# AsteriosPar/mmWave_MSc

Hardware: NVIDIA B200
Metric: radar frames/sec (cluster+track+pose) (higher is better)
Workload: dtype f64

## Files before the change

### mmwave_msc_b200/csrc/mmw_api.cu

```cuda
#include <algorithm>
#include <climits>
#include <dlfcn.h>
#include <cmath>
#include <cstdio>
#include <cstdlib>
#include <cstring>
#include <new>
#include <string>
#include <utility>
#include <vector>

#include "dbscan.cuh"
#include "linalg.cuh"
#include "mmw_internal.cuh"
#include "pose.cuh"
#include "pose_tc.cuh"

using namespace mmw;

static thread_local std::string g_err;

static int fail(int code, const std::string& msg) {
    g_err = msg;
    return code;
}

#define CK(call)                                                                                   \
    do {                                                                                           \
        cudaError_t e__ = (call);                                                                  \
        if (e__ != cudaSuccess)                                                                    \
            return fail(MMW_ERR_CUDA, std::string(#call) + ": " + cudaGetErrorString(e__));        \
    } while (0)

constexpr int kGroup = 4;
constexpr size_t kStageSlack = 64;

struct StageSlot {
    float* pts = nullptr;
    size_t pts_cap = 0;
    int32_t* offsets = nullptr;
    double* dt = nullptr;
    uint8_t* pk = nullptr;
    size_t pk_cap = 0;
    cudaEvent_t uploaded = nullptr, free = nullptr;
};

struct mmw_ctx {
    mmw_config cfg;
    DevConfig dc;
    int device = 0, S = 0, ncap = 0, tcap = 0;
    cudaStream_t stream = nullptr;
    std::vector<mmw_scene_sensor> sensors;
    SensorRec* d_sensors = nullptr;
    double* d_doppler_wrap = nullptr;
    TrackRec* d_tracks = nullptr;
    SceneRec* d_scenes = nullptr;
    float* d_track_ring = nullptr;
    float* d_uring = nullptr;
    float* d_keypoints = nullptr;
    float* d_default_posture = nullptr;
    int32_t* d_assoc = nullptr;
    int32_t* d_labels = nullptr;
    unsigned long long* d_counters = nullptr;
    unsigned long long* d_phase = nullptr;
    bool phase_clocks = false;
    uint8_t* d_ring_hist = nullptr;
    int32_t* h_defer_hint = nullptr;
    int32_t* d_defer_hint = nullptr;
    int32_t* h_rows_hint = nullptr;
    int32_t* d_rows_hint = nullptr;
    int32_t* d_scene_stats = nullptr;
    int32_t* d_defer = nullptr;
    bool fold_pose_index = true;
    StageSlot stage[2];
    unsigned stage_idx = 0;
    unsigned stage_pending = 0;
    cudaStream_t h2d_stream = nullptr, d2h_stream = nullptr;
    cudaStream_t pose_stream = nullptr;
    cudaEvent_t feat_done[2] = {nullptr, nullptr}, packt_done[2] = {nullptr, nullptr}, pose_done[2] = {nullptr, nullptr};
    int32_t *d_row_scene2 = nullptr, *d_row_track2 = nullptr, *d_row_slot2 = nullptr;
    int* d_pose_total2 = nullptr;
    int32_t* d_pose_extra = nullptr;
    int rows_buf = 0;
    unsigned pipe_idx = 0;
    int pipe_r = -1;
    bool pose_pending = false;
    cudaEvent_t packed[2] = {nullptr, nullptr}, results_done[2] = {nullptr, nullptr};
    float* d_results[2] = {nullptr, nullptr};
    double* d_export = nullptr;
    int32_t* d_export_valid = nullptr;
    unsigned char* d_move = nullptr;
    size_t move_cap = 0;
    unsigned result_idx = 0;
    int variant = -1;
    bool has_weights = false;
    int D = 0, Kf = 0, H = 0;
    float* d_blob = nullptr;
    const float *w1 = nullptr, *b1 = nullptr, *w2 = nullptr, *b2 = nullptr, *wd1 = nullptr, *bd1 = nullptr,
                *wd2 = nullptr, *bd2 = nullptr;
    float *d_bn1s = nullptr, *d_bn1t = nullptr, *d_bn2s = nullptr, *d_bn2t = nullptr;
    float* d_feats = nullptr;
    int32_t *d_row_scene = nullptr, *d_row_track = nullptr, *d_row_slot = nullptr;
    int* d_pose_total = nullptr;
    float *d_act2 = nullptr, *d_act3 = nullptr, *d_pose_out = nullptr;
    int pose_cap = 0;
    PoseTc tc;
    bool use_tc = true;
    int last_pose_run = 0;
    uint64_t launches = 0;
    bool profiling = false;
    std::vector<std::pair<cudaEvent_t, int>> marks;
    double kernel_ms[MMW_N_KERNELS] = {0, 0, 0, 0, 0, 0, 0, 0};
    uint64_t kernel_calls[MMW_N_KERNELS] = {0, 0, 0, 0, 0, 0, 0, 0};
};

static cudaError_t sync_main(mmw_ctx* x) {
    if (x->pose_pending) {
        cudaError_t e = cudaStreamSynchronize(x->pose_stream);
        if (e != cudaSuccess) return e;
        x->pose_pending = false;
    }
    return cudaStreamSynchronize(x->stream);
}
static cudaError_t join_pose(mmw_ctx* x) {
    if (!x->pose_pending) return cudaSuccess;
    x->pose_pending = false;
    return cudaStreamWaitEvent(x->stream, x->pose_done[(x->pipe_idx + 1) & 1], 0);
}

static void prof_mark(mmw_ctx* x, int next_kernel) {
    if (!x->profiling) return;
    cudaEvent_t e;
    if (cudaEventCreate(&e) != cudaSuccess) return;
    cudaEventRecord(e, x->stream);
    x->marks.emplace_back(e, next_kernel);
}

static SensorRec sensor_rec(const mmw_scene_sensor& p) {
    SensorRec r{};
    const double ang = p.s_tilt_deg * (M_PI / 180.0);
    r.cos_t = std::cos(ang);
    r.sin_t = std::sin(ang);
    r.s_height = p.s_height;
    r.z_max = p.z_max;
    r.doppler_res = p.doppler_res;
    r.xyz_scale = (float)std::ldexp(1.0, -(p.xyz_q_format));
    return r;
}

static double doppler_wrap(const mmw_scene_sensor& p) { return (double)p.num_doppler_bins / 2 - 1; }

static mmw_scene_sensor config_sensor(const mmw_config& c) {
    mmw_scene_sensor p{};
    p.s_height = c.s_height;
    p.s_tilt_deg = c.s_tilt_deg;
    p.z_max = c.z_max;
    p.doppler_res = c.doppler_res != 0.0 ? c.doppler_res : 1.0;
    p.xyz_q_format = c.xyz_q_format;
    return p;
}

static void fill_devconfig(const mmw_config& c, int ncap, int tcap, DevConfig* d) {
    d->sensor = sensor_rec(config_sensor(c));
    d->db_z_weight = c.db_z_weight;
    d->db_range_weight = c.db_range_weight;
    d->db_eps = c.db_eps;
    d->life_dyn = c.tr_lifetime_dynamic;
    d->life_sta = c.tr_lifetime_static;
    d->vel_thres = c.tr_vel_thres;
    d->gate = c.tr_gate;
    d->q_var = c.kf_q_var;
    d->p_init = c.kf_p_init;
    d->g_init = c.kf_group_disp_init;
    d->a_n = c.kf_a_n;
    d->a_spr = c.kf_a_spr;
    for (int i = 0; i < 6; ++i) d->spread_lim[i] = c.kf_spread_lim[i];
    d->int_mu = c.intensity_mu;
    d->int_std = c.intensity_std;
    d->nudge_thres = c.x_nudge_thres;
    d->nudge_gain = c.x_nudge_gain;
    d->db_min_samples = c.db_min_samples;
    d->ring_size = c.frames_batch + 1;
    d->tr_max_tracks = c.tr_max_tracks;
    d->enable_est = c.kf_enable_est;
    d->est_pointnum = c.kf_est_pointnum;
    d->ncap = ncap;
    d->tcap = tcap;
    grid_screen_config(c.db_eps, c.db_range_weight, c.db_z_weight, c.db_min_samples, &d->grid_inv_h, &d->grid_ybound,
                       &d->grid_ok);
    screen_config(c.db_eps, c.db_range_weight, c.db_z_weight, &d->screen_lo, &d->screen_hi, &d->screen_rmax);
}

static const float kDefaultPosture[57] = {
    0.0000f, -0.0007f, -0.0006f, -0.0038f, -0.1820f, -0.2540f, -0.2579f, 0.1830f, 0.2957f, 0.2940f,
    -0.0805f, -0.1141f, -0.1232f, -0.1358f, 0.0796f, 0.1436f, 0.1558f, 0.1720f, -0.0007f, 0.7699f,
    1.0906f, 1.4020f, 1.5513f, 1.2893f, 1.0360f, 0.7994f, 1.2865f, 1.0483f, 0.8117f, 0.7670f,
    0.3428f, 0.0000f, -0.0746f, 0.7713f, 0.3706f, -0.0128f, -0.0796f, 1.3255f, 0.0752f, 0.0533f,
    0.0203f, 0.0000f, 0.0496f, 0.1350f, 0.1303f, 0.0345f, 0.1277f, 0.1050f, 0.0392f, 0.0533f,
    0.0786f, -0.0056f, 0.0346f, -0.0007f, 0.0683f, -0.0082f, 0.0312f};

extern "C" {

int mmw_abi_version(void) { return MMW_ABI_VERSION; }
const char* mmw_last_error(void) { return g_err.c_str(); }

int mmw_default_config(mmw_config* c) {
    if (!c) return fail(MMW_ERR_INVALID, "cfg is NULL");
    std::memset(c, 0, sizeof(*c));
    c->s_height = 1.8; c->s_tilt_deg = -5; c->z_max = 2.5;
    c->frames_batch = 2; c->db_min_samples = 35;
    c->db_z_weight = 0.4; c->db_range_weight = 0.03; c->db_eps = 0.3;
    c->tr_max_tracks = 4; c->kf_enable_est = 0;
    c->tr_lifetime_dynamic = 3; c->tr_lifetime_static = 7; c->tr_vel_thres = 0.12; c->tr_gate = 4.5;
    c->kf_q_var = 1; c->kf_p_init = 0.1; c->kf_group_disp_init = 0.1; c->kf_a_n = 0.9; c->kf_a_spr = 0.9;
    const double lim[6] = {0.2, 0.2, 2, 1.2, 1.2, 0.2};
    for (int i = 0; i < 6; ++i) c->kf_spread_lim[i] = lim[i];
    c->kf_est_pointnum = 10;
    c->intensity_mu = 27.0187; c->intensity_std = 70.351;
    c->x_nudge_thres = 0.6; c->x_nudge_gain = 0.4;
    std::memcpy(c->default_posture, kDefaultPosture, sizeof(kDefaultPosture));
    c->m_x = 0.32; c->m_y = -0.6; c->m_z = 1.3;
    c->fade_size_max = 0.3; c->fade_size_min = 0.2; c->fade_weight = 0.08;
    c->doppler_res = 1.0;
    c->xyz_q_format = 9;
    return MMW_OK;
}

int mmw_destroy(mmw_ctx* x) {
    if (!x) return MMW_OK;
    cudaSetDevice(x->device);
    if (x->stream) cudaStreamSynchronize(x->stream);
    void* ptrs[] = {x->d_sensors, x->d_doppler_wrap, x->d_export, x->d_export_valid, x->d_move, x->d_tracks, x->d_scenes, x->d_track_ring, x->d_uring, x->d_keypoints, x->d_default_posture,
                    x->d_assoc, x->d_labels, x->d_counters, x->d_phase, x->d_defer, x->d_scene_stats, x->d_ring_hist,
                    x->d_results[0], x->d_results[1], x->d_blob, x->d_bn1s,
                    x->d_bn1t, x->d_bn2s, x->d_bn2t, x->d_feats, x->d_row_scene, x->d_row_track, x->d_row_slot,
                    x->d_pose_total, x->d_act2, x->d_act3, x->d_pose_out, x->d_row_scene2, x->d_row_track2, x->d_row_slot2,
                    x->d_pose_total2, x->d_pose_extra};
    for (void* p : ptrs)
        if (p) cudaFree(p);
    pose_tc_free(&x->tc);
    if (x->h_defer_hint) cudaFreeHost(x->h_defer_hint);
    if (x->h_rows_hint) cudaFreeHost(x->h_rows_hint);
    for (int i = 0; i < 2; ++i) {
        const StageSlot& s = x->stage[i];
        for (void* p : {(void*)s.pts, (void*)s.offsets, (void*)s.dt, (void*)s.pk})
            if (p) cudaFree(p);
        for (cudaEvent_t e : {s.uploaded, s.free, x->packed[i], x->results_done[i], x->feat_done[i], x->packt_done[i],
                              x->pose_done[i]})
            if (e) cudaEventDestroy(e);
    }
    if (x->h2d_stream) cudaStreamDestroy(x->h2d_stream);
    if (x->d2h_stream) cudaStreamDestroy(x->d2h_stream);
    if (x->pose_stream) { cudaStreamSynchronize(x->pose_stream); cudaStreamDestroy(x->pose_stream); }
    if (x->stream) cudaStreamDestroy(x->stream);
    delete x;
    return MMW_OK;
}

int mmw_reset(mmw_ctx* x) {
    if (!x) return fail(MMW_ERR_INVALID, "ctx is NULL");
    CK(cudaSetDevice(x->device));
    if (x->pose_stream) CK(join_pose(x));
    x->pipe_r = -1;
    x->last_pose_run = 0;
    CK(cudaMemsetAsync(x->d_scenes, 0, sizeof(SceneRec) * x->S, x->stream));
    CK(cudaMemsetAsync(x->d_tracks, 0, sizeof(TrackRec) * (size_t)x->S * x->tcap, x->stream));
    CK(cudaMemsetAsync(x->d_counters, 0, sizeof(unsigned long long) * 8, x->stream));
    CK(cudaMemsetAsync(x->d_assoc, 0xff, sizeof(int32_t) * (size_t)x->S * x->ncap, x->stream));
    CK(cudaMemsetAsync(x->d_pose_total, 0, sizeof(int), x->stream));
    CK(cudaMemsetAsync(x->d_pose_total2, 0, sizeof(int), x->stream));
    CK(cudaMemsetAsync(x->d_pose_extra, 0, 2 * sizeof(int32_t), x->stream));
    CK(cudaMemsetAsync(x->d_defer, 0, sizeof(int32_t) * (2 + 2 * (size_t)x->S), x->stream));
    CK(cudaMemsetAsync(x->d_scene_stats, 0, sizeof(int32_t) * 8 * (size_t)x->S, x->stream));
    CK(cudaMemsetAsync(x->d_ring_hist, 0, (size_t)kRing * kHistBytes * x->S, x->stream));
    return MMW_OK;
}

namespace {
struct StateHeader {
    uint32_t magic, abi;
    int32_t S, ncap, tcap, ring_size;
    uint64_t bytes;
};
constexpr uint32_t kStateMagic = 0x4d4d5753u;
struct StatePart { void* dev; size_t bytes; };
enum { kPartScene, kPartTracks, kPartTrackRing, kPartURing, kPartHist, kPartKeypoints, kPartPoseCnt, kNumStateParts };
std::vector<StatePart> state_parts(mmw_ctx* x) {
    const size_t S = x->S;
    return {{x->d_scenes, sizeof(SceneRec) * S},
            {x->d_tracks, sizeof(TrackRec) * S * x->tcap},
            {x->d_track_ring, sizeof(float) * S * x->tcap * kRing * kFeatPts * kRawCols},
            {x->d_uring, sizeof(float) * S * kRing * x->ncap * kRawCols},
            {x->d_ring_hist, (size_t)kRing * kHistBytes * S},
            {x->d_keypoints, sizeof(float) * S * x->tcap * kKp},
            {x->d_defer + 1 + S, sizeof(int32_t) * S}};
}
}

size_t mmw_state_size(mmw_ctx* x) {
    if (!x) return 0;
    size_t n = sizeof(StateHeader);
    for (const StatePart& p : state_parts(x)) n += p.bytes;
    return n;
}

int mmw_state_dump(mmw_ctx* x, void* host_blob, size_t bytes) {
    if (!x || !host_blob) return fail(MMW_ERR_INVALID, "ctx/host_blob is NULL");
    const size_t need = mmw_state_size(x);
    if (bytes < need) return fail(MMW_ERR_CAPACITY, "state blob buffer is smaller than mmw_state_size()");
    CK(cudaSetDevice(x->device));
    CK(sync_main(x));
    StateHeader h{kStateMagic, MMW_ABI_VERSION, x->S, x->ncap, x->tcap, x->dc.ring_size, (uint64_t)need};
    unsigned char* o = static_cast<unsigned char*>(host_blob);
    std::memcpy(o, &h, sizeof(h));
    o += sizeof(h);
    for (const StatePart& p : state_parts(x)) {
        CK(cudaMemcpy(o, p.dev, p.bytes, cudaMemcpyDeviceToHost));
        o += p.bytes;
    }
    return MMW_OK;
}

int mmw_state_restore(mmw_ctx* x, const void* host_blob, size_t bytes) {
    if (!x || !host_blob) return fail(MMW_ERR_INVALID, "ctx/host_blob is NULL");
    StateHeader h;
    if (bytes < sizeof(h)) return fail(MMW_ERR_INVALID, "state blob is truncated");
    std::memcpy(&h, host_blob, sizeof(h));
    if (h.magic != kStateMagic || h.abi != MMW_ABI_VERSION)
        return fail(MMW_ERR_INVALID, "not a state blob of this library version");
    if (h.S != x->S || h.ncap != x->ncap || h.tcap != x->tcap || h.ring_size != x->dc.ring_size)
        return fail(MMW_ERR_INVALID, "state blob was taken from a context of another shape "
                                     "(n_scenes / max_points_per_frame / max_tracks / frames_batch)");
    if (h.bytes != mmw_state_size(x) || bytes < h.bytes) return fail(MMW_ERR_INVALID, "state blob is truncated");
    CK(cudaSetDevice(x->device));
    CK(mmw_sync(x) == MMW_OK ? cudaSuccess : cudaErrorUnknown);
    const unsigned char* o = static_cast<const unsigned char*>(host_blob) + sizeof(h);
    for (const StatePart& p : state_parts(x)) {
        CK(cudaMemcpy(p.dev, o, p.bytes, cudaMemcpyHostToDevice));
        o += p.bytes;
    }
    return MMW_OK;
}

int mmw_create(const mmw_config* cfg, int device, int n_scenes, int max_points, int max_tracks, mmw_ctx** out) {
    if (!cfg || !out) return fail(MMW_ERR_INVALID, "cfg/out is NULL");
    if (n_scenes < 1 || max_points < 1 || max_tracks < 1 || max_tracks > kMaxTcap)
        return fail(MMW_ERR_INVALID, "n_scenes >= 1, max_points >= 1, 1 <= max_tracks <= 32 required");
    if (cfg->frames_batch < 0 || cfg->frames_batch > kRing - 1)
        return fail(MMW_ERR_INVALID, "frames_batch must be 0..2");
    if (cfg->xyz_q_format < 0 || cfg->xyz_q_format > 15) return fail(MMW_ERR_INVALID, "xyz_q_format must be 0..15");
    if (cfg->db_min_samples < 1 || cfg->tr_max_tracks < 0)
        return fail(MMW_ERR_INVALID, "db_min_samples >= 1 and tr_max_tracks >= 0 required");
    int ndev = 0;
    CK(cudaGetDeviceCount(&ndev));
    if (device < 0 || device >= ndev) return fail(MMW_ERR_CUDA, "no such CUDA device");
    CK(cudaSetDevice(device));
    cudaDeviceProp prop;
    CK(cudaGetDeviceProperties(&prop, device));
    const int smem = step_smem_bytes(max_points, max_tracks);
    if ((size_t)smem > prop.sharedMemPerBlockOptin || (size_t)dbscan_big_smem_bytes(max_points) > prop.sharedMemPerBlockOptin)
        return fail(MMW_ERR_CAPACITY, "max_points/max_tracks need more shared memory than one CTA can have");
    mmw_ctx* x = new (std::nothrow) mmw_ctx();
    if (!x) return fail(MMW_ERR_INVALID, "out of host memory");
    x->cfg = *cfg;
    x->device = device; x->S = n_scenes; x->ncap = max_points; x->tcap = max_tracks;
    fill_devconfig(*cfg, max_points, max_tracks, &x->dc);
    const size_t S = n_scenes;
#define ALLOC(p, bytes)                                                       \
    do {                                                                      \
        cudaError_t e__ = cudaMalloc((void**)&(p), (bytes));                  \
        if (e__ != cudaSuccess) {                                             \
            mmw_destroy(x);                                                   \
            return fail(MMW_ERR_CUDA, std::string("cudaMalloc: ") + cudaGetErrorString(e__)); \
        }                                                                     \
    } while (0)
    if (cudaStreamCreateWithFlags(&x->stream, cudaStreamNonBlocking) != cudaSuccess) {
        delete x;
        return fail(MMW_ERR_CUDA, "cudaStreamCreate failed");
    }
    ALLOC(x->d_tracks, sizeof(TrackRec) * S * max_tracks);
    ALLOC(x->d_scenes, sizeof(SceneRec) * S);
    ALLOC(x->d_track_ring, sizeof(float) * S * max_tracks * kRing * kFeatPts * kRawCols);
    ALLOC(x->d_uring, sizeof(float) * S * kRing * max_points * kRawCols);
    ALLOC(x->d_keypoints, sizeof(float) * S * max_tracks * kKp);
    ALLOC(x->d_default_posture, sizeof(float) * kKp);
    ALLOC(x->d_assoc, sizeof(int32_t) * S * max_points);
    ALLOC(x->d_labels, sizeof(int32_t) * S * 3 * max_points);
    ALLOC(x->d_counters, sizeof(unsigned long long) * 8);
    ALLOC(x->d_phase, sizeof(unsigned long long) * (16 + 3 * S + 16));
    ALLOC(x->d_defer, sizeof(int32_t) * (2 + 2 * S));
    ALLOC(x->d_scene_stats, sizeof(int32_t) * 8 * S);
    if (cudaHostAlloc((void**)&x->h_defer_hint, sizeof(int32_t), cudaHostAllocMapped) == cudaSuccess) {
        *x->h_defer_hint = 0;
        if (cudaHostGetDevicePointer((void**)&x->d_defer_hint, x->h_defer_hint, 0) != cudaSuccess) x->d_defer_hint = nullptr;
    } else {
        (void)cudaGetLastError();
        x->h_defer_hint = nullptr;
    }
    if (cudaHostAlloc((void**)&x->h_rows_hint, sizeof(int32_t), cudaHostAllocMapped) == cudaSuccess) {
        *x->h_rows_hint = 0;
        if (cudaHostGetDevicePointer((void**)&x->d_rows_hint, x->h_rows_hint, 0) != cudaSuccess) x->d_rows_hint = nullptr;
    } else {
        (void)cudaGetLastError();
        x->h_rows_hint = nullptr;
    }
    ALLOC(x->d_ring_hist, (size_t)kRing * kHistBytes * S);
    {
        const char* env = getenv("MMW_POSE_INDEX_FOLD");
        x->fold_pose_index = S <= 4096 && !(env && env[0] == '0');
    }
    for (int i = 0; i < 2; ++i) {
        StageSlot& st = x->stage[i];
        st.pts_cap = sizeof(float) * kRawCols * S * max_points + kStageSlack;
        ALLOC(st.pts, st.pts_cap);
        ALLOC(st.offsets, sizeof(int32_t) * kGroup * (S + 1));
        ALLOC(st.dt, sizeof(double) * kGroup * S);
        ALLOC(x->d_results[i], sizeof(float) * S * max_tracks * MMW_RESULT_FLOATS);
        if (cudaEventCreateWithFlags(&st.uploaded, cudaEventDisableTiming) != cudaSuccess ||
            cudaEventCreateWithFlags(&st.free, cudaEventDisableTiming) != cudaSuccess ||
            cudaEventCreateWithFlags(&x->packed[i], cudaEventDisableTiming) != cudaSuccess ||
            cudaEventCreateWithFlags(&x->results_done[i], cudaEventDisableTiming) != cudaSuccess ||
            cudaEventCreateWithFlags(&x->feat_done[i], cudaEventDisableTiming) != cudaSuccess ||
            cudaEventCreateWithFlags(&x->packt_done[i], cudaEventDisableTiming) != cudaSuccess ||
            cudaEventCreateWithFlags(&x->pose_done[i], cudaEventDisableTiming) != cudaSuccess) {
            mmw_destroy(x);
            return fail(MMW_ERR_CUDA, "cudaEventCreate failed");
        }
    }
    int prio_lo = 0, prio_hi = 0;
    cudaDeviceGetStreamPriorityRange(&prio_lo, &prio_hi);
    if (cudaStreamCreateWithFlags(&x->h2d_stream, cudaStreamNonBlocking) != cudaSuccess ||
        cudaStreamCreateWithPriority(&x->pose_stream, cudaStreamNonBlocking, prio_hi) != cudaSuccess ||
        cudaStreamCreateWithFlags(&x->d2h_stream, cudaStreamNonBlocking) != cudaSuccess) {
        mmw_destroy(x);
        return fail(MMW_ERR_CUDA, "cudaStreamCreate failed");
    }
    ALLOC(x->d_pose_total, sizeof(int));
    ALLOC(x->d_pose_extra, 2 * sizeof(int32_t));
    x->pose_cap = n_scenes * max_tracks;
    ALLOC(x->d_row_scene, sizeof(int32_t) * x->pose_cap);
    ALLOC(x->d_row_track, sizeof(int32_t) * x->pose_cap);
    ALLOC(x->d_row_slot, sizeof(int32_t) * x->pose_cap);
    ALLOC(x->d_row_scene2, sizeof(int32_t) * x->pose_cap);
    ALLOC(x->d_row_track2, sizeof(int32_t) * x->pose_cap);
    ALLOC(x->d_row_slot2, sizeof(int32_t) * x->pose_cap);
    ALLOC(x->d_pose_total2, sizeof(int));
    ALLOC(x->d_feats, sizeof(float) * (size_t)x->pose_cap * kRing * kFeatPts * kRawCols);
    ALLOC(x->d_pose_out, sizeof(float) * (size_t)x->pose_cap * kKp);
    ALLOC(x->d_sensors, sizeof(SensorRec) * S);
    ALLOC(x->d_doppler_wrap, sizeof(double) * S);
#undef ALLOC
    cudaMemcpy(x->d_default_posture, cfg->default_posture, sizeof(float) * kKp, cudaMemcpyHostToDevice);
    x->sensors.assign(S, config_sensor(*cfg));
    {
        const std::vector<SensorRec> recs(S, x->dc.sensor);
        const std::vector<double> wrap(S, doppler_wrap(x->sensors[0]));
        if (cudaMemcpy(x->d_sensors, recs.data(), sizeof(SensorRec) * S, cudaMemcpyHostToDevice) != cudaSuccess ||
            cudaMemcpy(x->d_doppler_wrap, wrap.data(), sizeof(double) * S, cudaMemcpyHostToDevice) != cudaSuccess) {
            mmw_destroy(x);
            return fail(MMW_ERR_CUDA, "upload of the sensor table failed");
        }
    }
    cudaMemset(x->d_keypoints, 0, sizeof(float) * S * max_tracks * kKp);
    int rc = mmw_reset(x);
    if (rc != MMW_OK) { mmw_destroy(x); return rc; }
    sync_main(x);
    *out = x;
    return MMW_OK;
}

static int upload_sensors(mmw_ctx* x, int first, int n) {
    std::vector<SensorRec> recs(n);
    std::vector<double> wrap(n);
    for (int i = 0; i < n; ++i) {
        recs[i] = sensor_rec(x->sensors[first + i]);
        wrap[i] = doppler_wrap(x->sensors[first + i]);
    }
    CK(cudaSetDevice(x->device));
    CK(cudaMemcpyAsync(x->d_sensors + first, recs.data(), sizeof(SensorRec) * n, cudaMemcpyHostToDevice, x->stream));
    CK(cudaMemcpyAsync(x->d_doppler_wrap + first, wrap.data(), sizeof(double) * n, cudaMemcpyHostToDevice, x->stream));
    return MMW_OK;
}

int mmw_set_doppler_resolution(mmw_ctx* x, double doppler_res) {
    if (!x) return fail(MMW_ERR_INVALID, "ctx is NULL");
    if (!(doppler_res > 0.0) || !std::isfinite(doppler_res)) return fail(MMW_ERR_INVALID, "doppler_res must be positive and finite");
    x->cfg.doppler_res = doppler_res;
    x->dc.sensor.doppler_res = doppler_res;
    for (mmw_scene_sensor& p : x->sensors) p.doppler_res = doppler_res;
    return upload_sensors(x, 0, x->S);
}

static const char* sensor_error(const mmw_scene_sensor& p) {
    if (!std::isfinite(p.s_height) || !std::isfinite(p.s_tilt_deg) || !std::isfinite(p.z_max) ||
        !std::isfinite(p.doppler_res))
        return "sensor parameters must be finite";
    if (!(p.doppler_res > 0.0)) return "doppler_res must be positive";
    if (p.xyz_q_format < 0 || p.xyz_q_format > 15) return "xyz_q_format must be 0..15";
    if (p.num_doppler_bins < 0) return "num_doppler_bins must not be negative";
    return nullptr;
}

int mmw_set_scene_sensors(mmw_ctx* x, int first, int n, const mmw_scene_sensor* params) {
    if (!x || !params) return fail(MMW_ERR_INVALID, "ctx/params is NULL");
    if (first < 0 || n < 0 || n > x->S - first) return fail(MMW_ERR_INVALID, "scene range out of bounds");
    for (int i = 0; i < n; ++i)
        if (const char* e = sensor_error(params[i])) return fail(MMW_ERR_INVALID, e);
    if (n == 0) return MMW_OK;
    for (int i = 0; i < n; ++i) x->sensors[first + i] = params[i];
    return upload_sensors(x, first, n);
}

int mmw_get_scene_sensors(mmw_ctx* x, int first, int n, mmw_scene_sensor* out) {
    if (!x || !out) return fail(MMW_ERR_INVALID, "ctx/out is NULL");
    if (first < 0 || n < 0 || n > x->S - first) return fail(MMW_ERR_INVALID, "scene range out of bounds");
    for (int i = 0; i < n; ++i) out[i] = x->sensors[first + i];
    return MMW_OK;
}

static int check_scene_list(const mmw_ctx* x, const int32_t* scenes, int n) {
    if (n < 0) return fail(MMW_ERR_INVALID, "n must not be negative");
    std::vector<char> seen(x->S, 0);
    for (int i = 0; i < n; ++i) {
        const int s = scenes[i];
        if (s < 0 || s >= x->S) return fail(MMW_ERR_INVALID, "scene index out of range");
        if (seen[s]) return fail(MMW_ERR_INVALID, "scene index listed twice");
        seen[s] = 1;
    }
    return MMW_OK;
}

int mmw_reset_scenes(mmw_ctx* x, const int32_t* scenes, int n) {
    if (!x || (!scenes && n > 0)) return fail(MMW_ERR_INVALID, "ctx/scenes is NULL");
    const int rc = check_scene_list(x, scenes, n);
    if (rc != MMW_OK) return rc;
    CK(cudaSetDevice(x->device));
    if (x->pose_stream) CK(join_pose(x));
    int32_t* pose_cnt = x->d_defer + 1 + x->S;
    for (int i = 0; i < n; ++i) {
        const size_t s = scenes[i];
        CK(cudaMemsetAsync(x->d_scenes + s, 0, sizeof(SceneRec), x->stream));
        CK(cudaMemsetAsync(x->d_tracks + s * x->tcap, 0, sizeof(TrackRec) * x->tcap, x->stream));
        CK(cudaMemsetAsync(x->d_ring_hist + s * kRing * kHistBytes, 0, (size_t)kRing * kHistBytes, x->stream));
        CK(cudaMemsetAsync(x->d_scene_stats + s * 8, 0, sizeof(int32_t) * 8, x->stream));
        CK(cudaMemsetAsync(pose_cnt + s, 0, sizeof(int32_t), x->stream));
    }
    return MMW_OK;
}

int mmw_sync(mmw_ctx* x) {
    if (!x) return fail(MMW_ERR_INVALID, "ctx is NULL");
    CK(cudaSetDevice(x->device));
    CK(cudaStreamSynchronize(x->h2d_stream));
    CK(sync_main(x));
    CK(cudaStreamSynchronize(x->d2h_stream));
    return MMW_OK;
}

void* mmw_stream(mmw_ctx* x) { return x ? (void*)x->stream : nullptr; }
uint64_t mmw_launch_count(mmw_ctx* x) { return x ? x->launches : 0; }

int mmw_load_pose_weights(mmw_ctx* x, int variant, const float* blob, size_t n) {
    if (!x || !blob) return fail(MMW_ERR_INVALID, "ctx/blob is NULL");
    if (variant != MMW_POSE_2D && variant != MMW_POSE_3D) return fail(MMW_ERR_INVALID, "unknown pose variant");
    const int D = variant == MMW_POSE_3D ? 3 : 1;
    if (D != x->dc.ring_size)
        return fail(MMW_ERR_INVALID, "pose variant does not match frames_batch (2-D net needs frames_batch=0, "
                                     "3-D net needs frames_batch=2; Utils.py:517-520)");
    const int taps = D == 3 ? 27 : 9;
    const int Kf = D * 64 * 32, H = D * 512;
    const size_t sz[16] = {(size_t)taps * 5 * 16, 16, (size_t)taps * 16 * 32, 32, 32, 32, 32, 32,
                           (size_t)Kf * H, (size_t)H, (size_t)H, (size_t)H, (size_t)H, (size_t)H,
                           (size_t)H * kKp, (size_t)kKp};
    size_t off[17];
    off[0] = 0;
    for (int i = 0; i < 16; ++i) off[i + 1] = off[i] + sz[i];
    if (n != off[16]) return fail(MMW_ERR_INVALID, "weight blob has the wrong number of floats for this variant");
    CK(cudaSetDevice(x->device));
    CK(sync_main(x));
    x->has_weights = false;
    x->last_pose_run = 0;
    if (x->d_blob) { cudaFree(x->d_blob); x->d_blob = nullptr; }
    for (float** p : {&x->d_bn1s, &x->d_bn1t, &x->d_bn2s, &x->d_bn2t, &x->d_act2, &x->d_act3})
        if (*p) { cudaFree(*p); *p = nullptr; }
    CK(cudaMalloc((void**)&x->d_blob, sizeof(float) * n));
    CK(cudaMemcpy(x->d_blob, blob, sizeof(float) * n, cudaMemcpyHostToDevice));
    x->w1 = x->d_blob + off[0]; x->b1 = x->d_blob + off[1];
    x->w2 = x->d_blob + off[2]; x->b2 = x->d_blob + off[3];
    x->wd1 = x->d_blob + off[8]; x->bd1 = x->d_blob + off[9];
    x->wd2 = x->d_blob + off[14]; x->bd2 = x->d_blob + off[15];
    auto bn = [&](size_t g, int cnt, float** ds, float** dt) -> int {
        std::vector<float> sc(cnt), sh(cnt);
        for (int i = 0; i < cnt; ++i) {
            const float gamma = blob[off[g] + i], beta = blob[off[g + 1] + i], mean = blob[off[g + 2] + i],
                        var = blob[off[g + 3] + i];
            const float s = gamma / std::sqrt(var + 1e-3f);
            sc[i] = s;
            sh[i] = beta - mean * s;
        }
        if (cudaMalloc((void**)ds, sizeof(float) * cnt) != cudaSuccess) return -1;
        if (cudaMalloc((void**)dt, sizeof(float) * cnt) != cudaSuccess) return -1;
        cudaMemcpy(*ds, sc.data(), sizeof(float) * cnt, cudaMemcpyHostToDevice);
        cudaMemcpy(*dt, sh.data(), sizeof(float) * cnt, cudaMemcpyHostToDevice);
        return 0;
    };
    if (bn(4, 32, &x->d_bn1s, &x->d_bn1t) || bn(10, H, &x->d_bn2s, &x->d_bn2t))
        return fail(MMW_ERR_CUDA, "cudaMalloc failed for BatchNorm constants");
    CK(cudaMalloc((void**)&x->d_act2, sizeof(float) * (size_t)x->pose_cap * Kf));
    CK(cudaMalloc((void**)&x->d_act3, sizeof(float) * (size_t)x->pose_cap * H));
    x->variant = variant; x->D = D; x->Kf = Kf; x->H = H;
    int rc = pose_tc_init(&x->tc, blob, off, D, x->pose_cap);
    if (rc != 0) return fail(MMW_ERR_CUDA, std::string("tensor-core dense path init failed: ") + pose_tc_error());
    x->has_weights = true;
    return MMW_OK;
}

static int run_pose_tc(mmw_ctx* x, const PoseTcRun& r, int max_rows, int b, cudaStream_t st,
                       cudaEvent_t before_fc2 = nullptr) {
    const bool marks = st == x->stream;
    int nl = 0;
    if (marks) prof_mark(x, MMW_K_CONV);
    if (pose_tc_conv(&x->tc, r, st, &nl, b) != 0) return fail(MMW_ERR_CUDA, std::string("tensor-core conv: ") + pose_tc_error());
    x->launches += nl;
    if (marks) prof_mark(x, MMW_K_FC1);
    if (pose_tc_fc1(&x->tc, r, max_rows, st, &nl, x->h_rows_hint ? *(volatile int32_t*)x->h_rows_hint : 0) != 0)
        return fail(MMW_ERR_CUDA, std::string("tensor-core dense 1: ") + pose_tc_error());
    x->launches += nl;
    if (before_fc2) CK(cudaStreamWaitEvent(st, before_fc2, 0));
    if (marks) prof_mark(x, MMW_K_FC2);
    if (pose_tc_fc2(&x->tc, r, max_rows, st, &nl) != 0) return fail(MMW_ERR_CUDA, std::string("tensor-core dense 2: ") + pose_tc_error());
    x->launches += nl;
    if (marks) prof_mark(x, -1);
    return MMW_OK;
}

static int run_pose_net(mmw_ctx* x, float* keypoints_by_slot, int max_rows) {
    x->last_pose_run = x->use_tc && x->tc.ready ? 1 : 2;
    if (x->use_tc && x->tc.ready) {
        PoseTcRun r{x->d_pose_total, x->b1, x->b2, x->d_bn1s, x->d_bn1t, x->bd1, x->d_bn2s, x->d_bn2t, x->bd2,
                    x->d_pose_out, keypoints_by_slot, x->d_row_scene, x->d_row_slot, x->tcap};
        return run_pose_tc(x, r, max_rows, 0, x->stream);
    }
    ConvArgs ca{x->d_feats, x->w1, x->b1, x->w2, x->b2, x->d_bn1s, x->d_bn1t, x->d_act2, x->d_pose_total};
    int grid = max_rows < 296 ? max_rows : 296;
    prof_mark(x, MMW_K_CONV);
    CK(launch_conv(ca, x->D, grid, x->stream));
    x->launches++;
    FcArgs fa{x->d_act2, x->wd1, x->bd1, x->d_bn2s, x->d_bn2t, x->d_act3, x->d_pose_total, x->Kf, x->H};
    prof_mark(x, MMW_K_FC1);
    CK(launch_fc1_simt(fa, max_rows, x->stream));
    x->launches++;
    Fc2Args f2{x->d_act3, x->wd2, x->bd2, x->d_pose_out, keypoints_by_slot, x->d_row_scene, x->d_row_slot,
               x->d_pose_total, x->H, x->tcap};
    grid = (max_rows + 7) / 8 < 148 * 4 ? (max_rows + 7) / 8 : 148 * 4;
    prof_mark(x, MMW_K_FC2);
    CK(launch_fc2(f2, grid, x->stream));
    x->launches++;
    prof_mark(x, -1);
    return MMW_OK;
}

static int pipeline_pose(mmw_ctx* x);
static int estimate_posture_impl(mmw_ctx* x, bool late);
static int launch_pack_tracks(mmw_ctx* x, float* results);

static int launch_feature_stage(mmw_ctx* x, int b, bool late, cudaStream_t st) {
    int* pose_total = b ? x->d_pose_total2 : x->d_pose_total;
    if (!x->fold_pose_index) {
        prof_mark(x, MMW_K_POSE_INDEX);
        CK(launch_pose_index(x->d_scenes, x->S, pose_total, x->d_counters, st));
        x->launches++;
    }
    PoseFeatArgs fa{x->dc, x->d_sensors, x->d_scenes, x->d_tracks, x->d_track_ring, x->d_feats,
                    (x->use_tc && x->tc.ready) ? pose_tc_input(&x->tc, b) : nullptr, b ? x->d_row_scene2 : x->d_row_scene,
                    b ? x->d_row_track2 : x->d_row_track, b ? x->d_row_slot2 : x->d_row_slot,
                    x->fold_pose_index ? x->d_defer + 1 + x->S : nullptr, pose_total, x->d_counters, x->S};
    fa.rows_hint = x->d_rows_hint;
    fa.late_extra = late ? x->d_pose_extra + b : nullptr;
    x->rows_buf = b;
    prof_mark(x, MMW_K_POSE_FEATURES);
    CK(launch_pose_features(fa, x->S, st));
    x->launches++;
    return MMW_OK;
}

static int check_step_flags(const mmw_ctx* x, uint32_t flags) {
    if ((flags & MMW_STEP_POSE) && !x->has_weights)
        return fail(MMW_ERR_STATE, "MMW_STEP_POSE needs mmw_load_pose_weights first");
    if ((flags & MMW_STEP_PIPELINE) && (!(flags & MMW_STEP_POSE) || !(x->use_tc && x->tc.ready)))
        return fail(MMW_ERR_STATE, "MMW_STEP_PIPELINE needs MMW_STEP_POSE and the tensor-core pose path");
    if ((flags & MMW_STEP_PIPELINE) && (flags & MMW_STEP_RECORD_LABELS))
        return fail(MMW_ERR_INVALID, "MMW_STEP_PIPELINE cannot record labels");
    return MMW_OK;
}

static long long offsets_total(const int32_t* offsets, int S) {
    if (offsets[0] != 0) return -1;
    for (int i = 0; i < S; ++i)
        if (offsets[i] > offsets[i + 1]) return -1;
    return offsets[S];
}


static cudaError_t grow(void** buf, size_t* cap, size_t bytes) {
    if (bytes <= *cap) return cudaSuccess;
    cudaError_t e = cudaFree(*buf);
    *buf = nullptr;
    *cap = 0;
    if (e == cudaSuccess && (e = cudaMalloc(buf, bytes)) == cudaSuccess) *cap = bytes;
    return e;
}

static int stage_acquire(mmw_ctx* x, size_t pts_bytes, size_t pk_bytes, int* k) {
    for (int i = 0; i < 2; ++i)
        if (x->stage_pending & (1u << i)) CK(cudaEventRecord(x->stage[i].free, x->stream));
    x->stage_pending = 0;
    *k = (int)(x->stage_idx++ & 1u);
    StageSlot& s = x->stage[*k];
    if (pts_bytes + kStageSlack > s.pts_cap || pk_bytes > s.pk_cap) {
        CK(cudaEventSynchronize(s.free));
        CK(grow((void**)&s.pts, &s.pts_cap, pts_bytes + kStageSlack));
        CK(grow((void**)&s.pk, &s.pk_cap, pk_bytes));
    }
    CK(cudaStreamWaitEvent(x->h2d_stream, s.free, 0));
    return MMW_OK;
}

static int stage_submit(mmw_ctx* x, int k) {
    CK(cudaEventRecord(x->stage[k].uploaded, x->h2d_stream));
    CK(cudaStreamWaitEvent(x->stream, x->stage[k].uploaded, 0));
    return MMW_OK;
}

static void stage_release(mmw_ctx* x, int k) { x->stage_pending |= 1u << k; }

static int step_queue(mmw_ctx* x, StepArgs& a, uint32_t flags);

int mmw_step(mmw_ctx* x, const float* pts, const int32_t* offsets, const double* dt, uint32_t flags) {
    if (!x || !offsets || !dt) return fail(MMW_ERR_INVALID, "ctx/offsets/dt is NULL");
    if ((flags & MMW_STEP_DEVICE_INPUT) && !pts) return fail(MMW_ERR_INVALID, "pts is NULL");
    int rc = check_step_flags(x, flags);
    if (rc != MMW_OK) return rc;
    CK(cudaSetDevice(x->device));
    StepArgs a;
    if (flags & MMW_STEP_DEVICE_INPUT) {
        a.pts = pts; a.offsets = offsets; a.dt = dt;
        return step_queue(x, a, flags);
    }
    const long long total = offsets_total(offsets, x->S);
    if (total < 0) return fail(MMW_ERR_INVALID, "offsets must start at 0 and must not decrease");
    if (total > (long long)x->S * x->ncap)
        return fail(MMW_ERR_CAPACITY, "more points than n_scenes * max_points_per_frame");
    if (total > 0 && !pts) return fail(MMW_ERR_INVALID, "pts is NULL");
    const size_t bytes = ((flags & MMW_STEP_INPUT_I16) ? sizeof(int16_t) : sizeof(float)) * kRawCols * total;
    int k;
    if ((rc = stage_acquire(x, bytes, 0, &k)) != MMW_OK) return rc;
    const StageSlot& s = x->stage[k];
    if (total) CK(cudaMemcpyAsync(s.pts, pts, bytes, cudaMemcpyHostToDevice, x->h2d_stream));
    CK(cudaMemcpyAsync(s.offsets, offsets, sizeof(int32_t) * (x->S + 1), cudaMemcpyHostToDevice, x->h2d_stream));
    CK(cudaMemcpyAsync(s.dt, dt, sizeof(double) * x->S, cudaMemcpyHostToDevice, x->h2d_stream));
    if ((rc = stage_submit(x, k)) != MMW_OK) return rc;
    a.pts = s.pts; a.offsets = s.offsets; a.dt = s.dt;
    rc = step_queue(x, a, flags);
    stage_release(x, k);
    return rc;
}

static int step_queue(mmw_ctx* x, StepArgs& a, uint32_t flags) {
    a.cfg = x->dc;
    a.sensors = x->d_sensors;
    a.tracks = x->d_tracks; a.scenes = x->d_scenes; a.track_ring = x->d_track_ring; a.uring = x->d_uring;
    a.keypoints = x->d_keypoints; a.default_posture = x->d_default_posture; a.assoc_out = x->d_assoc;
    a.labels_out = (flags & MMW_STEP_RECORD_LABELS) ? x->d_labels : nullptr;
    a.counters = x->d_counters; a.n_scenes = x->S; a.flags = flags;
    a.phase_cycles = x->phase_clocks ? x->d_phase : nullptr;
    a.defer_count = x->d_defer;
    a.defer_done = x->d_defer + 1 + 2 * x->S;
    a.defer_list = x->d_defer + 1;
    a.pose_cnt = x->d_defer + 1 + x->S;
    a.scene_stats = x->d_scene_stats;
    a.defer_hint = x->d_defer_hint;
    a.ring_hist = x->d_ring_hist;
    const bool pipelined = (flags & MMW_STEP_PIPELINE) != 0;
    const bool late = !pipelined && (flags & MMW_STEP_POSE) && x->fold_pose_index && x->use_tc && x->tc.ready;
    if (late) {
        a.nr_feats = x->d_feats;
        a.nr_packed = pose_tc_input(&x->tc);
        a.nr_row_scene = x->d_row_scene;
        a.nr_row_track = x->d_row_track;
        a.nr_row_slot = x->d_row_slot;
        a.nr_extra = x->d_pose_extra;
    }
    if (pipelined) {
        if (x->pipe_idx >= 2) CK(cudaStreamWaitEvent(x->stream, x->pose_done[x->pipe_idx & 1u], 0));
    } else {
        CK(join_pose(x));
        x->pipe_r = -1;
    }
    prof_mark(x, MMW_K_STEP);
    CK(launch_step(a, x->stream));
    prof_mark(x, MMW_K_DBSCAN_BIG);
    CK(launch_dbscan_big(a, x->stream, x->h_defer_hint ? *(volatile int32_t*)x->h_defer_hint : 16));
    x->launches += 2;
    prof_mark(x, -1);
    if (pipelined) return pipeline_pose(x);
    if (flags & MMW_STEP_POSE) return estimate_posture_impl(x, late);
    return MMW_OK;
}

int mmw_estimate_posture(mmw_ctx* x) { return estimate_posture_impl(x, false); }

static int estimate_posture_impl(mmw_ctx* x, bool late) {
    if (!x) return fail(MMW_ERR_INVALID, "ctx is NULL");
    if (!x->has_weights) return fail(MMW_ERR_STATE, "estimate_posture needs mmw_load_pose_weights first");
    CK(cudaSetDevice(x->device));
    CK(join_pose(x));
    const int rc = launch_feature_stage(x, 0, late, x->stream);
    if (rc != MMW_OK) return rc;
    return run_pose_net(x, x->d_keypoints, x->pose_cap);
}

int mmw_pose_features_only(mmw_ctx* x) {
    if (!x) return fail(MMW_ERR_INVALID, "ctx is NULL");
    CK(cudaSetDevice(x->device));
    CK(join_pose(x));
    x->last_pose_run = 0;
    return launch_feature_stage(x, 0, false, x->stream);
}

int mmw_set_keypoints(mmw_ctx* x, int scene, int track_index, const float* kp57) {
    if (!x || !kp57) return fail(MMW_ERR_INVALID, "NULL argument");
    if (scene < 0 || scene >= x->S || track_index < 0 || track_index >= x->tcap)
        return fail(MMW_ERR_INVALID, "scene/track out of range");
    CK(cudaSetDevice(x->device));
    CK(sync_main(x));
    TrackRec t;
    CK(cudaMemcpy(&t, x->d_tracks + (size_t)scene * x->tcap + track_index, sizeof(t), cudaMemcpyDeviceToHost));
    CK(cudaMemcpy(x->d_keypoints + ((size_t)scene * x->tcap + t.slot) * kKp, kp57, sizeof(float) * kKp,
                  cudaMemcpyHostToDevice));
    return MMW_OK;
}

int mmw_get_tracks(mmw_ctx* x, mmw_track_out* tracks, int32_t* n_tracks) {
    if (!x) return fail(MMW_ERR_INVALID, "ctx is NULL");
    CK(cudaSetDevice(x->device));
    CK(sync_main(x));
    std::vector<SceneRec> sc(x->S);
    CK(cudaMemcpy(sc.data(), x->d_scenes, sizeof(SceneRec) * x->S, cudaMemcpyDeviceToHost));
    if (n_tracks)
        for (int s = 0; s < x->S; ++s) n_tracks[s] = sc[s].n_tracks;
    if (!tracks) return MMW_OK;
    std::vector<TrackRec> tr((size_t)x->S * x->tcap);
    std::vector<float> kp((size_t)x->S * x->tcap * kKp);
    CK(cudaMemcpy(tr.data(), x->d_tracks, sizeof(TrackRec) * tr.size(), cudaMemcpyDeviceToHost));
    CK(cudaMemcpy(kp.data(), x->d_keypoints, sizeof(float) * kp.size(), cudaMemcpyDeviceToHost));
    for (int s = 0; s < x->S; ++s) {
        for (int k = 0; k < x->tcap; ++k) {
            mmw_track_out& o = tracks[(size_t)s * x->tcap + k];
            std::memset(&o, 0, sizeof(o));
            if (k >= sc[s].n_tracks) { o.id = -1; continue; }
            const TrackRec& t = tr[(size_t)s * x->tcap + k];
            o.id = t.id; o.point_num = t.point_num; o.is_static = t.is_static; o.ring_frames = t.ring_n;
            for (int f = 0; f < kRing; ++f)
                o.ring_counts[f] = f < t.ring_n ? t.ring_cnt[(t.ring_head + f) % x->dc.ring_size] : -1;
            o.lifetime = t.lifetime; o.n_est = t.n_est;
            std::memcpy(o.x, t.x, sizeof(t.x)); std::memcpy(o.P, t.P, sizeof(t.P));
            std::memcpy(o.spread_est, t.spread, sizeof(t.spread));
            std::memcpy(o.group_disp_est, t.G, sizeof(t.G));
            std::memcpy(o.centroid, t.centroid, sizeof(t.centroid));
            std::memcpy(o.min_vals, t.minv, sizeof(t.minv)); std::memcpy(o.max_vals, t.maxv, sizeof(t.maxv));
            std::memcpy(o.keypoints, &kp[((size_t)s * x->tcap + t.slot) * kKp], sizeof(float) * kKp);
        }
    }
    return MMW_OK;
}

int mmw_get_scene_summary(mmw_ctx* x, int32_t* n_tracks, int32_t* next_id, int32_t* last_M) {
    if (!x) return fail(MMW_ERR_INVALID, "ctx is NULL");
    CK(cudaSetDevice(x->device));
    std::vector<SceneRec> sc(x->S);
    CK(cudaMemcpyAsync(sc.data(), x->d_scenes, sizeof(SceneRec) * x->S, cudaMemcpyDeviceToHost, x->stream));
    CK(sync_main(x));
    for (int s = 0; s < x->S; ++s) {
        if (n_tracks) n_tracks[s] = sc[s].n_tracks;
        if (next_id) next_id[s] = sc[s].next_id;
        if (last_M) last_M[s] = sc[s].last_M;
    }
    return MMW_OK;
}

int mmw_get_point_assoc(mmw_ctx* x, int32_t* assoc, size_t n) {
    if (!x || !assoc) return fail(MMW_ERR_INVALID, "ctx/assoc is NULL");
    if (n > (size_t)x->S * x->ncap) return fail(MMW_ERR_CAPACITY, "n exceeds n_scenes * max_points_per_frame");
    CK(cudaSetDevice(x->device));
    CK(cudaMemcpyAsync(assoc, x->d_assoc, sizeof(int32_t) * n, cudaMemcpyDeviceToHost, x->stream));
    CK(sync_main(x));
    return MMW_OK;
}

int mmw_get_labels(mmw_ctx* x, int32_t* labels, int32_t* n_fused) {
    if (!x) return fail(MMW_ERR_INVALID, "ctx is NULL");
    CK(cudaSetDevice(x->device));
    CK(sync_main(x));
    if (labels)
        CK(cudaMemcpy(labels, x->d_labels, sizeof(int32_t) * (size_t)x->S * 3 * x->ncap, cudaMemcpyDeviceToHost));
    if (n_fused) {
        std::vector<SceneRec> sc(x->S);
        CK(cudaMemcpy(sc.data(), x->d_scenes, sizeof(SceneRec) * x->S, cudaMemcpyDeviceToHost));
        for (int s = 0; s < x->S; ++s) n_fused[s] = sc[s].last_ran ? sc[s].dbscan_n : -1;
    }
    return MMW_OK;
}

int mmw_get_status(mmw_ctx* x, uint32_t* flags) {
    if (!x || !flags) return fail(MMW_ERR_INVALID, "ctx/flags is NULL");
    CK(cudaSetDevice(x->device));
    CK(sync_main(x));
    std::vector<SceneRec> sc(x->S);
    CK(cudaMemcpy(sc.data(), x->d_scenes, sizeof(SceneRec) * x->S, cudaMemcpyDeviceToHost));
    for (int s = 0; s < x->S; ++s) flags[s] = sc[s].flags;
    return MMW_OK;
}

int mmw_get_ring_counts(mmw_ctx* x, int32_t* counts) {
    if (!x || !counts) return fail(MMW_ERR_INVALID, "ctx/counts is NULL");
    CK(cudaSetDevice(x->device));
    CK(sync_main(x));
    std::vector<SceneRec> sc(x->S);
    CK(cudaMemcpy(sc.data(), x->d_scenes, sizeof(SceneRec) * x->S, cudaMemcpyDeviceToHost));
    for (int s = 0; s < x->S; ++s)
        for (int f = 0; f < kRing; ++f)
            counts[s * kRing + f] =
                f < sc[s].ring_n ? sc[s].ring_cnt[(sc[s].ring_head + f) % x->dc.ring_size] : -1;
    return MMW_OK;
}

static int ring_edit(mmw_ctx* x, int scene, bool clear) {
    if (!x) return fail(MMW_ERR_INVALID, "ctx is NULL");
    if (scene < 0 || scene >= x->S) return fail(MMW_ERR_INVALID, "scene out of range");
    CK(cudaSetDevice(x->device));
    CK(sync_main(x));
    SceneRec sc;
    CK(cudaMemcpy(&sc, x->d_scenes + scene, sizeof(sc), cudaMemcpyDeviceToHost));
    if (clear) {
        sc.ring_n = 0; sc.ring_head = 0; sc.ring_cnt[0] = sc.ring_cnt[1] = sc.ring_cnt[2] = 0;
        sc.ring_ph_gone = 1;
    } else if (!sc.ring_ph_gone) {
        sc.ring_ph_gone = 1;
    } else if (sc.ring_n > 0) {
        sc.ring_cnt[sc.ring_head] = 0;
        sc.ring_head = (sc.ring_head + 1) % x->dc.ring_size;
        sc.ring_n -= 1;
    }
    CK(cudaMemcpy(x->d_scenes + scene, &sc, sizeof(sc), cudaMemcpyHostToDevice));
    return MMW_OK;
}
int mmw_ring_pop(mmw_ctx* x, int scene) { return ring_edit(x, scene, false); }
int mmw_ring_clear(mmw_ctx* x, int scene) { return ring_edit(x, scene, true); }

int mmw_get_pose_rows(mmw_ctx* x, int32_t* n_rows, int32_t* scene_idx, int32_t* track_idx, float* feats,
                      size_t cap_floats) {
    if (!x || !n_rows) return fail(MMW_ERR_INVALID, "ctx/n_rows is NULL");
    CK(cudaSetDevice(x->device));
    CK(sync_main(x));
    const int b = x->rows_buf;
    int n = 0;
    CK(cudaMemcpy(&n, b ? x->d_pose_total2 : x->d_pose_total, sizeof(int), cudaMemcpyDeviceToHost));
    *n_rows = n;
    if (n == 0 || (!scene_idx && !track_idx && !feats)) return MMW_OK;
    std::vector<int32_t> hs(n), ht(n);
    CK(cudaMemcpy(hs.data(), b ? x->d_row_scene2 : x->d_row_scene, sizeof(int32_t) * n, cudaMemcpyDeviceToHost));
    CK(cudaMemcpy(ht.data(), b ? x->d_row_track2 : x->d_row_track, sizeof(int32_t) * n, cudaMemcpyDeviceToHost));
    std::vector<int> order(n);
    for (int i = 0; i < n; ++i) order[i] = i;
    std::stable_sort(order.begin(), order.end(), [&](int p, int q) { return hs[p] != hs[q] ? hs[p] < hs[q] : ht[p] < ht[q]; });
    for (int i = 0; i < n; ++i) {
        if (scene_idx) scene_idx[i] = hs[order[i]];
        if (track_idx) track_idx[i] = ht[order[i]];
    }
    if (feats) {
        const size_t per = (size_t)x->dc.ring_size * kFeatPts * kRawCols;
        if (cap_floats < per * n) return fail(MMW_ERR_CAPACITY, "feats buffer too small");
        std::vector<float> hf(per * n);
        CK(cudaMemcpy(hf.data(), x->d_feats, sizeof(float) * per * n, cudaMemcpyDeviceToHost));
        for (int i = 0; i < n; ++i) std::memcpy(feats + per * i, hf.data() + per * order[i], sizeof(float) * per);
    }
    return MMW_OK;
}

int mmw_get_counters(mmw_ctx* x, uint64_t out[8], int reset) {
    if (!x || !out) return fail(MMW_ERR_INVALID, "ctx/out is NULL");
    CK(cudaSetDevice(x->device));
    CK(sync_main(x));
    unsigned long long h[8];
    CK(cudaMemcpy(h, x->d_counters, sizeof(h), cudaMemcpyDeviceToHost));
    for (int i = 0; i < 8; ++i) out[i] = h[i];
    if (reset) CK(cudaMemset(x->d_counters, 0, sizeof(h)));
    return MMW_OK;
}

}

namespace mmw {

__global__ void preprocess_kernel(DevConfig c, const float* pts, size_t n, double* world, uint8_t* keep) {
    const size_t i = (size_t)blockIdx.x * blockDim.x + threadIdx.x;
    if (i >= n) return;
    const float* p = pts + i * kRawCols;
    double w[6];
    world_from_raw(c.sensor, p[0], p[1], p[2], p[3], w);
    double* o = world + i * 8;
#pragma unroll
    for (int k = 0; k < 6; ++k) o[k] = w[k];
    o[6] = __dmul_rn((double)p[3], c.sensor.doppler_res);
    o[7] = (double)p[4];
    keep[i] = ((w[2] <= c.sensor.z_max) && (w[2] > 0.0) && (w[1] > 0.0)) ? 1 : 0;
}

__global__ void __launch_bounds__(kStepThreads) dbscan_stage_kernel(DevConfig c, const double* xyz,
                                                                    const int32_t* offsets, double eps, int min_samples,
                                                                    int32_t* labels, int maxB) {
    extern __shared__ __align__(16) unsigned char smem[];
    double* X = reinterpret_cast<double*>(smem);
    double* Y = X + maxB;
    double* Z = Y + maxB;
    int* par = reinterpret_cast<int*>(Z + maxB);
    int* cl = par + maxB;
    int* scan = cl + maxB;
    const int off = offsets[blockIdx.x];
    const int B = offsets[blockIdx.x + 1] - off;
    if (B <= 0) return;
    for (int b = threadIdx.x; b < B; b += blockDim.x) {
        X[b] = xyz[(size_t)(off + b) * 3 + 0];
        Y[b] = xyz[(size_t)(off + b) * 3 + 1];
        Z[b] = xyz[(size_t)(off + b) * 3 + 2];
    }
    __syncthreads();
    dbscan_block(NbExact{c, X, Y, Z, eps}, B, min_samples, par, cl, scan);
    for (int b = threadIdx.x; b < B; b += blockDim.x) labels[off + b] = cl[b];
}

__global__ void __launch_bounds__(128) kalman_predict_kernel(double* x, double* P, const double* dt, int n, double q_var) {
    __shared__ double sx[9], sP[81];
    const int i = blockIdx.x, tid = threadIdx.x;
    const Elem el(tid);
    if (tid < 81) sP[tid] = P[(size_t)i * 81 + tid];
    if (tid < 9) sx[tid] = x[(size_t)i * 9 + tid];
    __syncthreads();
    const double pv = tid < 81 ? kf_predict_elem(sP, dt[i], q_var, el) : 0.0;
    const double xn = tid < 9 ? kf_predict_x(sx, dt[i], tid) : 0.0;
    if (tid < 81) P[(size_t)i * 81 + tid] = pv;
    if (tid < 9) x[(size_t)i * 9 + tid] = xn;
}

__global__ void __launch_bounds__(128) kalman_update_kernel(double* x, double* P, const double* z, const double* R,
                                                            const uint8_t* life0, int n, double thres, double gain) {
    __shared__ double sx[9], sP[81], sz[6], sR[36], sS[36], sM1[81], sK[54], sKR[54];
    const int i = blockIdx.x, tid = threadIdx.x, lane = tid & 31, warp = tid >> 5;
    const Elem el(tid);
    if (tid < 81) sP[tid] = P[(size_t)i * 81 + tid];
    if (tid < 36) sR[tid] = R[(size_t)i * 36 + tid];
    if (tid < 9) sx[tid] = x[(size_t)i * 9 + tid];
    if (tid < 6) sz[tid] = z[(size_t)i * 6 + tid];
    __syncthreads();
    if (tid < 36) sS[tid] = sP[el.i6 * 9 + el.a6] + sR[tid];
    __syncthreads();
    if (warp == 0) {
        double r[6];
        (void)inv6_spd_half(lane < 16 ? sS : nullptr, lane, r);
        __syncwarp();
        if (lane >= 6 && lane < 12) {
#pragma unroll
            for (int k = 0; k < 6; ++k) sS[k * 6 + (lane - 6)] = r[k];
        }
    }
    __syncthreads();
    if (tid < 54) sK[tid] = kf_update_K_elem(sP, sS, el);
    __syncthreads();
    if (tid < 81) sM1[tid] = kf_update_M1_elem(sP, sK, el);
    if (tid < 54) sKR[tid] = kf_update_KR_elem(sK, sR, el);
    if (warp == 3) {
        const double xv = lane < 9 ? kf_update_x(sx, sz, sK, lane) : 0.0;
        __syncwarp();
        if (lane < 9) sx[lane] = xv;
    }
    __syncthreads();
    if (tid < 81) sP[tid] = kf_update_P_elem(sM1, sK, sKR, el);
    if (tid == 96) kf_update_nudge(sx, sz, life0[i] != 0, thres, gain);
    __syncthreads();
    if (tid < 81) P[(size_t)i * 81 + tid] = sP[tid];
    if (tid < 9) x[(size_t)i * 9 + tid] = sx[tid];
}

__global__ void __launch_bounds__(128) gate_stage_kernel(const double* pts, int M, const double* hx, const double* C,
                                                         int T, double gate, double* d2, int32_t* assoc) {
    extern __shared__ __align__(16) unsigned char smem[];
    double* gp = reinterpret_cast<double*>(smem);
    double* sC = gp + (size_t)T * kGateWords;
    const int warp = threadIdx.x >> 5, lane = threadIdx.x & 31;
    for (int e = threadIdx.x; e < T * 36; e += blockDim.x) sC[e] = C[e];
    for (int e = threadIdx.x; e < T * 6; e += blockDim.x) gp[(e / 6) * kGateWords + 21 + e % 6] = hx[e];
    __syncthreads();
    for (int j0 = 0; j0 < T; j0 += 8) {
        const int j = j0 + 2 * warp + (lane >> 4);
        const bool live = j < T;
        if (__ballot_sync(kFull, live) == 0u) continue;
        double r[6];
        const double det = inv6_spd_half(live ? sC + j * 36 : nullptr, lane, r);
        if (live) gate_pack_half(gp + j * kGateWords, r, det, lane);
    }
    __syncthreads();
    for (int i = threadIdx.x; i < M; i += blockDim.x) {
        double w[6];
#pragma unroll
        for (int k = 0; k < 6; ++k) w[k] = pts[(size_t)i * 6 + k];
        double best = INFINITY;
        int bj = -1;
        for (int j = 0; j < T; ++j) {
            const double v = gate_score(gp + j * kGateWords, w);
            d2[(size_t)i * T + j] = v;
            if (v < gate && v < best) { best = v; bj = j; }
        }
// ... 1076 lines not shown
```

### mmwave_msc_b200/csrc/mmw_internal.cuh

```cuda
#pragma once
#include <utility>
#include <cuda_runtime.h>
#include <stdint.h>
#include "../../include/mmw.h"

namespace mmw {

constexpr int kRing = 3;
constexpr int kFeatPts = 64;
constexpr int kRawCols = 5;
constexpr int kKp = 57;
constexpr int kHistBytes = 272;
constexpr int kStepThreads = 128;
constexpr int kStepWarps = kStepThreads / 32;
constexpr int kMaxTcap = 32;

struct SensorRec {
    double cos_t, sin_t, s_height, z_max;
    double doppler_res;
    float xyz_scale;
    int32_t pad;
};
static_assert(sizeof(SensorRec) == 48, "SensorRec is three 16-byte chunks (moved with one bulk copy)");

__device__ __forceinline__ SensorRec sensor_at_use(const SensorRec& r) {
    const volatile SensorRec& v = r;
    SensorRec o;
    o.cos_t = v.cos_t; o.sin_t = v.sin_t; o.s_height = v.s_height; o.z_max = v.z_max;
    o.doppler_res = v.doppler_res; o.xyz_scale = v.xyz_scale; o.pad = 0;
    return o;
}

struct DevConfig {
    SensorRec sensor;
    double db_z_weight, db_range_weight, db_eps;
    double life_dyn, life_sta, vel_thres, gate;
    double q_var, p_init, g_init, a_n, a_spr;
    double spread_lim[6];
    double int_mu, int_std, nudge_thres, nudge_gain;
    int db_min_samples, ring_size, tr_max_tracks, enable_est, est_pointnum;
    int ncap, tcap;
    float grid_inv_h, grid_ybound;
    int grid_ok;
    float screen_lo, screen_hi, screen_rmax;
};

struct TrackRec {
    double x[9];
    double P[81];
    double spread[6];
    double G[36];
    double centroid[6];
    double minv[6];
    double maxv[6];
    double n_est;
    double lifetime;
    int32_t id;
    int32_t point_num;
    int32_t is_static;
    int32_t slot;
    int32_t ring_n;
    int32_t ring_head;
    int32_t ring_cnt[kRing];
    int32_t pad[3];
};
static_assert(sizeof(TrackRec) % 16 == 0, "TrackRec must be a whole number of 16-byte chunks");
constexpr int kTrackWords = sizeof(TrackRec) / 8;

struct SceneRec {
    int32_t n_tracks;
    int32_t next_id;
    int32_t ring_n;
    int32_t ring_head;
    int32_t ring_cnt[kRing];
    uint32_t slot_mask;
    uint32_t flags;
    int32_t last_M;
    int32_t last_ran;
    int32_t dbscan_n;
    int32_t pose_base;
    int32_t ring_ph_gone;
    int32_t pad[2];
};
static_assert(sizeof(SceneRec) == 64, "SceneRec is one 64-byte record");

struct StepArgs {
    DevConfig cfg;
    const SensorRec* sensors;
    const float* pts;
    const int32_t* offsets;
    const double* dt;
    TrackRec* tracks;
    SceneRec* scenes;
    float* track_ring;
    float* uring;
    float* keypoints;
    const float* default_posture;
    int32_t* assoc_out;
    int32_t* labels_out;
    unsigned long long* counters;
    unsigned long long* phase_cycles;
    int32_t* defer_list;
    int32_t* defer_count;
    int32_t* defer_done;
    int32_t* defer_hint;
    int32_t* pose_cnt;
    uint8_t* ring_hist;
    int32_t* scene_stats;
    int n_scenes;
    uint32_t flags;
    float* nr_feats = nullptr;
    void* nr_packed = nullptr;
    int32_t *nr_row_scene = nullptr, *nr_row_track = nullptr, *nr_row_slot = nullptr;
    int32_t* nr_extra = nullptr;
    long long pts_row0 = 0;
};

__device__ __forceinline__ void pdl_wait() { asm volatile("griddepcontrol.wait;" ::: "memory"); }
__device__ __forceinline__ void pdl_launch_dependents() { asm volatile("griddepcontrol.launch_dependents;" ::: "memory"); }

template <class... KArgs, class... Args>
inline cudaError_t launch_pdl(void (*kernel)(KArgs...), dim3 grid, dim3 block, size_t smem, cudaStream_t st,
                              dim3 cluster, Args&&... args) {
    cudaLaunchConfig_t cfg{};
    cfg.gridDim = grid; cfg.blockDim = block; cfg.dynamicSmemBytes = smem; cfg.stream = st;
    cudaLaunchAttribute at[2];
    int n = 0;
    if (cluster.x * cluster.y * cluster.z > 1) {
        at[n].id = cudaLaunchAttributeClusterDimension;
        at[n].val.clusterDim.x = cluster.x; at[n].val.clusterDim.y = cluster.y; at[n].val.clusterDim.z = cluster.z;
        ++n;
    }
    at[n].id = cudaLaunchAttributeProgrammaticStreamSerialization;
    at[n].val.programmaticStreamSerializationAllowed = 1;
    ++n;
    cfg.attrs = at; cfg.numAttrs = n;
    return cudaLaunchKernelEx(&cfg, kernel, std::forward<Args>(args)...);
}

constexpr int kMaxDevices = 64;
inline cudaError_t ensure_smem_attr(const void* fn, int* configured , int smem) {
    int dev = 0;
    cudaError_t e = cudaGetDevice(&dev);
    if (e != cudaSuccess) return e;
    if (dev < 0 || dev >= kMaxDevices) return cudaErrorInvalidDevice;
    const int want = smem < 0 ? 1 : smem;
    if (want > configured[dev]) {
        if (smem >= 0) {
            e = cudaFuncSetAttribute(fn, cudaFuncAttributeMaxDynamicSharedMemorySize, smem);
            if (e != cudaSuccess) return e;
        }
        e = cudaFuncSetAttribute(fn, cudaFuncAttributePreferredSharedMemoryCarveout, cudaSharedmemCarveoutMaxShared);
        if (e != cudaSuccess) return e;
        configured[dev] = want;
    }
    return cudaSuccess;
}

__device__ __forceinline__ void world_yz(const SensorRec& c, double y, double z, double& yw, double& zw) {
    yw = __dadd_rn(__dmul_rn(c.cos_t, y), __dmul_rn(-c.sin_t, z));
    zw = __dadd_rn(__dadd_rn(__dmul_rn(c.sin_t, y), __dmul_rn(c.cos_t, z)), c.s_height);
}

__device__ __forceinline__ int ring_wrap(int v, int ring_size) {
    v = v >= ring_size ? v - ring_size : v;
    return v >= ring_size ? v - ring_size : v;
}

__device__ __forceinline__ double div_zero_fast(double num, double den) {
    const bool z = num == 0.0 && den != 0.0 && fabs(den) <= 1.7976931348623157e308;
    double nsafe = z ? 1.0 : num;
    asm("" : "+d"(nsafe));
    const double q = __ddiv_rn(nsafe, den);
    return z ? (den < 0.0 ? -num : num) : q;
}

__device__ __forceinline__ void world_from_raw(const SensorRec& c, float fx, float fy, float fz, float fd,
                                               double w[6]) {
    const double x = fx, y = fy, z = fz, d = __dmul_rn((double)fd, c.doppler_res);
    const double r = sqrt(__dadd_rn(__dadd_rn(__dmul_rn(x, x), __dmul_rn(y, y)), __dmul_rn(z, z)));
    double vx, vy, vz;
    if (r == 0.0) {
        vx = 0.0; vy = d; vz = 0.0;
    } else {
        vx = div_zero_fast(__dmul_rn(d, x), r);
        vy = div_zero_fast(__dmul_rn(d, y), r);
        vz = div_zero_fast(__dmul_rn(d, z), r);
    }
    w[0] = x;
    world_yz(c, y, z, w[1], w[2]);
    w[3] = vx;
    w[4] = __dadd_rn(__dmul_rn(c.cos_t, vy), __dmul_rn(-c.sin_t, vz));
    w[5] = __dadd_rn(__dmul_rn(c.sin_t, vy), __dmul_rn(c.cos_t, vz));
}

struct FadeCfg { double m_x, m_y, m_z, smax, smin, weight; };

__device__ __forceinline__ void projection_point(const FadeCfg& f, double xo, double yo, double zo, double& xp,
                                                 double& zp) {
    const double xd = xo - f.m_x, yd = yo - f.m_y, zd = zo - f.m_z;
    xp = (xd == 0.0) ? xo : (-f.m_y / (yd / xd)) + f.m_x;
    zp = (zd == 0.0) ? zo : (-f.m_y / (yd / zd)) + f.m_z;
}

__device__ __forceinline__ void write_fade_square(const FadeCfg& fade, double x0, double x1, const float* kp, float* rec) {
    double cx, cz;
    projection_point(fade, x0 + (double)kp[3], x1 + (double)kp[41], (double)kp[22], cx, cz);
    const double size = fmax(fade.smin, fmin(fade.smax, fade.smax - (x1 + (double)kp[12]) * fade.weight));
    rec[68] = (float)cx; rec[69] = (float)cz; rec[70] = (float)size; rec[71] = 0.f;
}

__device__ __forceinline__ bool eps_neighbour(const DevConfig& c, double x1, double y1, double z1, double x2,
                                              double y2, double z2, double eps) {
    const double w = __dsub_rn(1.0, __dmul_rn(__dmul_rn(__dadd_rn(y1, y2), 0.5), c.db_range_weight));
    const double dx = __dsub_rn(x1, x2), dy = __dsub_rn(y1, y2), dz = __dsub_rn(z1, z2);
    const double q = __dadd_rn(__dadd_rn(__dmul_rn(dx, dx), __dmul_rn(dy, dy)),
                               __dmul_rn(c.db_z_weight, __dmul_rn(dz, dz)));
    return __dmul_rn(w, q) <= eps;
}

}
```

### mmwave_msc_b200/csrc/pose.cuh

```cuda
#pragma once
#include <cuda_bf16.h>

#include "mmw_internal.cuh"

namespace mmw {

struct PoseFeatArgs {
    DevConfig cfg;
    const SensorRec* sensors;
    const SceneRec* scenes;
    const TrackRec* tracks;
    const float* track_ring;
    float* feats;
    __nv_bfloat16* packed;
    int32_t* row_scene;
    int32_t* row_track;
    int32_t* row_slot;
    const int32_t* pose_cnt;
    int* pose_total;
    unsigned long long* counters;
    int n_scenes;
    int dbg = 0;
    const int32_t* late_extra = nullptr;
    int* rows_hint = nullptr;
};

struct ConvArgs {
    const float* feats;
    const float *w1, *b1, *w2, *b2, *bn1_scale, *bn1_shift;
    float* act2;
    const int* n_rows;
};

struct FcArgs {
    const float* A;
    const float* W;
    const float *bias, *bn_scale, *bn_shift;
    float* out;
    const int* n_rows;
    int K, H;
};

struct Fc2Args {
    const float* act3;
    const float* W;
    const float* bias;
    float* out;
    float* keypoints;
    const int32_t* row_scene;
    const int32_t* row_slot;
    const int* n_rows;
    int H, tcap;
};

cudaError_t launch_pose_index(SceneRec* scenes, int S, int* pose_total, unsigned long long* counters,
                              cudaStream_t st);
cudaError_t launch_pose_features(const PoseFeatArgs& a, int S, cudaStream_t st);
cudaError_t launch_conv(const ConvArgs& a, int D, int grid, cudaStream_t st);
cudaError_t launch_fc1_simt(const FcArgs& a, int max_rows, cudaStream_t st);
cudaError_t launch_fc2(const Fc2Args& a, int grid, cudaStream_t st);

int step_smem_bytes(int ncap, int tcap);
int dbscan_big_smem_bytes(int ncap);
cudaError_t launch_step(const StepArgs& a, cudaStream_t stream);
cudaError_t launch_dbscan_big(const StepArgs& a, cudaStream_t stream, int grid = 16);

}
```

### mmwave_msc_b200/csrc/pose_kernels.cu

```cuda
#include "mmw_internal.cuh"
#include <cstdlib>

#include "pose.cuh"
#include "pose_feat.cuh"

namespace mmw {

__global__ void __launch_bounds__(1024) pose_index_kernel(SceneRec* scenes, int S, int* pose_total,
                                                          unsigned long long* counters) {
    __shared__ int wsum[32];
    __shared__ int running;
    const int tid = threadIdx.x, lane = tid & 31, warp = tid >> 5;
    if (tid == 0) running = 0;
    __syncthreads();
    for (int base = 0; base < S; base += 1024) {
        const int s = base + tid;
        int v = 0;
        if (s < S && scenes[s].last_ran) v = scenes[s].n_tracks;
        int incl = v;
#pragma unroll
        for (int o = 1; o < 32; o <<= 1) {
            const int t = __shfl_up_sync(0xffffffffu, incl, o);
            if (lane >= o) incl += t;
        }
        if (lane == 31) wsum[warp] = incl;
        __syncthreads();
        int before = 0, tot = 0;
        for (int w = 0; w < 32; ++w) {
            const int cw = wsum[w];
            if (w < warp) before += cw;
            tot += cw;
        }
        const int r0 = running;
        if (s < S) scenes[s].pose_base = r0 + before + incl - v;
        __syncthreads();
        if (tid == 0) running = r0 + tot;
        __syncthreads();
    }
    if (tid == 0) {
        *pose_total = running;
        atomicAdd(&counters[7], (unsigned long long)running);
    }
}

constexpr int kFeatWarps = 6;
__global__ void __launch_bounds__(kFeatWarps * 32, 7) pose_feature_kernel(PoseFeatArgs a) {
    __shared__ __align__(16) long long keys[kFeatWarps][kFeatPts];
    __shared__ __align__(16) float srow[kFeatWarps][kFeatPts * kRawCols];
    __shared__ __align__(16) uint4 spk[kFeatWarps][kFeatPts * 2];
    const int s = blockIdx.x;
    const int lane = threadIdx.x & 31, warp = threadIdx.x >> 5;
    const bool late = a.late_extra != nullptr && a.pose_cnt != nullptr;
    if (!late) pdl_wait();
    pdl_launch_dependents();
    SceneRec sc;
    if (!late) sc = a.scenes[s];
    int pose_base = late ? 0 : sc.pose_base;
    int n_tr = 0;
    if (a.dbg & 1) { pose_base = 2 * s; n_tr = late ? __ldg(a.pose_cnt + s) : (sc.last_ran ? sc.n_tracks : 0); }
    else if (a.pose_cnt != nullptr) {
        __shared__ int wpart[kFeatWarps];
        int part = 0;
        for (int i = threadIdx.x; i < s; i += kFeatWarps * 32) part += __ldg(a.pose_cnt + i);
#pragma unroll
        for (int o = 16; o > 0; o >>= 1) part += __shfl_xor_sync(0xffffffffu, part, o);
        if (lane == 0) wpart[warp] = part;
        __syncthreads();
        pose_base = 0;
#pragma unroll
        for (int w = 0; w < kFeatWarps; ++w) pose_base += wpart[w];
        n_tr = late ? __ldg(a.pose_cnt + s) : (sc.last_ran ? sc.n_tracks : 0);
    } else {
        n_tr = sc.last_ran ? sc.n_tracks : 0;
    }
    const DevConfig& c = a.cfg;
    __shared__ SensorRec sr;
    if (threadIdx.x < sizeof(SensorRec) / 8)
        reinterpret_cast<double*>(&sr)[threadIdx.x] = reinterpret_cast<const double*>(a.sensors + s)[threadIdx.x];
    __syncthreads();
    const int nfr = c.ring_size;
    const int items = n_tr * nfr;
    for (int item = warp; item < items; item += kFeatWarps) {
        const int k = item / nfr, f = item - k * nfr;
        const TrackRec* t = a.tracks + (size_t)s * c.tcap + k;
        const int row = pose_base + k;
        const int slot = t->slot, rn = t->ring_n, rh = t->ring_head;
        if (f == 0 && lane == 0) {
            a.row_scene[row] = s;
            a.row_track[row] = k;
            a.row_slot[row] = slot;
        }
        float* out = a.feats + ((size_t)row * nfr + f) * (kFeatPts * kRawCols);
        uint4* pk = a.packed ? reinterpret_cast<uint4*>(a.packed + (size_t)row * nfr * kFeatPts * 16) : nullptr;
        const float* src = nullptr;
        int cnt = 0;
        if (f < rn) {
            const int phys = ring_wrap(rh + f, c.ring_size);
            cnt = t->ring_cnt[phys];
            src = a.track_ring + (((size_t)s * c.tcap + slot) * kRing + phys) * (kFeatPts * kRawCols);
        }
        pose_feature_item<true>(c, sr, src, cnt, t->centroid[0], t->centroid[1], f, out, pk, keys[warp], srow[warp],
                                spk[warp], lane, a.dbg);
    }
    if (a.pose_cnt != nullptr && !(a.dbg & 1) && s == a.n_scenes - 1 && threadIdx.x == 0) {
        int total = pose_base + n_tr;
        if (late) {
            pdl_wait();
            total += __ldcg(a.late_extra);
        }
        *a.pose_total = total;
        if (a.rows_hint != nullptr) *a.rows_hint = total;
        atomicAdd(&a.counters[7], (unsigned long long)total);
    }
}

template <int D>
__global__ void __launch_bounds__(256) conv_kernel(ConvArgs a) {
    constexpr int P = D * 64;
    constexpr int TAPS = (D == 3 ? 27 : 9);
    constexpr int A1S = 17;
    extern __shared__ __align__(16) float sm[];
    float* w2 = sm;
    float* w1 = w2 + TAPS * 16 * 32;
    float* in = w1 + TAPS * 5 * 16;
    float* a1 = in + P * 5;
    __shared__ int total;
    if (threadIdx.x == 0) total = *a.n_rows;
    for (int i = threadIdx.x; i < TAPS * 16 * 32; i += 256) w2[i] = a.w2[i];
    for (int i = threadIdx.x; i < TAPS * 5 * 16; i += 256) w1[i] = a.w1[i];
    __syncthreads();
    for (int row = blockIdx.x; row < total; row += gridDim.x) {
        const float* feat = a.feats + (size_t)row * P * 5;
        for (int i = threadIdx.x; i < P * 5; i += 256) in[i] = feat[i];
        __syncthreads();
        for (int it = threadIdx.x; it < P * 2; it += 256) {
            const int pos = it >> 1, c0 = (it & 1) * 8;
            const int d = pos / 64, h = (pos / 8) % 8, w = pos % 8;
            float acc[8];
#pragma unroll
            for (int q = 0; q < 8; ++q) acc[q] = a.b1[c0 + q];
            for (int tap = 0; tap < TAPS; ++tap) {
                const int kd = (D == 3) ? tap / 9 - 1 : 0, kh = (tap / 3) % 3 - 1, kw = tap % 3 - 1;
                const int dd = d + kd, hh = h + kh, ww = w + kw;
                if (dd < 0 || dd >= D || hh < 0 || hh >= 8 || ww < 0 || ww >= 8) continue;
                const float* ip = in + ((dd * 8 + hh) * 8 + ww) * 5;
                const float* wp_ = w1 + tap * 5 * 16 + c0;
#pragma unroll
                for (int ci = 0; ci < 5; ++ci) {
                    const float v = ip[ci];
#pragma unroll
                    for (int q = 0; q < 8; ++q) acc[q] = fmaf(v, wp_[ci * 16 + q], acc[q]);
                }
            }
#pragma unroll
            for (int q = 0; q < 8; ++q) a1[pos * A1S + c0 + q] = fmaxf(acc[q], 0.f);
        }
        __syncthreads();
        float* out = a.act2 + (size_t)row * P * 32;
        for (int it = threadIdx.x; it < P * 4; it += 256) {
            const int pos = it % P, c0 = (it / P) * 8;
            const int d = pos / 64, h = (pos / 8) % 8, w = pos % 8;
            float acc[8];
#pragma unroll
            for (int q = 0; q < 8; ++q) acc[q] = a.b2[c0 + q];
            for (int tap = 0; tap < TAPS; ++tap) {
                const int kd = (D == 3) ? tap / 9 - 1 : 0, kh = (tap / 3) % 3 - 1, kw = tap % 3 - 1;
                const int dd = d + kd, hh = h + kh, ww = w + kw;
                if (dd < 0 || dd >= D || hh < 0 || hh >= 8 || ww < 0 || ww >= 8) continue;
                const float* ip = a1 + ((dd * 8 + hh) * 8 + ww) * A1S;
                const float* wp_ = w2 + tap * 16 * 32 + c0;
#pragma unroll
                for (int ci = 0; ci < 16; ++ci) {
                    const float v = ip[ci];
#pragma unroll
                    for (int q = 0; q < 8; ++q) acc[q] = fmaf(v, wp_[ci * 32 + q], acc[q]);
                }
            }
#pragma unroll
            for (int q = 0; q < 8; ++q)
                out[pos * 32 + c0 + q] = fmaf(fmaxf(acc[q], 0.f), a.bn1_scale[c0 + q], a.bn1_shift[c0 + q]);
        }
        __syncthreads();
    }
}

size_t conv_smem_bytes(int D) {
    const int P = D * 64, TAPS = (D == 3 ? 27 : 9);
    return sizeof(float) * (size_t)(TAPS * 16 * 32 + TAPS * 5 * 16 + P * 5 + P * 17);
}

cudaError_t launch_conv(const ConvArgs& a, int D, int grid, cudaStream_t st) {
    const size_t smem = conv_smem_bytes(D);
    cudaError_t e;
    if (D == 3) {
        e = cudaFuncSetAttribute(conv_kernel<3>, cudaFuncAttributeMaxDynamicSharedMemorySize, (int)smem);
        if (e != cudaSuccess) return e;
        conv_kernel<3><<<grid, 256, smem, st>>>(a);
    } else {
        e = cudaFuncSetAttribute(conv_kernel<1>, cudaFuncAttributeMaxDynamicSharedMemorySize, (int)smem);
        if (e != cudaSuccess) return e;
        conv_kernel<1><<<grid, 256, smem, st>>>(a);
    }
    return cudaGetLastError();
}

__global__ void __launch_bounds__(256) fc1_simt_kernel(FcArgs a) {
    __shared__ float As[16][64 + 4];
    __shared__ float Bs[16][64 + 4];
    const int n = *a.n_rows;
    const int m0 = blockIdx.y * 64, h0 = blockIdx.x * 64;
    if (m0 >= n) return;
    const int tx = threadIdx.x % 16, ty = threadIdx.x / 16;
    float acc[4][4] = {};
    for (int k0 = 0; k0 < a.K; k0 += 16) {
        for (int i = threadIdx.x; i < 64 * 16; i += 256) {
            const int r = i / 16, kk = i % 16;
            As[kk][r] = (m0 + r < n) ? a.A[(size_t)(m0 + r) * a.K + k0 + kk] : 0.f;
        }
        for (int i = threadIdx.x; i < 16 * 64; i += 256) {
            const int kk = i / 64, cc = i % 64;
            Bs[kk][cc] = a.W[(size_t)(k0 + kk) * a.H + h0 + cc];
        }
        __syncthreads();
#pragma unroll
        for (int kk = 0; kk < 16; ++kk) {
            float av[4], bv[4];
#pragma unroll
            for (int i = 0; i < 4; ++i) av[i] = As[kk][ty * 4 + i];
#pragma unroll
            for (int j = 0; j < 4; ++j) bv[j] = Bs[kk][tx * 4 + j];
#pragma unroll
            for (int i = 0; i < 4; ++i)
#pragma unroll
                for (int j = 0; j < 4; ++j) acc[i][j] = fmaf(av[i], bv[j], acc[i][j]);
        }
        __syncthreads();
    }
#pragma unroll
    for (int i = 0; i < 4; ++i) {
        const int m = m0 + ty * 4 + i;
        if (m >= n) continue;
#pragma unroll
        for (int j = 0; j < 4; ++j) {
            const int h = h0 + tx * 4 + j;
            const float v = fmaxf(acc[i][j] + a.bias[h], 0.f);
            a.out[(size_t)m * a.H + h] = fmaf(v, a.bn_scale[h], a.bn_shift[h]);
        }
    }
}

cudaError_t launch_fc1_simt(const FcArgs& a, int max_rows, cudaStream_t st) {
    dim3 grid(a.H / 64, (max_rows + 63) / 64);
    fc1_simt_kernel<<<grid, 256, 0, st>>>(a);
    return cudaGetLastError();
}

constexpr int kFc2Rows = 8;
__global__ void __launch_bounds__(128) fc2_kernel(Fc2Args a) {
    extern __shared__ float xs[];
    __shared__ float part[kFc2Rows][64];
    const int n = *a.n_rows;
    const int o = threadIdx.x & 63, half = threadIdx.x >> 6;
    const int hlen = a.H / 2;
    for (int r0 = blockIdx.x * kFc2Rows; r0 < n; r0 += gridDim.x * kFc2Rows) {
        const int nr = min(kFc2Rows, n - r0);
        for (int i = threadIdx.x; i < kFc2Rows * a.H; i += 128) {
            const int r = i / a.H;
            xs[i] = r < nr ? a.act3[(size_t)(r0 + r) * a.H + (i - r * a.H)] : 0.f;
        }
        __syncthreads();
        float acc[kFc2Rows];
#pragma unroll
        for (int r = 0; r < kFc2Rows; ++r) acc[r] = 0.f;
        if (o < kKp) {
            const float* wp_ = a.W + (size_t)(half * hlen) * kKp + o;
            const float* xp = xs + half * hlen;
#pragma unroll 4
            for (int h = 0; h < hlen; ++h) {
                const float w = __ldg(wp_ + (size_t)h * kKp);
#pragma unroll
                for (int r = 0; r < kFc2Rows; ++r) acc[r] = fmaf(xp[r * a.H + h], w, acc[r]);
            }
        }
        if (half == 1) {
#pragma unroll
            for (int r = 0; r < kFc2Rows; ++r) part[r][o] = acc[r];
        }
        __syncthreads();
        if (half == 0 && o < kKp) {
#pragma unroll
            for (int r = 0; r < kFc2Rows; ++r) {
                if (r >= nr) break;
                const float v = (acc[r] + part[r][o]) + a.bias[o];
                const int row = r0 + r;
                a.out[(size_t)row * kKp + o] = v;
                if (a.keypoints != nullptr) {
                    const int s = a.row_scene[row], slot = a.row_slot[row];
                    a.keypoints[((size_t)s * a.tcap + slot) * kKp + o] = v;
                }
            }
        }
        __syncthreads();
    }
}

cudaError_t launch_fc2(const Fc2Args& a, int grid, cudaStream_t st) {
    const size_t smem = (size_t)kFc2Rows * a.H * sizeof(float);
    static int configured[kMaxDevices] = {0};
    cudaError_t e = ensure_smem_attr(reinterpret_cast<const void*>(fc2_kernel), configured, 64 * 1024);
    if (e != cudaSuccess) return e;
    fc2_kernel<<<grid, 128, smem, st>>>(a);
    return cudaGetLastError();
}

cudaError_t launch_pose_index(SceneRec* scenes, int S, int* pose_total, unsigned long long* counters,
                              cudaStream_t st) {
    pose_index_kernel<<<1, 1024, 0, st>>>(scenes, S, pose_total, counters);
    return cudaGetLastError();
}

cudaError_t launch_pose_features(const PoseFeatArgs& a, int S, cudaStream_t st) {
    static int configured[kMaxDevices] = {0};
    cudaError_t e = ensure_smem_attr(reinterpret_cast<const void*>(pose_feature_kernel), configured, -1);
    if (e != cudaSuccess) return e;
    const char* env = getenv("MMW_FEAT_DBG");
    const int dbg = env ? atoi(env) : 0;
    PoseFeatArgs b = a;
    b.dbg = dbg;
    return launch_pdl(pose_feature_kernel, dim3(S), dim3(kFeatWarps * 32), 0, st, dim3(1, 1, 1), b);
}

}
```

### mmwave_msc_b200/csrc/pose_tc.cu

```cuda
#include <cuda.h>
#include <cuda_bf16.h>
#include <cstdio>
#include <cstdlib>
#include <cstring>
#include <string>
#include <vector>

#include "pose_tc.cuh"

namespace mmw {

__device__ __forceinline__ uint32_t smem_u32(const void* p) { return (uint32_t)__cvta_generic_to_shared(p); }

__device__ __forceinline__ void mbar_init(uint64_t* bar, uint32_t count) {
    asm volatile("mbarrier.init.shared::cta.b64 [%0], %1;" ::"r"(smem_u32(bar)), "r"(count));
}
__device__ __forceinline__ void mbar_expect_tx(uint64_t* bar, uint32_t bytes) {
    asm volatile("mbarrier.arrive.expect_tx.shared::cta.b64 _, [%0], %1;" ::"r"(smem_u32(bar)), "r"(bytes) : "memory");
}
__device__ __forceinline__ void mbar_arrive(uint64_t* bar) {
    asm volatile("mbarrier.arrive.shared::cta.b64 _, [%0];" ::"r"(smem_u32(bar)) : "memory");
}
__device__ __forceinline__ void mbar_wait(uint64_t* bar, uint32_t parity) {
    asm volatile(
        "{\n\t"
        ".reg .pred p;\n\t"
        "WAIT_LOOP:\n\t"
        "mbarrier.try_wait.parity.shared::cta.b64 p, [%0], %1;\n\t"
        "@p bra DONE;\n\t"
        "bra WAIT_LOOP;\n\t"
        "DONE:\n\t"
        "}" ::"r"(smem_u32(bar)), "r"(parity) : "memory");
}
__device__ __forceinline__ void tma_load_2d(void* dst, const CUtensorMap* map, uint64_t* bar, int c0, int c1) {
    asm volatile(
        "cp.async.bulk.tensor.2d.shared::cluster.global.mbarrier::complete_tx::bytes [%0], [%1, {%3, %4}], [%2];" ::
            "r"(smem_u32(dst)), "l"(map), "r"(smem_u32(bar)), "r"(c0), "r"(c1)
        : "memory");
}
__device__ __forceinline__ void umma_bf16(uint32_t tmem_d, uint64_t adesc, uint64_t bdesc, uint32_t idesc,
                                          uint32_t accumulate) {
    asm volatile(
        "{\n\t"
        ".reg .pred p;\n\t"
        "setp.ne.b32 p, %4, 0;\n\t"
        "tcgen05.mma.cta_group::1.kind::f16 [%0], %1, %2, %3, p;\n\t"
        "}" ::"r"(tmem_d), "l"(adesc), "l"(bdesc), "r"(idesc), "r"(accumulate)
        : "memory");
}
__device__ __forceinline__ void umma_commit(uint64_t* bar) {
    asm volatile("tcgen05.commit.cta_group::1.mbarrier::arrive::one.shared::cluster.b64 [%0];" ::"r"(smem_u32(bar))
                 : "memory");
}
__device__ __forceinline__ void tmem_ld32(uint32_t taddr, uint32_t (&v)[32]) {
    asm volatile(
        "tcgen05.ld.sync.aligned.32x32b.x32.b32 "
        "{%0, %1, %2, %3, %4, %5, %6, %7, %8, %9, %10, %11, %12, %13, %14, %15, "
        "%16, %17, %18, %19, %20, %21, %22, %23, %24, %25, %26, %27, %28, %29, %30, %31}, [%32];"
        : "=r"(v[0]), "=r"(v[1]), "=r"(v[2]), "=r"(v[3]), "=r"(v[4]), "=r"(v[5]), "=r"(v[6]), "=r"(v[7]), "=r"(v[8]),
          "=r"(v[9]), "=r"(v[10]), "=r"(v[11]), "=r"(v[12]), "=r"(v[13]), "=r"(v[14]), "=r"(v[15]), "=r"(v[16]),
          "=r"(v[17]), "=r"(v[18]), "=r"(v[19]), "=r"(v[20]), "=r"(v[21]), "=r"(v[22]), "=r"(v[23]), "=r"(v[24]),
          "=r"(v[25]), "=r"(v[26]), "=r"(v[27]), "=r"(v[28]), "=r"(v[29]), "=r"(v[30]), "=r"(v[31])
        : "r"(taddr));
    asm volatile("tcgen05.wait::ld.sync.aligned;" ::: "memory");
}
__device__ __forceinline__ void tc_fence_before() { asm volatile("tcgen05.fence::before_thread_sync;" ::: "memory"); }
__device__ __forceinline__ void tc_fence_after() { asm volatile("tcgen05.fence::after_thread_sync;" ::: "memory"); }

template <uint32_t COLS>
__device__ __forceinline__ void tmem_alloc(uint32_t* slot) {
    asm volatile("tcgen05.alloc.cta_group::1.sync.aligned.shared::cta.b32 [%0], %1;" ::"r"(smem_u32(slot)), "r"(COLS)
                 : "memory");
    asm volatile("tcgen05.relinquish_alloc_permit.cta_group::1.sync.aligned;" ::: "memory");
}
template <uint32_t COLS>
__device__ __forceinline__ void tmem_dealloc(uint32_t addr) {
    asm volatile("tcgen05.dealloc.cta_group::1.sync.aligned.b32 %0, %1;" ::"r"(addr), "r"(COLS) : "memory");
}

template <int SW>
__device__ __forceinline__ uint64_t make_desc(uint32_t saddr) {
    constexpr uint64_t layout = SW == 128 ? 2 : (SW == 64 ? 4 : 6);
    uint64_t d = 0;
    d |= (uint64_t)((saddr >> 4) & 0x3fff);
    d |= (uint64_t)(((8 * SW) >> 4) & 0x3fff) << 32;
    d |= (uint64_t)1 << 46;
    d |= layout << 61;
    return d;
}
__device__ __forceinline__ constexpr uint32_t make_idesc(int n) {
    return (1u << 4) | (1u << 7) | (1u << 10) | ((uint32_t)(n >> 3) << 17) | ((uint32_t)(128 >> 4) << 24);
}

__device__ __forceinline__ void split2(float x, __nv_bfloat16& hi, __nv_bfloat16& lo) {
    hi = __float2bfloat16_rn(x);
    lo = __float2bfloat16_rn(x - __bfloat162float(hi));
}

struct ConvTcArgs {
    const int* n_rows;
    const float *bias, *bn_scale, *bn_shift;
    const __nv_bfloat16* in;
    __nv_bfloat16* out0;
    __nv_bfloat16* out1;
    int dbg;
};

constexpr int kSlabThreads = 320;
constexpr int kSlabAtoms = 1 + 5 * 10 + 3;

template <int CK>
__host__ __device__ constexpr int slab_ring() { return CK == 16 ? 8 : 4; }

template <int CK, int NOUT>
__host__ __device__ constexpr int conv_b_tap_bytes() { return CK == 32 ? (NOUT + NOUT / 2) * 32 : NOUT * CK * 2; }
template <int CK, int NOUT>
constexpr int conv_smem_bytes_tc(int taps) {
    return taps * conv_b_tap_bytes<CK, NOUT>() + slab_ring<CK>() * kSlabAtoms * (CK / 8) * 128 + 1024 + 1024;
}

__device__ __forceinline__ uint64_t make_desc_interleaved(uint32_t saddr, uint32_t lbo, uint32_t sbo) {
    uint64_t d = 0;
    d |= (uint64_t)((saddr >> 4) & 0x3fff);
    d |= (uint64_t)((lbo >> 4) & 0x3fff) << 16;
    d |= (uint64_t)((sbo >> 4) & 0x3fff) << 32;
    d |= (uint64_t)1 << 46;
    return d;
}

template <int CK, int NOUT, int MODE, int KD>
__global__ void __launch_bounds__(kSlabThreads, 1)
conv_slab_kernel(const __grid_constant__ CUtensorMap map_b, const ConvTcArgs a) {
    constexpr int D = 3;
    constexpr bool TRIPLE = KD == 1;
    constexpr int NCH = CK / 8;
    constexpr int ATOM = NCH * 128;
    constexpr int SLAB_BYTES = kSlabAtoms * ATOM;
    constexpr int NSLAB = slab_ring<CK>();
    constexpr int B_TAP = conv_b_tap_bytes<CK, NOUT>();
    constexpr int B_ROWS = CK == 32 ? NOUT + NOUT / 2 : NOUT;
    constexpr int COUT = NOUT / 2;
    constexpr uint32_t TCOLS = 4 * NOUT;
    constexpr int taps = KD == 3 ? 27 : 9;
    constexpr int MT = 2;

    extern __shared__ unsigned char smem_raw[];
    unsigned char* smem = reinterpret_cast<unsigned char*>(((uintptr_t)smem_raw + 1023) & ~(uintptr_t)1023);
    unsigned char* sB = smem;
    unsigned char* slab = smem + taps * B_TAP;
    uint64_t* sfull = reinterpret_cast<uint64_t*>(slab + NSLAB * SLAB_BYTES);
    uint64_t* sempty = sfull + NSLAB;
    uint64_t* tfull = sempty + NSLAB;
    uint64_t* tempty = tfull + 2;
    uint64_t* bfull = tempty + 2;
    uint32_t* tmem_slot = reinterpret_cast<uint32_t*>(bfull + 1);
    float* sconst = reinterpret_cast<float*>(tmem_slot + 2);

    const int warp = threadIdx.x >> 5, lane = threadIdx.x & 31;

    for (int i = threadIdx.x; i < NSLAB * SLAB_BYTES / 16; i += kSlabThreads)
        reinterpret_cast<uint4*>(slab)[i] = make_uint4(0, 0, 0, 0);
    if (threadIdx.x < COUT) {
        sconst[threadIdx.x] = a.bias[threadIdx.x];
        sconst[COUT + threadIdx.x] = MODE == 1 ? a.bn_scale[threadIdx.x] : 1.f;
        sconst[2 * COUT + threadIdx.x] = MODE == 1 ? a.bn_shift[threadIdx.x] : 0.f;
    }
    asm volatile("fence.proxy.async.shared::cta;" ::: "memory");
    if (warp == 4 && lane == 0) {
        asm volatile("prefetch.tensormap [%0];" ::"l"(&map_b) : "memory");
        for (int c = 0; c < NSLAB; ++c) { mbar_init(&sfull[c], 128); mbar_init(&sempty[c], MT); }
        for (int b = 0; b < 2; ++b) { mbar_init(&tfull[b], MT); mbar_init(&tempty[b], 4); }
        mbar_init(bfull, 1);
        asm volatile("fence.mbarrier_init.release.cluster;" ::: "memory");
        mbar_expect_tx(bfull, taps * B_TAP);
        for (int t = 0; t < taps; ++t) tma_load_2d(sB + t * B_TAP, &map_b, bfull, 0, t * B_ROWS);
    }
    if (warp == 4) tmem_alloc<TCOLS>(tmem_slot);
    tc_fence_before();
    __syncthreads();
    tc_fence_after();
    const uint32_t tmem_base = *tmem_slot;
    pdl_wait();
    pdl_launch_dependents();
    const int n_samples = *a.n_rows;
    const int rows = TRIPLE ? (n_samples + 2) / 3 : n_samples;

    if (warp < 4) {
        constexpr int ITEMS = D * 64 * NCH / 128;
        const int tid = threadIdx.x;
        int dstoff[ITEMS];
        const int hsrc = tid & 7;
#pragma unroll
        for (int j = 0; j < ITEMS; ++j) {
            const int i = tid + 128 * j;
            const int chunk = (i >> 3) % NCH, w = (i / (8 * NCH)) & 7, d = i / (64 * NCH);
            dstoff[j] = (1 + (d + 1) * 10 + (w + 1)) * ATOM + chunk * 128;
        }
        uint4 cur[ITEMS], nxt[ITEMS];
        auto load_row = [&](int row, uint4 (&r)[ITEMS]) {
            const uint4* src = reinterpret_cast<const uint4*>(a.in) + (size_t)row * (D * 64 * NCH);
#pragma unroll
            for (int j = 0; j < ITEMS; ++j) {
                const bool there = !TRIPLE || row * 3 + (tid + 128 * j) / (64 * NCH) < n_samples;
                r[j] = there ? __ldg(src + tid + 128 * j) : make_uint4(0, 0, 0, 0);
            }
        };
        if ((int)blockIdx.x < rows && !(a.dbg & 8)) load_row(blockIdx.x, cur);
        int u = 0;
        for (int row = blockIdx.x; row < rows; row += gridDim.x) {
            const int next = row + gridDim.x;
            if (next < rows && !(a.dbg & 8)) load_row(next, nxt);
#pragma unroll
            for (int c = 0; c < 3; ++c, ++u) {
                const int slot = u % NSLAB;
                mbar_wait(&sempty[slot], (uint32_t)(((u / NSLAB) & 1) ^ 1));
                unsigned char* sl = slab + slot * SLAB_BYTES;
                const int hh = hsrc - (c - 1);
                if (hh >= 0 && hh <= 7 && !(a.dbg & 8)) {
#pragma unroll
                    for (int j = 0; j < ITEMS; ++j) *reinterpret_cast<uint4*>(sl + dstoff[j] + hh * 16) = cur[j];
                }
                const int hz = c == 0 ? 0 : (c == 2 ? 7 : -1);
                if (hz >= 0 && hsrc == hz) {
#pragma unroll
                    for (int j = 0; j < ITEMS; ++j)
                        *reinterpret_cast<uint4*>(sl + dstoff[j] + hz * 16) = make_uint4(0, 0, 0, 0);
                }
                asm volatile("fence.proxy.async.shared::cta;" ::: "memory");
                mbar_arrive(&sfull[slot]);
            }
#pragma unroll
            for (int j = 0; j < ITEMS; ++j) cur[j] = nxt[j];
        }
    } else if (warp == 4 || warp == 5) {
        const int mt = warp - 4;
        if (lane == 0) {
            constexpr uint32_t idesc = make_idesc(NOUT);
            constexpr uint32_t idesc_lo = make_idesc(NOUT / 2);
            const uint64_t db0 = make_desc<32>(smem_u32(sB));
            const uint64_t da00 = make_desc_interleaved(smem_u32(slab) + (uint32_t)((1 + mt * 16) * ATOM), 128, ATOM);
            mbar_wait(bfull, 0);
            int n = 0, u = 0;
            for (int row = blockIdx.x; row < rows; row += gridDim.x, ++n) {
                const int buf = n & 1;
                mbar_wait(&tempty[buf], (uint32_t)(((n >> 1) & 1) ^ 1));
                tc_fence_after();
                const uint32_t tmem_d = tmem_base + (uint32_t)((buf * 2 + mt) * NOUT);
#pragma unroll
                for (int c = 0; c < 3; ++c, ++u) {
                    const int slot = u % NSLAB;
                    mbar_wait(&sfull[slot], (uint32_t)((u / NSLAB) & 1));
                    tc_fence_after();
                    const uint64_t da0 = da00 + (uint64_t)((slot * SLAB_BYTES) >> 4);
#pragma unroll
                    for (int kdi = 0; kdi < (KD == 3 ? 3 : 1); ++kdi) {
#pragma unroll
                        for (int kwi = 0; kwi < 3; ++kwi) {
                            const int kd = KD == 3 ? kdi - 1 : 0, kw = kwi - 1;
                            const int tap = KD == 3 ? (kdi * 3 + c) * 3 + kwi : c * 3 + kwi;
                            const bool first = c == 0 && kdi == 0 && kwi == 0;
                            const int aoff = ((1 + kd) * 10 + kw) * ATOM;
#pragma unroll
                            for (int kk = 0; kk < CK / 16; ++kk)
                                if (!(a.dbg & 16)) umma_bf16(tmem_d, da0 + (uint64_t)((aoff + kk * 256) >> 4),
                                          db0 + (uint64_t)((tap * B_TAP + kk * NOUT * 32) >> 4), kk == 0 ? idesc : idesc_lo,
                                          (first && kk == 0) ? 0u : 1u);
                        }
                    }
                    umma_commit(&sempty[slot]);
                }
                umma_commit(&tfull[buf]);
            }
        }
    } else {
        const int q = warp & 3;
        int n = 0;
        for (int row = blockIdx.x; row < rows; row += gridDim.x, ++n) {
            const int buf = n & 1;
            mbar_wait(&tfull[buf], (uint32_t)((n >> 1) & 1));
            tc_fence_after();
            float y[2][COUT];
#pragma unroll
            for (int mt = 0; mt < MT; ++mt) {
                const uint32_t taddr = tmem_base + ((uint32_t)(q * 32) << 16) + (uint32_t)((buf * 2 + mt) * NOUT);
                uint32_t v[32];
                tmem_ld32(taddr, v);
                if (NOUT == 32) {
#pragma unroll
                    for (int c = 0; c < COUT; ++c) y[mt][c] = __uint_as_float(v[c]) + __uint_as_float(v[COUT + c]);
                } else {
#pragma unroll
                    for (int c = 0; c < 32; ++c) y[mt][c % COUT] = __uint_as_float(v[c]);
                    tmem_ld32(taddr + 32, v);
#pragma unroll
                    for (int c = 0; c < 32; ++c) y[mt][c % COUT] += __uint_as_float(v[c]);
                }
            }
            tc_fence_before();
            __syncwarp();
            if (lane == 0) mbar_arrive(&tempty[buf]);
#pragma unroll
            for (int mt = 0; mt < MT; ++mt) {
                const int m = q * 32 + lane;
                const int aidx = mt * 16 + (m >> 3), hh = m & 7;
                const int d = aidx / 10, w2 = aidx % 10;
                if (d >= D || w2 < 1 || w2 > 8 || (a.dbg & 32)) continue;
                if (TRIPLE && row * 3 + d >= n_samples) continue;
                __align__(16) __nv_bfloat16 hi[COUT], lo[COUT];
#pragma unroll
                for (int c = 0; c < COUT; ++c) {
                    float x = fmaxf(y[mt][c] + sconst[c], 0.f);
                    if (MODE == 1) x = fmaf(x, sconst[COUT + c], sconst[2 * COUT + c]);
                    split2(x, hi[c], lo[c]);
                }
                if (MODE == 0) {
                    uint4* o = reinterpret_cast<uint4*>(a.out0) +
                               ((((size_t)row * D + d) * 8 + (w2 - 1)) * (2 * COUT / 8)) * 8 + hh;
#pragma unroll
                    for (int i = 0; i < COUT / 8; ++i) o[i * 8] = reinterpret_cast<const uint4*>(hi)[i];
#pragma unroll
                    for (int i = 0; i < COUT / 8; ++i) o[(COUT / 8 + i) * 8] = reinterpret_cast<const uint4*>(lo)[i];
                } else {
                    const size_t p = ((size_t)row * D + d) * 64 + hh * 8 + (w2 - 1);
                    uint4* oh = reinterpret_cast<uint4*>(a.out0 + p * COUT);
                    uint4* ol = reinterpret_cast<uint4*>(a.out1 + p * COUT);
#pragma unroll
                    for (int i = 0; i < COUT / 8; ++i) {
                        oh[i] = reinterpret_cast<const uint4*>(hi)[i];
                        ol[i] = reinterpret_cast<const uint4*>(lo)[i];
                    }
                }
            }
        }
    }
    tc_fence_before();
    __syncthreads();
    if (warp == 4) {
        tc_fence_after();
        tmem_dealloc<TCOLS>(tmem_base);
    }
}

struct GemmTcArgs {
    const int* n_rows;
    const float *bias, *bn_scale, *bn_shift;
    __nv_bfloat16 *out_hi, *out_lo;
    float* out;
    float* keypoints;
    const int32_t *row_scene, *row_slot;
    int K, N, tcap;
    int dbg;
    float* results = nullptr;
    const int32_t* row_track = nullptr;
    FadeCfg fade = {0, 0, 0, 0, 0, 0};
};

constexpr int kGemmThreads = 192;
constexpr int kBK = 64;

__device__ __forceinline__ uint32_t cluster_ctarank() {
    uint32_t r;
    asm volatile("mov.u32 %0, %%cluster_ctarank;" : "=r"(r));
    return r;
}
__device__ __forceinline__ void cluster_sync_all() {
    asm volatile("barrier.cluster.arrive.release.aligned;" ::: "memory");
    asm volatile("barrier.cluster.wait.acquire.aligned;" ::: "memory");
}
__device__ __forceinline__ uint32_t mapa_shared(uint32_t addr, uint32_t rank) {
    uint32_t r;
    asm volatile("mapa.shared::cluster.u32 %0, %1, %2;" : "=r"(r) : "r"(addr), "r"(rank));
    return r;
}

__device__ __forceinline__ void gemm_load_row_maps(const GemmTcArgs& a, int* maps, int row0, int nrow, int et) {
    for (int i = et; i < nrow; i += 128) {
        maps[i] = a.keypoints || a.results ? __ldg(a.row_scene + row0 + i) : 0;
        maps[128 + i] = a.keypoints ? __ldg(a.row_slot + row0 + i) : 0;
        maps[256 + i] = a.results ? __ldg(a.row_track + row0 + i) : 0;
    }
}
__device__ __forceinline__ void gemm_store_keypoints(const GemmTcArgs& a, const float* stg, const int* maps, int row0,
                                                     int nrow, int q, int lane, int et) {
    float* o = a.out + (size_t)row0 * kKp;
    for (int i = et; i < nrow * kKp; i += 128) o[i] = stg[i];
    if (a.keypoints) {
        for (int r = q; r < nrow; r += 4) {
            float* kp = a.keypoints + ((size_t)maps[r] * a.tcap + maps[128 + r]) * kKp;
            for (int n = lane; n < kKp; n += 32) kp[n] = stg[r * kKp + n];
        }
    }
    if (a.results) {
        for (int r = q; r < nrow; r += 4) {
            float* rec = a.results + ((size_t)maps[r] * a.tcap + maps[256 + r]) * MMW_RESULT_FLOATS;
            for (int n = lane; n < kKp; n += 32) rec[11 + n] = stg[r * kKp + n];
            if (lane == 0) {
                const double x0 = reinterpret_cast<const double*>(rec + 68)[0], x1 = reinterpret_cast<const double*>(rec + 68)[1];
                write_fade_square(a.fade, x0, x1, stg + r * kKp, rec);
            }
        }
    }
}

template <int BN, int STAGES>
constexpr int gemm_smem_bytes() { return STAGES * (2 * 128 * kBK * 2 + 2 * BN * kBK * 2) + 1024 + 256 + 3 * 128 * 4; }

template <int BN, int STAGES, int KS = 1>
__global__ void __launch_bounds__(kGemmThreads, 1)
gemm_tc_kernel(const __grid_constant__ CUtensorMap map_ah, const __grid_constant__ CUtensorMap map_al,
               const __grid_constant__ CUtensorMap map_wh, const __grid_constant__ CUtensorMap map_wl,
               const GemmTcArgs a) {
    constexpr int BM = 128, UK = 16;
    constexpr int A_BYTES = BM * kBK * 2, B_BYTES = BN * kBK * 2;
    constexpr int STAGE_BYTES = 2 * A_BYTES + 2 * B_BYTES;
    constexpr uint32_t TCOLS = BN <= 32 ? 32 : (BN <= 64 ? 64 : (BN <= 128 ? 128 : 256));
    const int rows = __ldcg(a.n_rows);
    const int m0 = blockIdx.y * BM;
    if (m0 >= rows) return;

    extern __shared__ unsigned char smem_raw[];
    unsigned char* smem = reinterpret_cast<unsigned char*>(((uintptr_t)smem_raw + 1023) & ~(uintptr_t)1023);
    uint64_t* full = reinterpret_cast<uint64_t*>(smem + STAGES * STAGE_BYTES);
    uint64_t* empty = full + STAGES;
    uint64_t* tmem_full = empty + STAGES;
    uint32_t* tmem_slot = reinterpret_cast<uint32_t*>(tmem_full + 1);
    const int warp = threadIdx.x >> 5, lane = threadIdx.x & 31;
    const int ks = KS > 1 ? (int)blockIdx.x : 0;
    const int nkb = a.K / kBK / KS, kb0 = ks * nkb;

    if (warp == 0 && lane == 0) {
        asm volatile("prefetch.tensormap [%0];" ::"l"(&map_ah) : "memory");
        asm volatile("prefetch.tensormap [%0];" ::"l"(&map_al) : "memory");
        asm volatile("prefetch.tensormap [%0];" ::"l"(&map_wh) : "memory");
        asm volatile("prefetch.tensormap [%0];" ::"l"(&map_wl) : "memory");
        for (int s = 0; s < STAGES; ++s) { mbar_init(&full[s], 1); mbar_init(&empty[s], 1); }
        mbar_init(tmem_full, 1);
        asm volatile("fence.mbarrier_init.release.cluster;" ::: "memory");
    }
    if (warp == 1) tmem_alloc<TCOLS>(tmem_slot);
    tc_fence_before();
    __syncthreads();
    tc_fence_after();
    const uint32_t tmem_d = *tmem_slot;
    pdl_wait();
    pdl_launch_dependents();

    if (warp == 0) {
        if (lane == 0) {
            for (int kb = 0; kb < nkb; ++kb) {
                const int s = kb % STAGES;
                const uint32_t ph = (kb / STAGES) & 1;
                mbar_wait(&empty[s], ph ^ 1);
                unsigned char* st = smem + s * STAGE_BYTES;
                if (a.dbg & 1) { mbar_arrive(&full[s]); continue; }
                mbar_expect_tx(&full[s], STAGE_BYTES);
                const int k0 = (kb0 + kb) * kBK;
                tma_load_2d(st, &map_ah, &full[s], k0, m0);
                tma_load_2d(st + A_BYTES, &map_al, &full[s], k0, m0);
                tma_load_2d(st + 2 * A_BYTES, &map_wh, &full[s], k0, 0);
                tma_load_2d(st + 2 * A_BYTES + B_BYTES, &map_wl, &full[s], k0, 0);
            }
        }
    } else if (warp == 1) {
        if (lane == 0) {
            const uint32_t idesc = make_idesc(BN);
            for (int kb = 0; kb < nkb; ++kb) {
                const int s = kb % STAGES;
                const uint32_t ph = (kb / STAGES) & 1;
                mbar_wait(&full[s], ph);
                tc_fence_after();
                const uint32_t st = smem_u32(smem + s * STAGE_BYTES);
                const uint64_t dah = make_desc<128>(st), dal = make_desc<128>(st + A_BYTES);
                const uint64_t dwh = make_desc<128>(st + 2 * A_BYTES), dwl = make_desc<128>(st + 2 * A_BYTES + B_BYTES);
#pragma unroll
                for (int kk = 0; kk < kBK / UK; ++kk) {
                    if (a.dbg & 2) break;
                    const uint64_t adv = (uint64_t)((kk * UK * 2) >> 4);
                    umma_bf16(tmem_d, dah + adv, dwh + adv, idesc, (kb | kk) != 0);
                    umma_bf16(tmem_d, dah + adv, dwl + adv, idesc, 1);
                    umma_bf16(tmem_d, dal + adv, dwh + adv, idesc, 1);
                }
                umma_commit(&empty[s]);
            }
            umma_commit(tmem_full);
        }
    } else if (KS > 1) {
    } else {
        const int q = warp & 3;
        int* maps = reinterpret_cast<int*>(tmem_slot + 2);
        gemm_load_row_maps(a, maps, m0, min(BM, rows - m0), threadIdx.x - 64);
        mbar_wait(tmem_full, 0);
        tc_fence_after();
        const int row = m0 + q * 32 + lane;
        float* stg = reinterpret_cast<float*>(smem);
#pragma unroll 1
        for (int c0 = 0; c0 < BN; c0 += 32) {
            uint32_t v[32];
            tmem_ld32(tmem_d + ((uint32_t)(q * 32) << 16) + (uint32_t)c0, v);
            if (row >= rows) continue;
#pragma unroll
            for (int j = 0; j < 32; ++j) {
                const int n = c0 + j;
                if (n < kKp) stg[(q * 32 + lane) * kKp + n] = __uint_as_float(v[j]) + __ldg(a.bias + n);
            }
        }
        asm volatile("bar.sync 1, 128;" ::: "memory");
        gemm_store_keypoints(a, stg, maps, m0, min(BM, rows - m0), q, lane, threadIdx.x - 64);
    }
    if (KS > 1) {
        static_assert(KS == 1 || (KS == 4 && BN == 64), "split epilogue: 4 CTAs, 4 row quadrants, 64 columns");
        static_assert(KS == 1 || 32768 + 4 * 8192 <= STAGES * STAGE_BYTES, "partials fit in the pipeline stages");
        const int q = warp & 3;
        const int row0 = m0 + 32 * ks, nrow = max(0, min(32, rows - row0));
        int* maps = reinterpret_cast<int*>(tmem_slot + 2);
        uint32_t v0[32], v1[32];
        if (warp >= 2) {
            gemm_load_row_maps(a, maps, row0, nrow, threadIdx.x - 64);
            mbar_wait(tmem_full, 0);
            tc_fence_after();
            tmem_ld32(tmem_d + ((uint32_t)(q * 32) << 16), v0);
            tmem_ld32(tmem_d + ((uint32_t)(q * 32) << 16) + 32u, v1);
            tc_fence_before();
        }
        cluster_sync_all();
        float* part = reinterpret_cast<float*>(smem + 32768);
        if (warp >= 2 && q != ks) {
            const uint32_t base = mapa_shared(smem_u32(part + (size_t)ks * 2048 + lane * 4), (uint32_t)q);
#pragma unroll
            for (int g = 0; g < 16; ++g) {
                const uint32_t* v = g < 8 ? v0 : v1;
                const int j = (g & 7) * 4;
                asm volatile("st.shared::cluster.v4.b32 [%0], {%1, %2, %3, %4};" ::"r"(base + (uint32_t)(g * 512)),
                             "r"(v[j]), "r"(v[j + 1]), "r"(v[j + 2]), "r"(v[j + 3])
                             : "memory");
            }
        }
        cluster_sync_all();
        if (warp >= 2) {
            float* stg = reinterpret_cast<float*>(smem);
            if (q == ks) {
                const float4* p4 = reinterpret_cast<const float4*>(part);
#pragma unroll
                for (int g = 0; g < 16; ++g) {
                    const uint32_t* v = g < 8 ? v0 : v1;
                    const int j = (g & 7) * 4;
                    float acc[4] = {0.f, 0.f, 0.f, 0.f};
#pragma unroll
                    for (int o = 0; o < KS; ++o) {
                        if (o == ks) {
                            acc[0] += __uint_as_float(v[j]); acc[1] += __uint_as_float(v[j + 1]);
                            acc[2] += __uint_as_float(v[j + 2]); acc[3] += __uint_as_float(v[j + 3]);
                        } else {
                            const float4 t = p4[(size_t)o * 512 + g * 32 + lane];
                            acc[0] += t.x; acc[1] += t.y; acc[2] += t.z; acc[3] += t.w;
                        }
                    }
#pragma unroll
                    for (int e = 0; e < 4; ++e) {
                        const int n = g * 4 + e;
                        if (n < kKp) stg[lane * kKp + n] = acc[e] + __ldg(a.bias + n);
                    }
                }
            }
            asm volatile("bar.sync 1, 128;" ::: "memory");
            gemm_store_keypoints(a, stg, maps, row0, nrow, q, lane, threadIdx.x - 64);
        }
    }
    tc_fence_before();
    __syncthreads();
    if (warp == 1) {
        tc_fence_after();
        tmem_dealloc<TCOLS>(tmem_d);
    }
}

__device__ __forceinline__ void tma_load_2d_pair(void* dst, const CUtensorMap* map, uint32_t bar_cluster, int c0, int c1) {
    asm volatile(
        "cp.async.bulk.tensor.2d.cta_group::2.shared::cluster.global.mbarrier::complete_tx::bytes [%0], [%1, {%3, %4}], "
        "[%2];" ::"r"(smem_u32(dst)),
        "l"(map), "r"(bar_cluster), "r"(c0), "r"(c1)
        : "memory");
}
__device__ __forceinline__ void umma_bf16_pair(uint32_t tmem_d, uint64_t adesc, uint64_t bdesc, uint32_t idesc,
                                               uint32_t accumulate) {
    asm volatile(
        "{\n\t"
        ".reg .pred p;\n\t"
        "setp.ne.b32 p, %4, 0;\n\t"
        "tcgen05.mma.cta_group::2.kind::f16 [%0], %1, %2, %3, p;\n\t"
        "}" ::"r"(tmem_d), "l"(adesc), "l"(bdesc), "r"(idesc), "r"(accumulate)
        : "memory");
}
__device__ __forceinline__ void umma_commit_pair(uint64_t* bar, uint16_t mask) {
    asm volatile("tcgen05.commit.cta_group::2.mbarrier::arrive::one.shared::cluster.multicast::cluster.b64 [%0], %1;" ::
                     "r"(smem_u32(bar)), "h"(mask)
                 : "memory");
}
template <uint32_t COLS>
__device__ __forceinline__ void tmem_alloc_pair(uint32_t* slot) {
    asm volatile("tcgen05.alloc.cta_group::2.sync.aligned.shared::cta.b32 [%0], %1;" ::"r"(smem_u32(slot)), "r"(COLS)
                 : "memory");
    asm volatile("tcgen05.relinquish_alloc_permit.cta_group::2.sync.aligned;" ::: "memory");
}
template <uint32_t COLS>
__device__ __forceinline__ void tmem_dealloc_pair(uint32_t addr) {
    asm volatile("tcgen05.dealloc.cta_group::2.sync.aligned.b32 %0, %1;" ::"r"(addr), "r"(COLS) : "memory");
}
__device__ __forceinline__ constexpr uint32_t make_idesc_pair(int n) {
    return (1u << 4) | (1u << 7) | (1u << 10) | ((uint32_t)(n >> 3) << 17) | ((uint32_t)(256 >> 4) << 24);
}

template <int BN, int STAGES>
constexpr int gemm_pair_smem_bytes() {
    return STAGES * (2 * 128 * kBK * 2 + 2 * (BN / 2) * kBK * 2) + 1024 + 256 + 3 * BN * 4;
}

template <int BN, int STAGES>
__global__ void __launch_bounds__(kGemmThreads, 1)
gemm_tc_pair_kernel(const __grid_constant__ CUtensorMap map_ah, const __grid_constant__ CUtensorMap map_al,
                    const __grid_constant__ CUtensorMap map_wh_half, const __grid_constant__ CUtensorMap map_wl_half,
                    const GemmTcArgs a) {
    constexpr int BM = 128, UK = 16;
    constexpr int A_BYTES = BM * kBK * 2, BH_BYTES = (BN / 2) * kBK * 2;
    constexpr int STAGE_BYTES = 2 * A_BYTES + 2 * BH_BYTES;
    constexpr uint32_t TCOLS = BN <= 32 ? 32 : (BN <= 64 ? 64 : (BN <= 128 ? 128 : 256));
    __shared__ unsigned long long ts[8];
    auto mark = [&](int i) {
        if (a.dbg & 4) { unsigned long long t; asm volatile("mov.u64 %0, %%globaltimer;" : "=l"(t)); ts[i] = t; }
    };
    if (threadIdx.x == 0) mark(0);
    const int rows = __ldcg(a.n_rows);
    if ((int)(blockIdx.x & ~1u) * BM >= rows) return;
    const int m0 = blockIdx.x * BM, n0 = blockIdx.y * BN;
    const uint32_t rank = cluster_ctarank();

    extern __shared__ unsigned char smem_raw[];
    unsigned char* smem = reinterpret_cast<unsigned char*>(((uintptr_t)smem_raw + 1023) & ~(uintptr_t)1023);
    uint64_t* full = reinterpret_cast<uint64_t*>(smem + STAGES * STAGE_BYTES);
    uint64_t* empty = full + STAGES;
    uint64_t* tmem_full = empty + STAGES;
    uint32_t* tmem_slot = reinterpret_cast<uint32_t*>(tmem_full + 1);
    const int warp = threadIdx.x >> 5, lane = threadIdx.x & 31;
    const int nkb = a.K / kBK;

    if (warp == 0 && lane == 0) {
        asm volatile("prefetch.tensormap [%0];" ::"l"(&map_ah) : "memory");
        asm volatile("prefetch.tensormap [%0];" ::"l"(&map_al) : "memory");
        asm volatile("prefetch.tensormap [%0];" ::"l"(&map_wh_half) : "memory");
        asm volatile("prefetch.tensormap [%0];" ::"l"(&map_wl_half) : "memory");
        for (int s = 0; s < STAGES; ++s) { mbar_init(&full[s], 1); mbar_init(&empty[s], 1); }
        mbar_init(tmem_full, 1);
        asm volatile("fence.mbarrier_init.release.cluster;" ::: "memory");
    }
    if (warp == 1) tmem_alloc_pair<TCOLS>(tmem_slot);
    tc_fence_before();
    __syncthreads();
    cluster_sync_all();
    tc_fence_after();
    const uint32_t tmem_d = *tmem_slot;
    pdl_wait();
    pdl_launch_dependents();
    if (threadIdx.x == 0) mark(1);

    if (warp == 0) {
        if (lane == 0) {
            for (int kb = 0; kb < nkb; ++kb) {
                const int s = kb % STAGES;
                const uint32_t ph = (kb / STAGES) & 1;
                mbar_wait(&empty[s], ph ^ 1);
                unsigned char* st = smem + s * STAGE_BYTES;
                const uint32_t bar = mapa_shared(smem_u32(&full[s]), 0);
                if (a.dbg & 1) {
                    if (rank == 0) mbar_arrive(&full[s]);
                    continue;
                }
                if (rank == 0) mbar_expect_tx(&full[s], 2 * STAGE_BYTES);
                tma_load_2d_pair(st, &map_ah, bar, kb * kBK, m0);
                tma_load_2d_pair(st + A_BYTES, &map_al, bar, kb * kBK, m0);
                tma_load_2d_pair(st + 2 * A_BYTES, &map_wh_half, bar, kb * kBK, n0 + (int)rank * (BN / 2));
                tma_load_2d_pair(st + 2 * A_BYTES + BH_BYTES, &map_wl_half, bar, kb * kBK, n0 + (int)rank * (BN / 2));
            }
            mark(2);
        }
    } else if (warp == 1) {
        if (lane == 0 && rank == 0) {
            constexpr uint32_t idesc = make_idesc_pair(BN);
            for (int kb = 0; kb < nkb; ++kb) {
                const int s = kb % STAGES;
                const uint32_t ph = (kb / STAGES) & 1;
                mbar_wait(&full[s], ph);
                tc_fence_after();
                const uint32_t st = smem_u32(smem + s * STAGE_BYTES);
                const uint64_t dah = make_desc<128>(st), dal = make_desc<128>(st + A_BYTES);
                const uint64_t dwh = make_desc<128>(st + 2 * A_BYTES), dwl = make_desc<128>(st + 2 * A_BYTES + BH_BYTES);
#pragma unroll
                for (int kk = 0; kk < kBK / UK; ++kk) {
                    if (a.dbg & 2) break;
                    const uint64_t adv = (uint64_t)((kk * UK * 2) >> 4);
                    umma_bf16_pair(tmem_d, dah + adv, dwh + adv, idesc, (kb | kk) != 0);
                    umma_bf16_pair(tmem_d, dah + adv, dwl + adv, idesc, 1);
                    umma_bf16_pair(tmem_d, dal + adv, dwh + adv, idesc, 1);
                }
                umma_commit_pair(&empty[s], (uint16_t)3);
            }
            umma_commit_pair(tmem_full, (uint16_t)3);
            mark(3);
        }
    } else {
        const int q = warp & 3;
        float* sconst = reinterpret_cast<float*>(tmem_slot + 2);
        const int ncols = min(BN, a.N - n0);
        for (int i = threadIdx.x - 64; i < ncols; i += 128) {
            sconst[i] = __ldg(a.bias + n0 + i);
            sconst[BN + i] = __ldg(a.bn_scale + n0 + i);
            sconst[2 * BN + i] = __ldg(a.bn_shift + n0 + i);
        }
        asm volatile("bar.sync 1, 128;" ::: "memory");
        mbar_wait(tmem_full, 0);
        tc_fence_after();
        if (threadIdx.x == 64) mark(4);
        const int row = m0 + q * 32 + lane;
#pragma unroll 1
        for (int c0 = 0; c0 < ncols; c0 += 32) {
            uint32_t v[32];
            tmem_ld32(tmem_d + ((uint32_t)(q * 32) << 16) + (uint32_t)c0, v);
            if (row >= rows) continue;
            const int nv4 = min(32, ncols - c0) >> 3;
            __align__(16) __nv_bfloat16 hi[32], lo[32];
#pragma unroll
            for (int j = 0; j < 32; ++j) {
                float x = fmaxf(__uint_as_float(v[j]) + sconst[c0 + j], 0.f);
                x = fmaf(x, sconst[BN + c0 + j], sconst[2 * BN + c0 + j]);
                split2(x, hi[j], lo[j]);
            }
            uint4* oh = reinterpret_cast<uint4*>(a.out_hi + (size_t)row * a.N + n0 + c0);
            uint4* ol = reinterpret_cast<uint4*>(a.out_lo + (size_t)row * a.N + n0 + c0);
#pragma unroll
            for (int i = 0; i < 4; ++i) {
                if (i < nv4) {
                    oh[i] = reinterpret_cast<const uint4*>(hi)[i];
                    ol[i] = reinterpret_cast<const uint4*>(lo)[i];
                }
            }
        }
    }
    if (threadIdx.x == 64) mark(5);
    tc_fence_before();
    __syncthreads();
    if (threadIdx.x == 0) mark(6);
    cluster_sync_all();
    if (warp == 1) {
        tc_fence_after();
        tmem_dealloc_pair<TCOLS>(tmem_d);
    }
    if ((a.dbg & 4) && threadIdx.x == 0 && (blockIdx.x < 2 || blockIdx.x == 15) && (blockIdx.y == 0 || blockIdx.y == 7)) {
        unsigned long long t;
        asm volatile("mov.u64 %0, %%globaltimer;" : "=l"(t));
        printf("[pair %d,%d] t0 %llu | prologue %llu | tma issued %llu | mma issued %llu | acc ready %llu | epilogue %llu | "
               "sync %llu | end %llu (ns since t0)\n", (int)blockIdx.x, (int)blockIdx.y, ts[0], ts[1] - ts[0],
               ts[2] - ts[0], ts[3] - ts[0], ts[4] - ts[0], ts[5] - ts[0], ts[6] - ts[0], t - ts[0]);
    }
}

__global__ void pack_input_kernel(const float* __restrict__ feats, __nv_bfloat16* __restrict__ out, const int* n_rows,
                                  int P) {
    const size_t total = (size_t)(*n_rows) * P;
    for (size_t i = (size_t)blockIdx.x * blockDim.x + threadIdx.x; i < total; i += (size_t)gridDim.x * blockDim.x) {
        __align__(16) __nv_bfloat16 v[16];
#pragma unroll
        for (int k = 0; k < 16; ++k) v[k] = __float2bfloat16_rn(0.f);
#pragma unroll
        for (int k = 0; k < 5; ++k) split2(feats[i * 5 + k], v[k], v[8 + k]);
        const size_t slice = i / 64;
        const int pos = (int)(i % 64), h = pos >> 3, w = pos & 7;
        uint4* o = reinterpret_cast<uint4*>(out) + ((slice * 8 + w) * 2) * 8 + h;
        o[0] = reinterpret_cast<const uint4*>(v)[0];
        o[8] = reinterpret_cast<const uint4*>(v)[1];
    }
}

struct TcImpl {
    int D = 0, taps = 0, Kf = 0, H = 0, rows_cap = 0, rows_pad = 0;
    __nv_bfloat16 *in_p = nullptr, *in_p2 = nullptr, *act1_p = nullptr;
    __nv_bfloat16 *a_hi = nullptr, *a_lo = nullptr;
    __nv_bfloat16 *h_hi = nullptr, *h_lo = nullptr;
    __nv_bfloat16 *w1b = nullptr, *w2b = nullptr;
    __nv_bfloat16 *wd1_hi = nullptr, *wd1_lo = nullptr, *wd2_hi = nullptr, *wd2_lo = nullptr;
    CUtensorMap m_w1b, m_w2b, m_ah, m_al, m_hh, m_hl, m_w2h, m_w2l;
    CUtensorMap m_w1h_half256, m_w1l_half256, m_w1h_half192, m_w1l_half192, m_w1h_half176, m_w1l_half176;
    int force_bn = 0;
    int pair_slots = 74;
    int dbg = 0;
};

static std::string g_tc_err;
const char* pose_tc_error() { return g_tc_err.c_str(); }

typedef CUresult (*EncodeTiledFn)(CUtensorMap*, CUtensorMapDataType, cuuint32_t, void*, const cuuint64_t*,
                                  const cuuint64_t*, const cuuint32_t*, const cuuint32_t*, CUtensorMapInterleave,
                                  CUtensorMapSwizzle, CUtensorMapL2promotion, CUtensorMapFloatOOBfill);

static EncodeTiledFn get_encode() {
    static EncodeTiledFn fn = nullptr;
    if (fn) return fn;
    void* p = nullptr;
    cudaDriverEntryPointQueryResult qres;
    if (cudaGetDriverEntryPoint("cuTensorMapEncodeTiled", &p, cudaEnableDefault, &qres) != cudaSuccess ||
        qres != cudaDriverEntryPointSuccess)
        return nullptr;
    fn = reinterpret_cast<EncodeTiledFn>(p);
    return fn;
}

static CUtensorMapSwizzle swz(int bytes) {
    return bytes == 128 ? CU_TENSOR_MAP_SWIZZLE_128B : (bytes == 64 ? CU_TENSOR_MAP_SWIZZLE_64B : CU_TENSOR_MAP_SWIZZLE_32B);
}

static int make_map_2d(CUtensorMap* m, void* base, uint64_t rows, uint64_t K, uint32_t box_rows, uint32_t box_k) {
    EncodeTiledFn enc = get_encode();
    if (!enc) { g_tc_err = "cuTensorMapEncodeTiled not available"; return -1; }
    cuuint64_t dims[2] = {K, rows};
    cuuint64_t strides[1] = {K * 2};
    cuuint32_t box[2] = {box_k, box_rows};
    cuuint32_t estr[2] = {1, 1};
    CUresult r = enc(m, CU_TENSOR_MAP_DATA_TYPE_BFLOAT16, 2, base, dims, strides, box, estr, CU_TENSOR_MAP_INTERLEAVE_NONE,
                     swz((int)box_k * 2), CU_TENSOR_MAP_L2_PROMOTION_L2_256B, CU_TENSOR_MAP_FLOAT_OOB_FILL_NONE);
    if (r != CUDA_SUCCESS) { g_tc_err = "cuTensorMapEncodeTiled(2d) failed (" + std::to_string((int)r) + ")"; return -1; }
    return 0;
}

static inline uint16_t f2bf(float f) {
    uint32_t u;
    std::memcpy(&u, &f, 4);
    if ((u & 0x7fffffffu) > 0x7f800000u) return (uint16_t)((u >> 16) | 0x40);
    u += 0x7fffu + ((u >> 16) & 1u);
    return (uint16_t)(u >> 16);
}
static inline float bf2f(uint16_t h) {
    uint32_t u = (uint32_t)h << 16;
    float f;
    std::memcpy(&f, &u, 4);
    return f;
}

template <class T>
static bool dev_alloc(T** p, size_t bytes, bool zero = false) {
    if (cudaMalloc((void**)p, bytes) != cudaSuccess) return false;
    if (zero) cudaMemset(*p, 0, bytes);
    return true;
}
static bool upload(__nv_bfloat16** d, const std::vector<uint16_t>& h) {
    if (!dev_alloc(d, h.size() * 2)) return false;
    return cudaMemcpy(*d, h.data(), h.size() * 2, cudaMemcpyHostToDevice) == cudaSuccess;
}

static std::vector<uint16_t> conv_b(const float* w, int taps, int cin, int cinp, int cout) {
    const int CK = 2 * cinp, NO = 2 * cout;
    std::vector<uint16_t> b((size_t)taps * NO * CK, 0);
    for (int t = 0; t < taps; ++t)
        for (int n = 0; n < NO; ++n)
            for (int k = 0; k < CK; ++k) {
                const int ci = k % cinp, co = n % cout;
                if (ci >= cin) continue;
                const float wv = w[((size_t)t * cin + ci) * cout + co];
                const uint16_t hi = f2bf(wv), lo = f2bf(wv - bf2f(hi));
                uint16_t v = 0;
                if (n < cout) v = hi;
                else if (k < cinp) v = lo;
                b[((size_t)t * NO + n) * CK + k] = v;
            }
    return b;
}

static std::vector<uint16_t> conv_b2(const float* w, int taps, int cin, int cout) {
    std::vector<uint16_t> b((size_t)taps * 3 * cout * cin, 0);
    for (int t = 0; t < taps; ++t)
        for (int r = 0; r < 3 * cout; ++r)
            for (int ci = 0; ci < cin; ++ci) {
                const int co = r % cout;
                const float wv = w[((size_t)t * cin + ci) * cout + co];
                const uint16_t hi = f2bf(wv), lo = f2bf(wv - bf2f(hi));
                b[((size_t)t * 3 * cout + r) * cin + ci] = (r >= cout && r < 2 * cout) ? lo : hi;
            }
    return b;
}

static void dense_b(const float* w, int K, int N, int Npad, std::vector<uint16_t>& hi, std::vector<uint16_t>& lo) {
    hi.assign((size_t)Npad * K, 0);
    lo.assign((size_t)Npad * K, 0);
    for (int k = 0; k < K; ++k)
        for (int n = 0; n < N; ++n) {
            const float wv = w[(size_t)k * N + n];
            const uint16_t h = f2bf(wv);
            hi[(size_t)n * K + k] = h;
            lo[(size_t)n * K + k] = f2bf(wv - bf2f(h));
        }
}

int pose_tc_init(PoseTc* t, const float* blob, const size_t* off, int D, int rows_cap) {
    pose_tc_free(t);
    TcImpl* im = new TcImpl();
    t->impl = im;
    im->D = D; im->taps = D == 3 ? 27 : 9; im->Kf = D * 64 * 32; im->H = D * 512; im->rows_cap = rows_cap;
    im->rows_pad = (rows_cap + 127) / 128 * 128;
    t->D = D; t->K = im->Kf; t->H = im->H; t->rows_cap = rows_cap;
    const size_t R = im->rows_pad, P = (size_t)D * 64;
    bool ok = dev_alloc(&im->in_p, R * P * 16 * 2, true) && dev_alloc(&im->in_p2, R * P * 16 * 2, true) &&
              dev_alloc(&im->act1_p, R * P * 32 * 2, true) &&
              dev_alloc(&im->a_hi, R * im->Kf * 2, true) && dev_alloc(&im->a_lo, R * im->Kf * 2, true) &&
              dev_alloc(&im->h_hi, R * im->H * 2, true) && dev_alloc(&im->h_lo, R * im->H * 2, true);
    { const char* env = getenv("MMW_GEMM_DBG"); im->dbg = env ? atoi(env) : 0; }
    if (!ok) { g_tc_err = "cudaMalloc failed (activations)"; return -1; }
    std::vector<uint16_t> hi, lo;
    ok = upload(&im->w1b, conv_b(blob + off[0], im->taps, 5, 8, 16)) &&
         upload(&im->w2b, conv_b2(blob + off[2], im->taps, 16, 32));
    dense_b(blob + off[8], im->Kf, im->H, im->H, hi, lo);
    ok = ok && upload(&im->wd1_hi, hi) && upload(&im->wd1_lo, lo);
    dense_b(blob + off[14], im->H, kKp, 64, hi, lo);
    ok = ok && upload(&im->wd2_hi, hi) && upload(&im->wd2_lo, lo);
    if (!ok) { g_tc_err = "cudaMalloc/cudaMemcpy failed (weights)"; return -1; }
    if (make_map_2d(&im->m_w1b, im->w1b, (uint64_t)im->taps * 32, 16, 32, 16) ||
        make_map_2d(&im->m_w2b, im->w2b, (uint64_t)im->taps * 96, 16, 96, 16) ||
        make_map_2d(&im->m_ah, im->a_hi, R, im->Kf, 128, 64) || make_map_2d(&im->m_al, im->a_lo, R, im->Kf, 128, 64) ||
        make_map_2d(&im->m_w1h_half256, im->wd1_hi, im->H, im->Kf, 128, 64) ||
        make_map_2d(&im->m_w1l_half256, im->wd1_lo, im->H, im->Kf, 128, 64) ||
        make_map_2d(&im->m_hh, im->h_hi, R, im->H, 128, 64) || make_map_2d(&im->m_hl, im->h_lo, R, im->H, 128, 64) ||
        make_map_2d(&im->m_w2h, im->wd2_hi, 64, im->H, 64, 64) || make_map_2d(&im->m_w2l, im->wd2_lo, 64, im->H, 64, 64))
        return -1;
    cudaError_t e = cudaSuccess;
    auto set_smem = [&](const void* fn, int bytes) {
        if (e == cudaSuccess) e = cudaFuncSetAttribute(fn, cudaFuncAttributeMaxDynamicSharedMemorySize, bytes);
        if (e == cudaSuccess)
            e = cudaFuncSetAttribute(fn, cudaFuncAttributePreferredSharedMemoryCarveout, cudaSharedmemCarveoutMaxShared);
    };
    set_smem((const void*)conv_slab_kernel<16, 32, 0, 3>, conv_smem_bytes_tc<16, 32>(27));
    set_smem((const void*)conv_slab_kernel<32, 64, 1, 3>, conv_smem_bytes_tc<32, 64>(27));
    set_smem((const void*)conv_slab_kernel<16, 32, 0, 1>, conv_smem_bytes_tc<16, 32>(9));
    set_smem((const void*)conv_slab_kernel<32, 64, 1, 1>, conv_smem_bytes_tc<32, 64>(9));
    set_smem((const void*)gemm_tc_kernel<64, 4>, gemm_smem_bytes<64, 4>());
    set_smem((const void*)gemm_tc_kernel<64, 4, 4>, gemm_smem_bytes<64, 4>());
    if (e != cudaSuccess) { g_tc_err = std::string("cudaFuncSetAttribute: ") + cudaGetErrorString(e); return -1; }
    auto pair_fits = [&](const void* fn, int bytes, int bn) -> bool {
        set_smem(fn, bytes);
        int n = 0;
        if (e == cudaSuccess) {
            cudaLaunchConfig_t cfg{};
            cfg.gridDim = dim3(2, 8);
            cfg.blockDim = dim3(kGemmThreads);
            cfg.dynamicSmemBytes = bytes;
            cudaLaunchAttribute at[1];
            at[0].id = cudaLaunchAttributeClusterDimension;
            at[0].val.clusterDim.x = 2; at[0].val.clusterDim.y = 1; at[0].val.clusterDim.z = 1;
            cfg.attrs = at; cfg.numAttrs = 1;
            e = cudaOccupancyMaxActiveClusters(&n, fn, &cfg);
        }
        const std::string name = "gemm_tc_pair_kernel<" + std::to_string(bn) + ",3>";
        if (e != cudaSuccess) {
            (void)cudaGetLastError();
            g_tc_err = name + ": " + cudaGetErrorString(e);
            return false;
        }
        if (n < 1) {
            g_tc_err = name + ": a cluster of two CTAs with " + std::to_string(bytes) +
                       " bytes of shared memory each cannot be scheduled on this device";
            return false;
        }
        return true;
    };
    if (!pair_fits((const void*)gemm_tc_pair_kernel<256, 3>, gemm_pair_smem_bytes<256, 3>(), 256)) return -1;
    if (im->H % 192 == 0) {
        if (!pair_fits((const void*)gemm_tc_pair_kernel<192, 3>, gemm_pair_smem_bytes<192, 3>(), 192) ||
            !pair_fits((const void*)gemm_tc_pair_kernel<176, 3>, gemm_pair_smem_bytes<176, 3>(), 176))
            return -1;
        if (make_map_2d(&im->m_w1h_half192, im->wd1_hi, im->H, im->Kf, 96, 64) ||
            make_map_2d(&im->m_w1l_half192, im->wd1_lo, im->H, im->Kf, 96, 64) ||
            make_map_2d(&im->m_w1h_half176, im->wd1_hi, im->H, im->Kf, 88, 64) ||
            make_map_2d(&im->m_w1l_half176, im->wd1_lo, im->H, im->Kf, 88, 64))
            return -1;
    }
    {
        int dev = 0, sms = 148;
        cudaGetDevice(&dev);
        cudaDeviceGetAttribute(&sms, cudaDevAttrMultiProcessorCount, dev);
        im->pair_slots = sms / 2;
    }
    { const char* benv = getenv("MMW_FC1_BN"); im->force_bn = benv ? atoi(benv) : 0; }
    t->ready = true;
    return 0;
}

__nv_bfloat16* pose_tc_input(PoseTc* t, int buf) {
    TcImpl* im = reinterpret_cast<TcImpl*>(t->impl);
    return im ? (buf ? im->in_p2 : im->in_p) : nullptr;
}

static int check_launch(const char* what) {
    cudaError_t e = cudaGetLastError();
    if (e != cudaSuccess) { g_tc_err = std::string(what) + ": " + cudaGetErrorString(e); return -1; }
    return 0;
}

int pose_tc_pack_input(PoseTc* t, const float* feats, const int* n_rows, cudaStream_t st) {
    TcImpl* im = reinterpret_cast<TcImpl*>(t->impl);
    if (!im || !t->ready) { g_tc_err = "tensor-core path not initialised"; return -1; }
    pack_input_kernel<<<148 * 4, 256, 0, st>>>(feats, im->in_p, n_rows, im->D * 64);
    return check_launch("pack_input_kernel");
}

int pose_tc_conv(PoseTc* t, const PoseTcRun& r, cudaStream_t st, int* n_launches, int buf) {
    TcImpl* im = reinterpret_cast<TcImpl*>(t->impl);
    if (!im || !t->ready) { g_tc_err = "tensor-core path not initialised"; return -1; }
    ConvTcArgs c1{r.n_rows, r.b1, nullptr, nullptr, buf ? im->in_p2 : im->in_p, im->act1_p, nullptr, im->dbg};
    const dim3 one(1, 1, 1);
    cudaError_t le;
    if (im->D == 3)
        le = launch_pdl(conv_slab_kernel<16, 32, 0, 3>, dim3(148), dim3(kSlabThreads), conv_smem_bytes_tc<16, 32>(27), st, one,
                        im->m_w1b, c1);
    else
        le = launch_pdl(conv_slab_kernel<16, 32, 0, 1>, dim3(148), dim3(kSlabThreads), conv_smem_bytes_tc<16, 32>(9), st, one,
                        im->m_w1b, c1);
    if (le != cudaSuccess) { g_tc_err = std::string("conv_slab_kernel<conv1>: ") + cudaGetErrorString(le); return -1; }
    ConvTcArgs c2{r.n_rows, r.b2, r.bn1_scale, r.bn1_shift, im->act1_p, im->a_hi, im->a_lo, im->dbg};
    if (im->D == 3)
        le = launch_pdl(conv_slab_kernel<32, 64, 1, 3>, dim3(148), dim3(kSlabThreads), conv_smem_bytes_tc<32, 64>(27), st, one,
                        im->m_w2b, c2);
    else
        le = launch_pdl(conv_slab_kernel<32, 64, 1, 1>, dim3(148), dim3(kSlabThreads), conv_smem_bytes_tc<32, 64>(9), st, one,
                        im->m_w2b, c2);
    if (le != cudaSuccess) { g_tc_err = std::string("conv_slab_kernel<conv2>: ") + cudaGetErrorString(le); return -1; }
    if (n_launches) *n_launches = 2;
    return 0;
}

int pose_tc_fc1(PoseTc* t, const PoseTcRun& r, int max_rows, cudaStream_t st, int* n_launches, int rows_hint) {
    TcImpl* im = reinterpret_cast<TcImpl*>(t->impl);
    if (!im || !t->ready) { g_tc_err = "tensor-core path not initialised"; return -1; }
    GemmTcArgs g{r.n_rows, r.bd1, r.bn2_scale, r.bn2_shift, im->h_hi, im->h_lo, nullptr, nullptr, nullptr, nullptr,
                 im->Kf, im->H, r.tcap, im->dbg};
    int bn = 256;
    if (im->H % 192 == 0) {
        bn = 192;
        if (rows_hint > 0) {
            const int mt = (rows_hint + 48 + 255) / 256, P = im->pair_slots;
            auto cost = [&](int w) { return ((mt * ((im->H + w - 1) / w) + P - 1) / P) * w; };
            int best = cost(192);
            if (cost(256) < best) { best = cost(256); bn = 256; }
            if (cost(176) < best) bn = 176;
        }
        if (im->force_bn == 176 || im->force_bn == 192 || im->force_bn == 256) bn = im->force_bn;
    }
    const dim3 grid((((max_rows + 127) / 128) + 1) & ~1, (im->H + bn - 1) / bn), blk(kGemmThreads), cl(2, 1, 1);
    cudaError_t le;
    if (bn == 176)
        le = launch_pdl(gemm_tc_pair_kernel<176, 3>, grid, blk, gemm_pair_smem_bytes<176, 3>(), st, cl, im->m_ah, im->m_al,
                        im->m_w1h_half176, im->m_w1l_half176, g);
    else if (bn == 192)
        le = launch_pdl(gemm_tc_pair_kernel<192, 3>, grid, blk, gemm_pair_smem_bytes<192, 3>(), st, cl, im->m_ah, im->m_al,
                        im->m_w1h_half192, im->m_w1l_half192, g);
    else
        le = launch_pdl(gemm_tc_pair_kernel<256, 3>, grid, blk, gemm_pair_smem_bytes<256, 3>(), st, cl, im->m_ah, im->m_al,
                        im->m_w1h_half256, im->m_w1l_half256, g);
    if (le != cudaSuccess) { g_tc_err = std::string("dense 1 launch: ") + cudaGetErrorString(le); return -1; }
    if (n_launches) *n_launches = 1;
    return 0;
}

int pose_tc_fc2(PoseTc* t, const PoseTcRun& r, int max_rows, cudaStream_t st, int* n_launches) {
    TcImpl* im = reinterpret_cast<TcImpl*>(t->impl);
    if (!im || !t->ready) { g_tc_err = "tensor-core path not initialised"; return -1; }
    GemmTcArgs g{r.n_rows, r.bd2, nullptr, nullptr, nullptr, nullptr, r.out, r.keypoints, r.row_scene, r.row_slot,
                 im->H, 64, r.tcap, im->dbg, r.results, r.row_track, r.fade};
    cudaError_t le;
    if ((im->H / kBK) % 4 == 0 && (max_rows + 127) / 128 <= 128)
        le = launch_pdl(gemm_tc_kernel<64, 4, 4>, dim3(4, (max_rows + 127) / 128), dim3(kGemmThreads),
                        gemm_smem_bytes<64, 4>(), st, dim3(4, 1, 1), im->m_hh, im->m_hl, im->m_w2h, im->m_w2l, g);
    else
        le = launch_pdl(gemm_tc_kernel<64, 4>, dim3(1, (max_rows + 127) / 128), dim3(kGemmThreads),
                        gemm_smem_bytes<64, 4>(), st, dim3(1, 1, 1), im->m_hh, im->m_hl, im->m_w2h, im->m_w2l, g);
    if (le != cudaSuccess) { g_tc_err = std::string("dense 2 launch: ") + cudaGetErrorString(le); return -1; }
    if (n_launches) *n_launches = 1;
    return 0;
}

int pose_tc_intermediate(PoseTc* t, int layer, int n, uint16_t* out) {
    TcImpl* im = reinterpret_cast<TcImpl*>(t->impl);
    if (!im || !t->ready) { g_tc_err = "tensor-core path not initialised"; return -1; }
    const size_t P = (size_t)im->D * 64, rows = (size_t)n;
    const size_t per = layer == 0 ? P * 5 : layer == 1 ? P * 16 : layer == 2 ? (size_t)im->Kf : (size_t)im->H;
    uint16_t* lo_out = out + rows * per;
    if (layer >= 2) {
        const __nv_bfloat16* src[2] = {layer == 2 ? im->a_hi : im->h_hi, layer == 2 ? im->a_lo : im->h_lo};
        for (int p = 0; p < 2; ++p)
            if (cudaMemcpy(p ? lo_out : out, src[p], rows * per * 2, cudaMemcpyDeviceToHost) != cudaSuccess) {
                g_tc_err = "cudaMemcpy (intermediate)";
                return -1;
            }
        return 0;
    }
    const int nch = layer == 0 ? 2 : 4, cout = layer == 0 ? 5 : 16;
    std::vector<uint16_t> h(rows * P * nch * 8);
    if (cudaMemcpy(h.data(), layer == 0 ? im->in_p : im->act1_p, h.size() * 2, cudaMemcpyDeviceToHost) != cudaSuccess) {
        g_tc_err = "cudaMemcpy (intermediate)";
        return -1;
    }
    for (size_t r = 0; r < rows; ++r)
        for (size_t pos = 0; pos < P; ++pos) {
            const size_t d = pos / 64, hh = (pos / 8) % 8, w = pos % 8;
            const size_t base = ((r * im->D + d) * 8 + w) * nch;
            for (int c = 0; c < cout; ++c) {
                const int chunk_hi = c / 8, chunk_lo = nch / 2 + c / 8;
                const size_t o = (r * P + pos) * cout + c;
                out[o] = h[((base + chunk_hi) * 8 + hh) * 8 + c % 8];
                lo_out[o] = h[((base + chunk_lo) * 8 + hh) * 8 + c % 8];
            }
        }
    return 0;
}

void pose_tc_free(PoseTc* t) {
    TcImpl* im = reinterpret_cast<TcImpl*>(t->impl);
    if (im) {
        for (void* p : {(void*)im->in_p, (void*)im->in_p2, (void*)im->act1_p, (void*)im->a_hi, (void*)im->a_lo, (void*)im->h_hi,
                        (void*)im->h_lo, (void*)im->w1b, (void*)im->w2b, (void*)im->wd1_hi, (void*)im->wd1_lo,
                        (void*)im->wd2_hi, (void*)im->wd2_lo})
            if (p) cudaFree(p);
        delete im;
    }
    t->impl = nullptr;
    t->ready = false;
}

}
```

### mmwave_msc_b200/csrc/pose_tc.cuh

```cuda
#pragma once
#include <cuda_bf16.h>

#include "pose.cuh"

namespace mmw {

struct PoseTc {
    bool ready = false;
    int D = 0, K = 0, H = 0, rows_cap = 0;
    void* impl = nullptr;
};

struct PoseTcRun {
    const int* n_rows;
    const float *b1, *b2, *bn1_scale, *bn1_shift, *bd1, *bn2_scale, *bn2_shift, *bd2;
    float* out;
    float* keypoints;
    const int32_t *row_scene, *row_slot;
    int tcap;
    float* results = nullptr;
    const int32_t* row_track = nullptr;
    FadeCfg fade = {0, 0, 0, 0, 0, 0};
};

int pose_tc_init(PoseTc* tc, const float* host_blob, const size_t* off, int D, int rows_cap);
__nv_bfloat16* pose_tc_input(PoseTc* tc, int buf = 0);
int pose_tc_pack_input(PoseTc* tc, const float* feats, const int* n_rows, cudaStream_t st);
int pose_tc_conv(PoseTc* tc, const PoseTcRun& r, cudaStream_t st, int* n_launches, int buf = 0);
int pose_tc_fc1(PoseTc* tc, const PoseTcRun& r, int max_rows, cudaStream_t st, int* n_launches, int rows_hint = 0);
int pose_tc_fc2(PoseTc* tc, const PoseTcRun& r, int max_rows, cudaStream_t st, int* n_launches);
int pose_tc_intermediate(PoseTc* tc, int layer, int n, uint16_t* out);
void pose_tc_free(PoseTc* tc);
const char* pose_tc_error();

}
```

### mmwave_msc_b200/csrc/step_kernel.cu

```cuda
#include "dbscan.cuh"
#include "linalg.cuh"
#include "mmw_internal.cuh"
#include "pose_feat.cuh"

namespace mmw {

constexpr int kTile = 2 * kStepThreads;
constexpr int kChunks = kTile / 32;
constexpr int kLw = 7;
constexpr int kBw = 72;
constexpr int kGp = 0, kHx = kGp + 21, kNest = 28, kMin = 29, kMax = 35, kSum = 41, kSumX = 47, kProd = 48;
static_assert(kProd + 21 <= kBw, "B holds the statistics totals next to the gate form");
static_assert(kStepThreads == 128, "the element-parallel track phases are written for 128 threads per scene");

struct SmemLayout {
    int sensor, tracks, B, A, KK, stage, hist, hnew, misc, total;
};
constexpr int kMiscInts = 192;
enum { kT1 = 2, kFreed = 3, kFlag = 4, kCntK = 8 , kCntU = 16 , kBaseG = 24 ,
       kBaseU = 88 , kOrder = 92 , kCntG = 124  };
static_assert(kCntG + 64 <= kMiscInts, "misc layout");

__host__ __device__ inline SmemLayout make_layout(int ncap, int tcap) {
    SmemLayout L;
// ... 699 lines not shown
            const unsigned lo = reinterpret_cast<const unsigned*>(hnew)[2 * tid], hi = reinterpret_cast<const unsigned*>(hnew)[2 * tid + 1];
            const unsigned c0 = min(lo & 0xffffu, 255u), c1 = min(lo >> 16, 255u), c2 = min(hi & 0xffffu, 255u),
                           c3 = min(hi >> 16, 255u);
            wd = c0 | (c1 << 8) | (c2 << 16) | (c3 << 24);
        } else {
            wd = misc[kFlag] ? 1u : 0u;
        }
        reinterpret_cast<unsigned*>(hist + uphys * kHistBytes)[tid] = wd;
        reinterpret_cast<unsigned*>(a.ring_hist + ((size_t)s * kRing + uphys) * kHistBytes)[tid] = wd;
    }
    __syncthreads();
    PHASE_MARK(8);

    if (warp == 0) {
        bool kp = false;
        unsigned slotbit = 0u;
        if (lane < T0) {
            const double lim = tr[lane].is_static ? c.life_sta : c.life_dyn;
            kp = !(tr[lane].lifetime > lim);
            if (!kp) slotbit = 1u << tr[lane].slot;
        }
        const unsigned kmask = __ballot_sync(kFull, kp);
        const unsigned freed = __reduce_or_sync(kFull, slotbit);
        if (kp) misc[kOrder + __popc(kmask & ltmask)] = lane;
        if (lane == 0) { misc[kT1] = __popc(kmask); misc[kFreed] = (int)freed; }
    }
    __syncthreads();
    const int T1 = misc[kT1];
    sc.slot_mask &= ~(unsigned)misc[kFreed];
    PHASE_MARK(9);

    for (int k = 0; k < T1; ++k) {
        if (tid < 36) {
            const int j = misc[kOrder + k];
            const TrackRec& t = tr[j];
            const double Nn = (double)t.point_num;
            const double coef = div_zero_fast(t.n_est - Nn, (t.n_est - 1.0) * Nn);
            double rm = 0.0;
            if (el.i6 == el.a6) { const double h = t.spread[el.i6] / 2; rm = (h * h) / Nn; }
            const double rc = rm + coef * t.G[tid];
            double* b = Bm + j * kBw;
            b[36 + tid] = rc;
            b[tid] = t.P[el.i6 * 9 + el.a6] + rc;
        }
    }
    __syncthreads();
    for (int k0 = 0; k0 < T1; k0 += 2 * kStepWarps) {
        const int k = k0 + 2 * warp + (lane >> 4);
        const bool live = k < T1;
        if (__ballot_sync(kFull, live) == 0u) continue;
        const int j = live ? misc[kOrder + k] : 0;
        double r[6];
        (void)inv6_spd_half(live ? Bm + j * kBw : nullptr, lane, r);
        __syncwarp();
        const int cl16 = lane & 15;
        if (live && cl16 >= 6 && cl16 < 12) {
#pragma unroll
            for (int i = 0; i < 6; ++i) Bm[j * kBw + i * 6 + (cl16 - 6)] = r[i];
        }
    }
    __syncthreads();
    for (int k = 0; k < T1; ++k) {
        const int j = misc[kOrder + k];
        if (tid < 54) KKm[j * 108 + tid] = kf_update_K_elem(tr[j].P, Bm + j * kBw, el);
    }
    __syncthreads();
    for (int k = 0; k < T1; ++k) {
        const int j = misc[kOrder + k];
        TrackRec& t = tr[j];
        const double* K = KKm + j * 108;
        double mv = 0.0, rv = 0.0, xv = 0.0;
        if (tid < 81) mv = kf_update_M1_elem(t.P, K, el);
        if (tid < 54) rv = kf_update_KR_elem(K, Bm + j * kBw + 36, el);
        if (tid >= 96 && tid < 105) xv = kf_update_x(t.x, t.centroid, K, tid - 96);
        __syncwarp();
        if (tid < 81) Am[j * 81 + tid] = mv;
        if (tid < 54) KKm[j * 108 + 54 + tid] = rv;
        if (tid >= 96 && tid < 105) t.x[tid - 96] = xv;
    }
    __syncthreads();
    for (int k = 0; k < T1; ++k) {
        const int j = misc[kOrder + k];
        TrackRec& t = tr[j];
        if (tid < 81) t.P[tid] = kf_update_P_elem(Am + j * 81, KKm + j * 108, KKm + j * 108 + 54, el);
        if (tid == 96) kf_update_nudge(t.x, t.centroid, t.lifetime == 0.0, c.nudge_thres, c.nudge_gain);
    }
    PHASE_MARK(10);

    int Bf = 0;
    int fphys[kRing];
    bool fl = false;
    for (int f = 0; f < kRing; ++f) {
        fphys[f] = ring_wrap(sc.ring_head + f, c.ring_size);
        if (f < sc.ring_n) {
            Bf += sc.ring_cnt[fphys[f]];
            fl = fl || hist[fphys[f] * kHistBytes + kGridCells] != 0;
        }
    }
    const bool run_db = Bf > 0 && T1 < c.tr_max_tracks;
    if (run_db) {
        bool maybe = Bf >= c.db_min_samples;
        if (maybe && c.grid_ok && !fl) {
            for (int cell = tid; cell < kGridCells; cell += kStepThreads) {
                int n = 0;
                for (int f = 0; f < kRing; ++f)
                    if (f < sc.ring_n) n += hist[fphys[f] * kHistBytes + cell];
                hnew[cell] = (uint16_t)n;
            }
            __syncthreads();
            maybe = grid_screen_may_have_core(hnew, c.db_min_samples);
        }
        if (maybe) {
            if (tid == 0) a.defer_list[atomicAdd(a.defer_count, 1)] = s;
        } else if (a.labels_out != nullptr) {
            for (int b = tid; b < Bf; b += kStepThreads) a.labels_out[(size_t)s * 3 * ncap + b] = -1;
        }
        sc.dbscan_n = Bf;
    }
    __syncthreads();
    PHASE_MARK(11);

    pdl_launch_dependents();
    {
        double* dstbase = reinterpret_cast<double*>(a.tracks + (size_t)s * tcap);
        for (int i = tid; i < T1 * kTrackWords; i += kStepThreads) {
            const int k = i / kTrackWords, wd = i - k * kTrackWords;
            dstbase[i] = reinterpret_cast<const double*>(tr + misc[kOrder + k])[wd];
        }
    }
    if (tid == 0) {
        sc.n_tracks = T1;
        a.scenes[s] = sc;
        a.pose_cnt[s] = T1;
        int4* st4 = reinterpret_cast<int4*>(a.scene_stats + (size_t)s * 8);
        st4[0] = make_int4(N, M, U, run_db ? Bf : 0);
        st4[1] = make_int4(T1, ring_rows, 1, 0);
    }
    PHASE_MARK(12);
    if (dbg_clocks && threadIdx.x == 0) {
        a.phase_cycles[16 + blockIdx.x] = (unsigned long long)(clock64() - kernel_t0);
        unsigned long long ns;
        asm volatile("mov.u64 %0, %%globaltimer;" : "=l"(ns));
        a.phase_cycles[16 + 2 * gridDim.x + blockIdx.x] = ns;
    }
}

constexpr int kBigThreads = 512;
constexpr int kBitsMaxB = 768;
__host__ __device__ inline int big_bits_cap(int ncap) { return 3 * ncap < kBitsMaxB ? 3 * ncap : kBitsMaxB; }
constexpr int kBigWsWords = 4 + kMaxCompMasks;
__host__ __device__ inline int big_adj_offset(int ncap) { return 36 * ncap + 2 * 3 * ncap * 4 + 64 * 4; }
__host__ __device__ inline int big_w6_offset(int ncap) {
    const int cap = big_bits_cap(ncap), w = (cap + 31) / 32;
    const int o = 36 * ncap + 2 * 3 * ncap * 4 + 64 * 4 + (cap * w + (1 + kBigWsWords) * w) * 4 + cap * kRawCols * 4;
    return (o + 7) & ~7;
}
__global__ void __launch_bounds__(kBigThreads, 1) dbscan_big_kernel(const __grid_constant__ StepArgs a) {
    extern __shared__ __align__(16) unsigned char smem[];
    const DevConfig& c = a.cfg;
    const int ncap = c.ncap, tcap = c.tcap;
    float* Xf = reinterpret_cast<float*>(smem);
    int* par = reinterpret_cast<int*>(smem + 36 * ncap);
    int* cl = par + 3 * ncap;
    int* scan = cl + 3 * ncap;
    const int bits_cap = big_bits_cap(ncap), bits_w = (bits_cap + 31) >> 5;
    unsigned* adj = reinterpret_cast<unsigned*>(scan + 64);
    unsigned* cm = adj + (size_t)bits_cap * bits_w;
    unsigned* bws = cm + bits_w;
    float* rawc = reinterpret_cast<float*>(bws + kBigWsWords * bits_w);
    double* w6 = reinterpret_cast<double*>(smem + big_w6_offset(ncap));
    const int tid = threadIdx.x, lane = tid & 31, warp = tid >> 5;
    pdl_wait();
    pdl_launch_dependents();
    const int n_defer = *a.defer_count;
    unsigned long long* dbg = a.phase_cycles != nullptr ? a.phase_cycles + 16 + 3 * a.n_scenes : nullptr;
    long long dbg_t = clock64();
    auto stamp = [&](int k) {
        if (dbg != nullptr && tid == 0) {
            const long long now = clock64();
            atomicAdd(&dbg[k], (unsigned long long)(now - dbg_t));
            dbg_t = now;
        }
    };
    __shared__ SensorRec s_sr;
    for (int it = blockIdx.x; it < n_defer; it += gridDim.x) {
        const int s = a.defer_list[it];
        SceneRec sc = a.scenes[s];
        if (tid < (int)(sizeof(SensorRec) / 8))
            reinterpret_cast<double*>(&s_sr)[tid] = reinterpret_cast<const double*>(a.sensors + s)[tid];
        __syncthreads();
        const int T1 = sc.n_tracks;
        int B = 0;
        int fcnt[kRing], fphys[kRing];
        for (int f = 0; f < kRing; ++f) {
            fphys[f] = ring_wrap(sc.ring_head + f, c.ring_size);
            fcnt[f] = f < sc.ring_n ? sc.ring_cnt[fphys[f]] : 0;
            B += fcnt[f];
        }
        const bool bits = B <= bits_cap;
        NbScreened nb = load_fused_ring(a, s_sr, s, fcnt, fphys, Xf, 3 * ncap, bits ? rawc : nullptr);
        stamp(0);
        int ncl = bits ? dbscan_bits_block(nb, B, c.db_min_samples, adj, cm, bws, par, cl, dbg != nullptr ? dbg - 10 : nullptr)
                       : dbscan_block(nb, B, c.db_min_samples, par, cl, scan, dbg != nullptr ? dbg - 10 : nullptr, false,
                                      true);
        if (dbg != nullptr && tid == 0) dbg_t = clock64();
        if (a.labels_out != nullptr)
            for (int b = tid; b < B; b += kBigThreads) a.labels_out[(size_t)s * 3 * ncap + b] = cl[b];
        if (ncl > 0) {
            if (T1 + ncl > tcap) { ncl = tcap - T1; sc.flags |= MMW_SCENE_TRACK_OVERFLOW; }
            int newslot[kMaxTcap];
            {
                const unsigned capmask = tcap >= 32 ? 0xffffffffu : ((1u << tcap) - 1u);
                unsigned fs = ~sc.slot_mask & capmask;
                for (int q = 0; q < ncl; ++q) {
                    newslot[q] = __ffs(fs) - 1; fs &= fs - 1;
                    sc.slot_mask |= 1u << newslot[q];
                }
            }
            if (bits) {
                for (int b = tid; b < B; b += kBigThreads)
                    if (cl[b] >= 0) {
                        const float* r = rawc + (size_t)b * kRawCols;
                        double w[6];
                        world_from_raw(s_sr, r[0], r[1], r[2], r[3], w);
#pragma unroll
                        for (int k = 0; k < 6; ++k) w6[(size_t)b * 6 + k] = w[k];
                    }
                __syncthreads();
            }
            if (bits) {
                double* red = reinterpret_cast<double*>(adj);
                for (int q = 0; q < ncl; ++q)
                    spawn_track_block(a, s, a.tracks[(size_t)s * tcap + T1 + q], q, newslot[q], sc.next_id + q, cl, B, rawc,
                                      w6, red);
            } else {
                for (int q = warp; q < ncl; q += kBigThreads / 32)
                    spawn_track(a, s_sr, s, a.tracks[(size_t)s * tcap + T1 + q], q, newslot[q], sc.next_id + q, cl, fcnt,
                                fphys, lane, nullptr, nullptr);
            }
            if (a.nr_extra != nullptr) {
                __shared__ int s_part[kBigThreads / 32], s_row0;
                __syncthreads();
                int part = 0;
                for (int i = tid; i < a.n_scenes; i += kBigThreads) part += a.pose_cnt[i];
                part = __reduce_add_sync(kFullMask, part);
                if (lane == 0) s_part[warp] = part;
                __syncthreads();
                if (tid == 0) {
                    int r0 = 0;
                    for (int w = 0; w < kBigThreads / 32; ++w) r0 += s_part[w];
                    s_row0 = r0 + atomicAdd(a.nr_extra, ncl);
                }
                __syncthreads();
                const int nfr = c.ring_size;
                unsigned char* scratch = smem + ((big_adj_offset(ncap) + 15) & ~15) + warp * kFeatItemBytes;
                long long* fkeys = reinterpret_cast<long long*>(scratch);
                float* fso = reinterpret_cast<float*>(scratch + kFeatPts * 8);
                uint4* fsp = reinterpret_cast<uint4*>(scratch + kFeatPts * 8 + kFeatPts * kRawCols * 4);
                for (int item = warp; item < ncl * nfr; item += kBigThreads / 32) {
                    const int q = item / nfr, f = item - q * nfr, row = s_row0 + q, slot = newslot[q];
                    const TrackRec* t = a.tracks + (size_t)s * tcap + T1 + q;
                    if (f == 0 && lane == 0) {
                        a.nr_row_scene[row] = s; a.nr_row_track[row] = T1 + q; a.nr_row_slot[row] = slot;
                    }
                    const float* src = f == 0 ? a.track_ring + ((size_t)s * tcap + slot) * kRing * (kFeatPts * kRawCols) : nullptr;
                    const int cnt = f == 0 ? __ldcg(&t->ring_cnt[0]) : 0;
                    float* out = a.nr_feats + ((size_t)row * nfr + f) * (kFeatPts * kRawCols);
                    uint4* pk = a.nr_packed != nullptr
                                    ? reinterpret_cast<uint4*>(static_cast<unsigned char*>(a.nr_packed) + (size_t)row * nfr * kFeatPts * 32)
                                    : nullptr;
                    pose_feature_item<false>(c, s_sr, src, cnt, __ldcg(&t->centroid[0]), __ldcg(&t->centroid[1]), f, out, pk,
                                             fkeys, fso, fsp, lane, 0);
                }
            }
            sc.next_id += ncl;
            sc.n_tracks = T1 + ncl;
            sc.ring_n = 0;
            sc.ring_head = 0;
            sc.ring_cnt[0] = sc.ring_cnt[1] = sc.ring_cnt[2] = 0;
            sc.ring_ph_gone = 1;
            if (tid == 0) atomicAdd(&a.counters[5], (unsigned long long)ncl);
        }
        __syncthreads();
        if (tid == 0) { a.scenes[s] = sc; if (a.nr_extra == nullptr) a.pose_cnt[s] = sc.n_tracks; }
        __syncthreads();
        stamp(1);
        if (dbg != nullptr && tid == 0) { atomicAdd(&dbg[2], 1ull); atomicAdd(&dbg[7], (unsigned long long)B); }
    }
    if (blockIdx.x == gridDim.x - 1 && a.scene_stats != nullptr) {
        unsigned long long acc[7] = {0, 0, 0, 0, 0, 0, 0};
        for (int sidx = tid; sidx < a.n_scenes; sidx += kBigThreads) {
            const int4 s0 = reinterpret_cast<const int4*>(a.scene_stats)[2 * sidx];
            const int4 s1 = reinterpret_cast<const int4*>(a.scene_stats)[2 * sidx + 1];
            acc[0] += (unsigned)s1.z; acc[1] += (unsigned)s0.x; acc[2] += (unsigned)s0.y; acc[3] += (unsigned)s0.z;
            acc[4] += (unsigned)s0.w; acc[5] += (unsigned)s1.x; acc[6] += (unsigned)s1.y;
        }
#pragma unroll
        for (int k = 0; k < 7; ++k) {
            unsigned v = (unsigned)acc[k];
            v = __reduce_add_sync(kFullMask, v);
            if (lane == 0 && v) atomicAdd(&a.counters[k], (unsigned long long)v);
        }
    }
    __syncthreads();
    if (tid == 0) {
        __threadfence();
        if (atomicAdd(a.defer_done, 1) == (int)gridDim.x - 1) {
            if (a.defer_hint != nullptr) *a.defer_hint = n_defer;
            *a.defer_count = 0;
            *a.defer_done = 0;
        }
    }
}

int dbscan_big_smem_bytes(int ncap) {
    const int a = big_w6_offset(ncap) + big_bits_cap(ncap) * 6 * 8;
    const int b = ((big_adj_offset(ncap) + 15) & ~15) + (kBigThreads / 32) * kFeatItemBytes;
    return a > b ? a : b;
}

cudaError_t launch_step(const StepArgs& a, cudaStream_t stream) {
    const int smem = step_smem_bytes(a.cfg.ncap, a.cfg.tcap);
    static int configured[kMaxDevices] = {0};
    cudaError_t e = ensure_smem_attr(reinterpret_cast<const void*>(step_kernel), configured, smem);
    if (e != cudaSuccess) return e;
    step_kernel<<<a.n_scenes, kStepThreads, smem, stream>>>(a);
    return cudaGetLastError();
}

cudaError_t launch_dbscan_big(const StepArgs& a, cudaStream_t stream, int grid) {
    if (a.defer_count == nullptr) return cudaSuccess;
    const int big_smem = dbscan_big_smem_bytes(a.cfg.ncap);
    static int configured[kMaxDevices] = {0};
    cudaError_t e = ensure_smem_attr(reinterpret_cast<const void*>(dbscan_big_kernel), configured, big_smem);
    if (e != cudaSuccess) return e;
    return launch_pdl(dbscan_big_kernel, dim3(grid < 16 ? 16 : (grid > 148 ? 148 : grid)), dim3(kBigThreads), big_smem, stream,
                      dim3(1, 1, 1), a);
}

}
```

Measured before the change: 4.261 million.

## Let conv kernel start on early pose rows via epoch flags and dynamic row claiming

Replaces the PDL wait in the late pose path with epoch-tagged release/acquire flags. The feature kernel publishes a partial row count, and the last DBSCAN block publishes the final total. The tensor-core conv kernel now claims rows dynamically through an atomic scheduler and passes row indices to its MMA and epilogue warps through an mbarrier index ring, so it can process known rows before the total is ready. This aims to overlap the pose network with the tail of clustering, at the cost of spin-waiting, extra atomics and more complex inter-kernel synchronisation.

```diff
diff --git a/mmwave_msc_b200/csrc/mmw_api.cu b/mmwave_msc_b200/csrc/mmw_api.cu
--- a/mmwave_msc_b200/csrc/mmw_api.cu
+++ b/mmwave_msc_b200/csrc/mmw_api.cu
@@ -80,7 +80,8 @@
     cudaEvent_t feat_done[2] = {nullptr, nullptr}, packt_done[2] = {nullptr, nullptr}, pose_done[2] = {nullptr, nullptr};
     int32_t *d_row_scene2 = nullptr, *d_row_track2 = nullptr, *d_row_slot2 = nullptr;
     int* d_pose_total2 = nullptr;
-    int32_t* d_pose_extra = nullptr;
+    int32_t* d_late = nullptr;
+    unsigned late_epoch = 0;
     int rows_buf = 0;
     unsigned pipe_idx = 0;
     int pipe_r = -1;
@@ -235,7 +236,7 @@
                     x->d_results[0], x->d_results[1], x->d_blob, x->d_bn1s,
                     x->d_bn1t, x->d_bn2s, x->d_bn2t, x->d_feats, x->d_row_scene, x->d_row_track, x->d_row_slot,
                     x->d_pose_total, x->d_act2, x->d_act3, x->d_pose_out, x->d_row_scene2, x->d_row_track2, x->d_row_slot2,
-                    x->d_pose_total2, x->d_pose_extra};
+                    x->d_pose_total2, x->d_late};
     for (void* p : ptrs)
         if (p) cudaFree(p);
     pose_tc_free(&x->tc);
@@ -269,7 +270,7 @@
     CK(cudaMemsetAsync(x->d_assoc, 0xff, sizeof(int32_t) * (size_t)x->S * x->ncap, x->stream));
     CK(cudaMemsetAsync(x->d_pose_total, 0, sizeof(int), x->stream));
     CK(cudaMemsetAsync(x->d_pose_total2, 0, sizeof(int), x->stream));
-    CK(cudaMemsetAsync(x->d_pose_extra, 0, 2 * sizeof(int32_t), x->stream));
+    CK(cudaMemsetAsync(x->d_late, 0, 5 * sizeof(int32_t), x->stream));
     CK(cudaMemsetAsync(x->d_defer, 0, sizeof(int32_t) * (2 + 2 * (size_t)x->S), x->stream));
     CK(cudaMemsetAsync(x->d_scene_stats, 0, sizeof(int32_t) * 8 * (size_t)x->S, x->stream));
     CK(cudaMemsetAsync(x->d_ring_hist, 0, (size_t)kRing * kHistBytes * x->S, x->stream));
@@ -436,7 +437,7 @@
         return fail(MMW_ERR_CUDA, "cudaStreamCreate failed");
     }
     ALLOC(x->d_pose_total, sizeof(int));
-    ALLOC(x->d_pose_extra, 2 * sizeof(int32_t));
+    ALLOC(x->d_late, 5 * sizeof(int32_t));
     x->pose_cap = n_scenes * max_tracks;
     ALLOC(x->d_row_scene, sizeof(int32_t) * x->pose_cap);
     ALLOC(x->d_row_track, sizeof(int32_t) * x->pose_cap);
@@ -634,11 +635,17 @@
     return MMW_OK;
 }
 
-static int run_pose_net(mmw_ctx* x, float* keypoints_by_slot, int max_rows) {
+static int run_pose_net(mmw_ctx* x, float* keypoints_by_slot, int max_rows, bool late = false) {
     x->last_pose_run = x->use_tc && x->tc.ready ? 1 : 2;
     if (x->use_tc && x->tc.ready) {
         PoseTcRun r{x->d_pose_total, x->b1, x->b2, x->d_bn1s, x->d_bn1t, x->bd1, x->d_bn2s, x->d_bn2t, x->bd2,
                     x->d_pose_out, keypoints_by_slot, x->d_row_scene, x->d_row_slot, x->tcap};
+        if (late) {
+            r.rows_r0 = x->d_late + 1;
+            r.rows_ready = reinterpret_cast<const unsigned*>(x->d_late + 2);
+            r.feat_ready = reinterpret_cast<const unsigned*>(x->d_late + 4);
+            r.epoch = x->late_epoch;
+        }
         return run_pose_tc(x, r, max_rows, 0, x->stream);
     }
     ConvArgs ca{x->d_feats, x->w1, x->b1, x->w2, x->b2, x->d_bn1s, x->d_bn1t, x->d_act2, x->d_pose_total};
@@ -676,7 +683,12 @@
                     b ? x->d_row_track2 : x->d_row_track, b ? x->d_row_slot2 : x->d_row_slot,
                     x->fold_pose_index ? x->d_defer + 1 + x->S : nullptr, pose_total, x->d_counters, x->S};
     fa.rows_hint = x->d_rows_hint;
-    fa.late_extra = late ? x->d_pose_extra + b : nullptr;
+    if (late) {
+        fa.late_r0 = x->d_late + 1;
+        fa.late_done = x->d_late + 3;
+        fa.late_ready = reinterpret_cast<unsigned*>(x->d_late + 4);
+        fa.epoch = x->late_epoch;
+    }
     x->rows_buf = b;
     prof_mark(x, MMW_K_POSE_FEATURES);
     CK(launch_pose_features(fa, x->S, st));
@@ -789,7 +801,12 @@
         a.nr_row_scene = x->d_row_scene;
         a.nr_row_track = x->d_row_track;
         a.nr_row_slot = x->d_row_slot;
-        a.nr_extra = x->d_pose_extra;
+        a.nr_extra = x->d_late;
+        a.nr_total = x->d_pose_total;
+        a.nr_rows_hint = x->d_rows_hint;
+        a.nr_ready = reinterpret_cast<unsigned*>(x->d_late + 2);
+        if (++x->late_epoch == 0) ++x->late_epoch;
+        a.nr_epoch = x->late_epoch;
     }
     if (pipelined) {
         if (x->pipe_idx >= 2) CK(cudaStreamWaitEvent(x->stream, x->pose_done[x->pipe_idx & 1u], 0));
@@ -817,7 +834,7 @@
     CK(join_pose(x));
     const int rc = launch_feature_stage(x, 0, late, x->stream);
     if (rc != MMW_OK) return rc;
-    return run_pose_net(x, x->d_keypoints, x->pose_cap);
+    return run_pose_net(x, x->d_keypoints, x->pose_cap, late);
 }
 
 int mmw_pose_features_only(mmw_ctx* x) {
diff --git a/mmwave_msc_b200/csrc/mmw_internal.cuh b/mmwave_msc_b200/csrc/mmw_internal.cuh
--- a/mmwave_msc_b200/csrc/mmw_internal.cuh
+++ b/mmwave_msc_b200/csrc/mmw_internal.cuh
@@ -113,6 +113,10 @@
     void* nr_packed = nullptr;
     int32_t *nr_row_scene = nullptr, *nr_row_track = nullptr, *nr_row_slot = nullptr;
     int32_t* nr_extra = nullptr;
+    int* nr_total = nullptr;
+    int* nr_rows_hint = nullptr;
+    unsigned* nr_ready = nullptr;
+    unsigned nr_epoch = 0;
     long long pts_row0 = 0;
 };
 
diff --git a/mmwave_msc_b200/csrc/pose.cuh b/mmwave_msc_b200/csrc/pose.cuh
--- a/mmwave_msc_b200/csrc/pose.cuh
+++ b/mmwave_msc_b200/csrc/pose.cuh
@@ -21,7 +21,10 @@
     unsigned long long* counters;
     int n_scenes;
     int dbg = 0;
-    const int32_t* late_extra = nullptr;
+    int* late_r0 = nullptr;
+    int* late_done = nullptr;
+    unsigned* late_ready = nullptr;
+    unsigned epoch = 0;
     int* rows_hint = nullptr;
 };
 
diff --git a/mmwave_msc_b200/csrc/pose_kernels.cu b/mmwave_msc_b200/csrc/pose_kernels.cu
--- a/mmwave_msc_b200/csrc/pose_kernels.cu
+++ b/mmwave_msc_b200/csrc/pose_kernels.cu
@@ -50,7 +50,7 @@
     __shared__ __align__(16) uint4 spk[kFeatWarps][kFeatPts * 2];
     const int s = blockIdx.x;
     const int lane = threadIdx.x & 31, warp = threadIdx.x >> 5;
-    const bool late = a.late_extra != nullptr && a.pose_cnt != nullptr;
+    const bool late = a.late_r0 != nullptr && a.pose_cnt != nullptr;
     if (!late) pdl_wait();
     pdl_launch_dependents();
     SceneRec sc;
@@ -103,14 +103,25 @@
                                 spk[warp], lane, a.dbg);
     }
     if (a.pose_cnt != nullptr && !(a.dbg & 1) && s == a.n_scenes - 1 && threadIdx.x == 0) {
-        int total = pose_base + n_tr;
+        const int total = pose_base + n_tr;
         if (late) {
-            pdl_wait();
-            total += __ldcg(a.late_extra);
-        }
-        *a.pose_total = total;
-        if (a.rows_hint != nullptr) *a.rows_hint = total;
-        atomicAdd(&a.counters[7], (unsigned long long)total);
+            *a.late_r0 = total;
+        } else {
+            *a.pose_total = total;
+            if (a.rows_hint != nullptr) *a.rows_hint = total;
+            atomicAdd(&a.counters[7], (unsigned long long)total);
+        }
+    }
+    if (late) {
+        __syncthreads();
+        if (threadIdx.x == 0) {
+            __threadfence();
+            if (atomicAdd(a.late_done, 1) == (int)gridDim.x - 1) {
+                __threadfence();
+                *a.late_done = 0;
+                asm volatile("st.release.gpu.global.u32 [%0], %1;" ::"l"(a.late_ready), "r"(a.epoch) : "memory");
+            }
+        }
     }
 }
 
diff --git a/mmwave_msc_b200/csrc/pose_tc.cu b/mmwave_msc_b200/csrc/pose_tc.cu
--- a/mmwave_msc_b200/csrc/pose_tc.cu
+++ b/mmwave_msc_b200/csrc/pose_tc.cu
@@ -104,6 +104,11 @@
     __nv_bfloat16* out0;
     __nv_bfloat16* out1;
     int dbg;
+    int* sched;
+    const int* rows_r0 = nullptr;
+    const unsigned* rows_ready = nullptr;
+    const unsigned* feat_ready = nullptr;
+    unsigned epoch = 0;
 };
 
 constexpr int kSlabThreads = 320;
@@ -118,6 +123,14 @@
 constexpr int conv_smem_bytes_tc(int taps) {
     return taps * conv_b_tap_bytes<CK, NOUT>() + slab_ring<CK>() * kSlabAtoms * (CK / 8) * 128 + 1024 + 1024;
 }
+constexpr int kSlabIdx = 4;
+
+__device__ __forceinline__ unsigned ld_acquire_gpu(const unsigned* p) {
+    unsigned v;
+    asm volatile("ld.acquire.gpu.global.u32 %0, [%1];" : "=r"(v) : "l"(p) : "memory");
+    return v;
+}
+__device__ __forceinline__ void producer_sync() { asm volatile("bar.sync 1, 128;" ::: "memory"); }
 
 __device__ __forceinline__ uint64_t make_desc_interleaved(uint32_t saddr, uint32_t lbo, uint32_t sbo) {
     uint64_t d = 0;
@@ -153,7 +166,12 @@
     uint64_t* tfull = sempty + NSLAB;
     uint64_t* tempty = tfull + 2;
     uint64_t* bfull = tempty + 2;
-    uint32_t* tmem_slot = reinterpret_cast<uint32_t*>(bfull + 1);
+    uint64_t* ifull = bfull + 1;
+    uint64_t* iempty = ifull + kSlabIdx;
+    int2* sidx = reinterpret_cast<int2*>(iempty + kSlabIdx);
+    int* sclaim = reinterpret_cast<int*>(sidx + kSlabIdx);
+    int* stotal = sclaim + 2;
+    uint32_t* tmem_slot = reinterpret_cast<uint32_t*>(stotal + 2);
     float* sconst = reinterpret_cast<float*>(tmem_slot + 2);
 
     const int warp = threadIdx.x >> 5, lane = threadIdx.x & 31;
@@ -171,6 +189,7 @@
         for (int c = 0; c < NSLAB; ++c) { mbar_init(&sfull[c], 128); mbar_init(&sempty[c], MT); }
         for (int b = 0; b < 2; ++b) { mbar_init(&tfull[b], MT); mbar_init(&tempty[b], 4); }
         mbar_init(bfull, 1);
+        for (int k = 0; k < kSlabIdx; ++k) { mbar_init(&ifull[k], 1); mbar_init(&iempty[k], 2 + 4); }
         asm volatile("fence.mbarrier_init.release.cluster;" ::: "memory");
         mbar_expect_tx(bfull, taps * B_TAP);
         for (int t = 0; t < taps; ++t) tma_load_2d(sB + t * B_TAP, &map_b, bfull, 0, t * B_ROWS);
@@ -180,12 +199,38 @@
     __syncthreads();
     tc_fence_after();
     const uint32_t tmem_base = *tmem_slot;
-    pdl_wait();
+    const bool late = a.rows_ready != nullptr;
+    if (!late) pdl_wait();
     pdl_launch_dependents();
-    const int n_samples = *a.n_rows;
-    const int rows = TRIPLE ? (n_samples + 2) / 3 : n_samples;
-
+
+    constexpr int SPS = TRIPLE ? 3 : 1;
     if (warp < 4) {
+        auto wait_flag = [&](const unsigned* flag, const int* word, int k) {
+            if (threadIdx.x == 0) {
+                unsigned ns = 32;
+                while (ld_acquire_gpu(flag) != a.epoch) {
+                    __nanosleep(ns);
+                    ns = ns < 256 ? 2 * ns : 256;
+                }
+                stotal[k] = __ldcg(word);
+            }
+            producer_sync();
+            return stotal[k];
+        };
+        const int r0 = late ? wait_flag(a.feat_ready, a.rows_r0, 0) : *a.n_rows;
+        int total = late ? -1 : r0;
+        auto samples = [&](int i) -> int {
+            if ((i + 1) * SPS <= r0) return SPS;
+            if (total < 0) return -1;
+            return min(max(total - i * SPS, 0), SPS);
+        };
+        auto wait_total = [&]() { total = wait_flag(a.rows_ready, a.n_rows, 1); };
+        auto publish = [&](int n, int slab, int cnt) {
+            const int k = n % kSlabIdx;
+            mbar_wait(&iempty[k], (uint32_t)(((n / kSlabIdx) & 1) ^ 1));
+            sidx[k] = make_int2(slab, cnt);
+            mbar_arrive(&ifull[k]);
+        };
         constexpr int ITEMS = D * 64 * NCH / 128;
         const int tid = threadIdx.x;
         int dstoff[ITEMS];
@@ -197,19 +242,37 @@
             dstoff[j] = (1 + (d + 1) * 10 + (w + 1)) * ATOM + chunk * 128;
         }
         uint4 cur[ITEMS], nxt[ITEMS];
-        auto load_row = [&](int row, uint4 (&r)[ITEMS]) {
+        auto load_row = [&](int row, int cnt, uint4 (&r)[ITEMS]) {
+            if (a.dbg & 8) return;
             const uint4* src = reinterpret_cast<const uint4*>(a.in) + (size_t)row * (D * 64 * NCH);
 #pragma unroll
             for (int j = 0; j < ITEMS; ++j) {
-                const bool there = !TRIPLE || row * 3 + (tid + 128 * j) / (64 * NCH) < n_samples;
-                r[j] = there ? __ldg(src + tid + 128 * j) : make_uint4(0, 0, 0, 0);
+                const bool there = !TRIPLE || (tid + 128 * j) / (64 * NCH) < cnt;
+                r[j] = there ? __ldcg(src + tid + 128 * j) : make_uint4(0, 0, 0, 0);
             }
         };
-        if ((int)blockIdx.x < rows && !(a.dbg & 8)) load_row(blockIdx.x, cur);
+        int claim = 0, nclaims = 0;
+        auto share_claim = [&]() -> int {
+            const int k = nclaims++ & 1;
+            if (tid == 0) sclaim[k] = claim;
+            producer_sync();
+            return sclaim[k];
+        };
+        if (tid == 0) claim = (int)gridDim.x + atomicAdd(a.sched, 1);
+        int cnt = samples(blockIdx.x);
+        if (cnt < 0) { wait_total(); cnt = samples(blockIdx.x); }
+        if (tid == 0) publish(0, blockIdx.x, cnt);
+        load_row(blockIdx.x, cnt, cur);
+        int nrow = 0, ncnt = 0;
+        if (cnt > 0) {
+            nrow = share_claim();
+            ncnt = samples(nrow);
+            if (tid == 0 && ncnt >= 0) publish(1, nrow, ncnt);
+        }
         int u = 0;
-        for (int row = blockIdx.x; row < rows; row += gridDim.x) {
-            const int next = row + gridDim.x;
-            if (next < rows && !(a.dbg & 8)) load_row(next, nxt);
+        for (int n = 0; cnt > 0; ++n) {
+            if (ncnt > 0) load_row(nrow, ncnt, nxt);
+            if (tid == 0 && ncnt != 0) claim = (int)gridDim.x + atomicAdd(a.sched, 1);
 #pragma unroll
             for (int c = 0; c < 3; ++c, ++u) {
                 const int slot = u % NSLAB;
@@ -229,8 +292,27 @@
                 asm volatile("fence.proxy.async.shared::cta;" ::: "memory");
                 mbar_arrive(&sfull[slot]);
             }
+            if (ncnt < 0) {
+                wait_total();
+                ncnt = samples(nrow);
+                if (tid == 0) publish(n + 1, nrow, ncnt);
+                if (ncnt > 0) load_row(nrow, ncnt, nxt);
+            }
+            if (ncnt == 0) break;
+            const int c2 = share_claim();
+            const int c2cnt = samples(c2);
+            if (tid == 0 && c2cnt >= 0) publish(n + 2, c2, c2cnt);
 #pragma unroll
             for (int j = 0; j < ITEMS; ++j) cur[j] = nxt[j];
+            cnt = ncnt;
+            nrow = c2; ncnt = c2cnt;
+        }
+        if (tid == 0) {
+            __threadfence();
+            if (atomicAdd(a.sched + 1, 1) == (int)gridDim.x - 1) {
+                a.sched[0] = 0;
+                a.sched[1] = 0;
+            }
         }
     } else if (warp == 4 || warp == 5) {
         const int mt = warp - 4;
@@ -240,8 +322,12 @@
             const uint64_t db0 = make_desc<32>(smem_u32(sB));
             const uint64_t da00 = make_desc_interleaved(smem_u32(slab) + (uint32_t)((1 + mt * 16) * ATOM), 128, ATOM);
             mbar_wait(bfull, 0);
-            int n = 0, u = 0;
-            for (int row = blockIdx.x; row < rows; row += gridDim.x, ++n) {
+            int u = 0;
+            for (int n = 0;; ++n) {
+                mbar_wait(&ifull[n % kSlabIdx], (uint32_t)((n / kSlabIdx) & 1));
+                const int cnt = sidx[n % kSlabIdx].y;
+                mbar_arrive(&iempty[n % kSlabIdx]);
+                if (cnt == 0) break;
                 const int buf = n & 1;
                 mbar_wait(&tempty[buf], (uint32_t)(((n >> 1) & 1) ^ 1));
                 tc_fence_after();
@@ -274,8 +360,13 @@
         }
     } else {
         const int q = warp & 3;
-        int n = 0;
-        for (int row = blockIdx.x; row < rows; row += gridDim.x, ++n) {
+        for (int n = 0;; ++n) {
+            mbar_wait(&ifull[n % kSlabIdx], (uint32_t)((n / kSlabIdx) & 1));
+            const int2 e = sidx[n % kSlabIdx];
+            __syncwarp();
+            if (lane == 0) mbar_arrive(&iempty[n % kSlabIdx]);
+            if (e.y == 0) break;
+            const int row = e.x;
             const int buf = n & 1;
             mbar_wait(&tfull[buf], (uint32_t)((n >> 1) & 1));
             tc_fence_after();
@@ -305,7 +396,7 @@
                 const int aidx = mt * 16 + (m >> 3), hh = m & 7;
                 const int d = aidx / 10, w2 = aidx % 10;
                 if (d >= D || w2 < 1 || w2 > 8 || (a.dbg & 32)) continue;
-                if (TRIPLE && row * 3 + d >= n_samples) continue;
+                if (TRIPLE && d >= e.y) continue;
                 __align__(16) __nv_bfloat16 hi[COUT], lo[COUT];
 #pragma unroll
                 for (int c = 0; c < COUT; ++c) {
@@ -786,6 +877,7 @@
     __nv_bfloat16 *h_hi = nullptr, *h_lo = nullptr;
     __nv_bfloat16 *w1b = nullptr, *w2b = nullptr;
     __nv_bfloat16 *wd1_hi = nullptr, *wd1_lo = nullptr, *wd2_hi = nullptr, *wd2_lo = nullptr;
+    int* sched = nullptr;
     CUtensorMap m_w1b, m_w2b, m_ah, m_al, m_hh, m_hl, m_w2h, m_w2l;
     CUtensorMap m_w1h_half256, m_w1l_half256, m_w1h_half192, m_w1l_half192, m_w1h_half176, m_w1l_half176;
     int force_bn = 0;
@@ -908,7 +1000,8 @@
     bool ok = dev_alloc(&im->in_p, R * P * 16 * 2, true) && dev_alloc(&im->in_p2, R * P * 16 * 2, true) &&
               dev_alloc(&im->act1_p, R * P * 32 * 2, true) &&
               dev_alloc(&im->a_hi, R * im->Kf * 2, true) && dev_alloc(&im->a_lo, R * im->Kf * 2, true) &&
-              dev_alloc(&im->h_hi, R * im->H * 2, true) && dev_alloc(&im->h_lo, R * im->H * 2, true);
+              dev_alloc(&im->h_hi, R * im->H * 2, true) && dev_alloc(&im->h_lo, R * im->H * 2, true) &&
+              dev_alloc(&im->sched, 2 * 2 * 2 * sizeof(int), true);
     { const char* env = getenv("MMW_GEMM_DBG"); im->dbg = env ? atoi(env) : 0; }
     if (!ok) { g_tc_err = "cudaMalloc failed (activations)"; return -1; }
     std::vector<uint16_t> hi, lo;
@@ -1010,7 +1103,9 @@
 int pose_tc_conv(PoseTc* t, const PoseTcRun& r, cudaStream_t st, int* n_launches, int buf) {
     TcImpl* im = reinterpret_cast<TcImpl*>(t->impl);
     if (!im || !t->ready) { g_tc_err = "tensor-core path not initialised"; return -1; }
-    ConvTcArgs c1{r.n_rows, r.b1, nullptr, nullptr, buf ? im->in_p2 : im->in_p, im->act1_p, nullptr, im->dbg};
+    int* sched = im->sched + (buf ? 4 : 0);
+    ConvTcArgs c1{r.n_rows, r.b1, nullptr, nullptr, buf ? im->in_p2 : im->in_p, im->act1_p, nullptr, im->dbg, sched,
+                  r.rows_r0, r.rows_ready, r.feat_ready, r.epoch};
     const dim3 one(1, 1, 1);
     cudaError_t le;
     if (im->D == 3)
@@ -1020,7 +1115,7 @@
         le = launch_pdl(conv_slab_kernel<16, 32, 0, 1>, dim3(148), dim3(kSlabThreads), conv_smem_bytes_tc<16, 32>(9), st, one,
                         im->m_w1b, c1);
     if (le != cudaSuccess) { g_tc_err = std::string("conv_slab_kernel<conv1>: ") + cudaGetErrorString(le); return -1; }
-    ConvTcArgs c2{r.n_rows, r.b2, r.bn1_scale, r.bn1_shift, im->act1_p, im->a_hi, im->a_lo, im->dbg};
+    ConvTcArgs c2{r.n_rows, r.b2, r.bn1_scale, r.bn1_shift, im->act1_p, im->a_hi, im->a_lo, im->dbg, sched + 2};
     if (im->D == 3)
         le = launch_pdl(conv_slab_kernel<32, 64, 1, 3>, dim3(148), dim3(kSlabThreads), conv_smem_bytes_tc<32, 64>(27), st, one,
                         im->m_w2b, c2);
@@ -1121,7 +1216,7 @@
     TcImpl* im = reinterpret_cast<TcImpl*>(t->impl);
     if (im) {
         for (void* p : {(void*)im->in_p, (void*)im->in_p2, (void*)im->act1_p, (void*)im->a_hi, (void*)im->a_lo, (void*)im->h_hi,
-                        (void*)im->h_lo, (void*)im->w1b, (void*)im->w2b, (void*)im->wd1_hi, (void*)im->wd1_lo,
+                        (void*)im->h_lo, (void*)im->sched, (void*)im->w1b, (void*)im->w2b, (void*)im->wd1_hi, (void*)im->wd1_lo,
                         (void*)im->wd2_hi, (void*)im->wd2_lo})
             if (p) cudaFree(p);
         delete im;
diff --git a/mmwave_msc_b200/csrc/pose_tc.cuh b/mmwave_msc_b200/csrc/pose_tc.cuh
--- a/mmwave_msc_b200/csrc/pose_tc.cuh
+++ b/mmwave_msc_b200/csrc/pose_tc.cuh
@@ -21,6 +21,10 @@
     float* results = nullptr;
     const int32_t* row_track = nullptr;
     FadeCfg fade = {0, 0, 0, 0, 0, 0};
+    const int* rows_r0 = nullptr;
+    const unsigned* rows_ready = nullptr;
+    const unsigned* feat_ready = nullptr;
+    unsigned epoch = 0;
 };
 
 int pose_tc_init(PoseTc* tc, const float* host_blob, const size_t* off, int D, int rows_cap);
diff --git a/mmwave_msc_b200/csrc/step_kernel.cu b/mmwave_msc_b200/csrc/step_kernel.cu
--- a/mmwave_msc_b200/csrc/step_kernel.cu
+++ b/mmwave_msc_b200/csrc/step_kernel.cu
@@ -1025,13 +1025,35 @@
             if (lane == 0 && v) atomicAdd(&a.counters[k], (unsigned long long)v);
         }
     }
+    __shared__ int s_last;
     __syncthreads();
     if (tid == 0) {
         __threadfence();
-        if (atomicAdd(a.defer_done, 1) == (int)gridDim.x - 1) {
-            if (a.defer_hint != nullptr) *a.defer_hint = n_defer;
-            *a.defer_count = 0;
-            *a.defer_done = 0;
+        s_last = atomicAdd(a.defer_done, 1) == (int)gridDim.x - 1;
+    }
+    __syncthreads();
+    if (!s_last) return;
+    __threadfence();
+    if (tid == 0) {
+        if (a.defer_hint != nullptr) *a.defer_hint = n_defer;
+        *a.defer_count = 0;
+        *a.defer_done = 0;
+    }
+    if (a.nr_extra != nullptr) {
+        __shared__ int s_rows[kBigThreads / 32];
+        int part = 0;
+        for (int i = tid; i < a.n_scenes; i += kBigThreads) part += a.pose_cnt[i];
+        part = __reduce_add_sync(kFullMask, part);
+        if (lane == 0) s_rows[warp] = part;
+        __syncthreads();
+        if (tid == 0) {
+            int total = __ldcg(a.nr_extra);
+            for (int w = 0; w < kBigThreads / 32; ++w) total += s_rows[w];
+            *a.nr_total = total;
+            if (a.nr_rows_hint != nullptr) *a.nr_rows_hint = total;
+            atomicAdd(&a.counters[7], (unsigned long long)total);
+            __threadfence();
+            asm volatile("st.release.gpu.global.u32 [%0], %1;" ::"l"(a.nr_ready), "r"(a.nr_epoch) : "memory");
         }
     }
 }
```

Result: faster. 4.562 million, median of 6 (+7.1%).
